# coolbeam/UPFlow_pytorch

Measured on AMD Instinct MI355X. Metric: frame-pairs/sec at 384x1280 bf16, higher is better.
Workload: dtype bf16; 1 GPU; config2: UPFlow_net inference forward (flow fwd+bwd, occlusion masks, SGU on), 384x1280, batch 4 per GPU, random-init weights; global_batch=4, parallelism=replicas x1 (image pairs sharded, no collective), ranks=1, hip_graph=True, capture_fallback=False, steps_in_flight=4, pyramid_convs=HIP (MFMA kernel), pyramid_dtype=fp16

## Files before the change

### include/upflow_hip.h

```cpp
#ifndef UPFLOW_HIP_H
#define UPFLOW_HIP_H

#ifdef __cplusplus
extern "C" {
#endif

enum { UPF_F32 = 0, UPF_F16 = 1, UPF_BF16 = 2 };
enum { UPF_OK = 0, UPF_EINVAL = -1, UPF_EDTYPE = -2, UPF_EALIGN = -3, UPF_EUNSUPPORTED = -4 };
enum { UPF_MASK_NONE = 0, UPF_MASK_LITERAL = 1, UPF_MASK_ROBUST = 2 };

const char* upf_version(void);
const char* upf_last_error(void);

int upf_corr81_forward(const void* f1, const void* f2, void* out,
                       int B, int C, int H, int W, int dtype,
                       long long out_batch_stride, float leaky_slope, void* stream);

int upf_corr81_forward_timed(const void* f1, const void* f2, void* out,
                             int B, int C, int H, int W, int dtype,
                             long long out_batch_stride, float leaky_slope, void* stream,
                             int nrep, float* avg_us, float* min_us);

int upf_corr81_norm_supported(int C, int dtype);
long long upf_corr81_norm_workspace_bytes(int B, int C, int H, int W);
int upf_corr81_norm_forward(const void* f1, const void* f2, void* out,
                            int B, int C, int H, int W, int dtype,
                            long long out_batch_stride, float leaky_slope, void* workspace, void* stream);
int upf_corr81_norm_forward_c8(const void* f1, const void* f2, void* out8, long long out8_batch_stride,
                               int B, int C, int H, int W, int dtype, float leaky_slope, void* workspace, void* stream);
int upf_corr81_norm_forward_pitched(const void* f1, const void* f2, int f_row_pitch, void* out,
                                    int B, int C, int H, int W, int dtype,
                                    long long out_batch_stride, float leaky_slope, void* workspace, void* stream);
int upf_corr81_norm_forward_c8_pitched(const void* f1, const void* f2, int f_row_pitch, void* out8, long long out8_batch_stride,
                                       int B, int C, int H, int W, int dtype, float leaky_slope, void* workspace, void* stream);
int upf_corr81_norm_forward_mixed(const void* f1, const void* f2, int f_row_pitch, void* out,
                                  int B, int C, int H, int W, int dtype, int out_dtype,
                                  long long out_batch_stride, float leaky_slope, void* workspace, void* stream);
int upf_corr81_norm_forward_c8_mixed(const void* f1, const void* f2, int f_row_pitch, void* out8, long long out8_batch_stride,
                                     int B, int C, int H, int W, int dtype, int out_dtype, float leaky_slope, void* workspace, void* stream);
int upf_corr81_norm_forward_timed(const void* f1, const void* f2, void* out,
                                  int B, int C, int H, int W, int dtype,
                                  long long out_batch_stride, float leaky_slope, void* workspace, void* stream,
                                  int nrep, float* avg_us, float* min_us);
int upf_corr81_norm_forward_c8_timed(const void* f1, const void* f2, void* out8, long long out8_batch_stride,
                                     int B, int C, int H, int W, int dtype, float leaky_slope, void* workspace, void* stream,
                                     int nrep, float* avg_us, float* min_us);

int upf_corr81_norm_forward_c8_timed_pitched(const void* f1, const void* f2, int f_row_pitch, void* out8, long long out8_batch_stride,
                                             int B, int C, int H, int W, int dtype, float leaky_slope, void* workspace, void* stream,
                                             int nrep, float* avg_us, float* min_us);

int upf_corr81_norm_forward_c8_timed_mixed(const void* f1, const void* f2, int f_row_pitch, void* out8, long long out8_batch_stride,
                                           int B, int C, int H, int W, int dtype, int out_dtype, float leaky_slope, void* workspace, void* stream,
                                           int nrep, float* avg_us, float* min_us);

int upf_corr_set_option(const char* name, int value);

int upf_corr81_backward(const void* f1, const void* f2, const void* grad_out, void* g1, void* g2,
                        int B, int C, int H, int W, int dtype, void* stream);

int upf_correlation_forward(const void* in1, const void* in2, void* out,
                            int B, int C, int H, int W, int dtype,
                            int pad_size, int kernel_size, int max_displacement,
                            int stride1, int stride2, int corr_type_multiply, void* stream);
int upf_correlation_backward(const void* in1, const void* in2, const void* grad_out, void* g1, void* g2,
                             int B, int C, int H, int W, int dtype,
                             int pad_size, int kernel_size, int max_displacement,
                             int stride1, int stride2, int corr_type_multiply, void* stream);
int upf_correlation_out_shape(int H, int W, int pad_size, int kernel_size, int max_displacement,
                              int stride1, int stride2, int* out_channels, int* out_h, int* out_w);

int upf_warp_forward(const void* x, const float* flow, void* y,
                     int B, int C, int H, int W, int dtype, int mask_mode, int batch_shift, void* stream);
int upf_warp_forward_strided(const void* x, long long x_batch_stride, const float* flow, void* y, long long y_batch_stride,
                             int B, int C, int H, int W, int dtype, int mask_mode, int batch_shift, void* stream);
int upf_warp_forward_pitched(const void* x, long long x_batch_stride, int x_row_pitch, const float* flow, void* y, long long y_batch_stride,
                             int y_row_pitch, int B, int C, int H, int W, int dtype, int mask_mode, int batch_shift, void* stream);
int upf_warp_forward_c8(const void* x8, long long x_batch_stride, const float* flow, void* y8, long long y_batch_stride,
                        int B, int n_oct, int H, int W, int dtype, int mask_mode, int batch_shift, void* stream);
long long upf_warp_backward_workspace_bytes(int B, int C, int H, int W);
int upf_warp_backward(const void* x, const float* flow, const void* grad_y,
                      void* gx, float* gflow, void* workspace,
                      int B, int C, int H, int W, int dtype, int mask_mode, int batch_shift, void* stream);

int upf_flow_upsample_forward(const float* x, float* y, int B, int C, int h, int w, int H, int W,
                              int if_rate, void* stream);
int upf_flow_upsample_backward(const float* grad_y, float* gx, int B, int C, int h, int w, int H, int W,
                               int if_rate, void* stream);

long long upf_sgu_blend_forward_workspace_bytes(int B, int h, int w, int Hf, int Wf);
int upf_sgu_blend_forward(const float* flow_init, const void* x_out, float* flow_up,
                          float* inter_flow, float* inter_mask, void* workspace,
                          int B, int h, int w, int Hf, int Wf, int dtype, void* stream);
int upf_sgu_blend_forward_flow16(const float* flow_init, const void* x_out, float* flow_up, void* flow16, long long flow16_batch_stride,
                                 int flow16_is_c8, int B, int H, int W, int dtype, void* stream);
long long upf_sgu_blend_backward_workspace_bytes(int B, int h, int w, int Hf, int Wf);
int upf_sgu_blend_backward(const float* flow_init, const void* x_out, const float* grad_flow_up,
                           float* g_flow_init32, float* g_x_out32, void* workspace,
                           int B, int h, int w, int Hf, int Wf, int dtype, void* stream);

long long upf_normalize_workspace_bytes(long long N, int HW);
int upf_normalize_forward(const void* x, void* y, float* mean, float* rstd, void* workspace,
                          long long N, int HW, int dtype, void* stream);
int upf_normalize_backward(const void* y, const void* grad_y, const float* rstd, void* gx,
                           long long N, int HW, int dtype, void* stream);

long long upf_conv_packed_bytes(int Cin, int Cout, int kernel_size);
int upf_conv_pack_weights(const void* w , void* w_packed, int Cin, int Cout, int kernel_size,
                          int dtype, void* stream);
int upf_conv_forward(const void* x, long long x_batch_stride, const void* w_packed, const float* bias,
                     void* y, long long y_batch_stride, int B, int Cin, int Cout, int H, int W,
                     int kernel_size, int dilation, int stride, float leaky_slope, int dtype, void* stream);
int upf_conv_forward_pitched(const void* x, long long x_batch_stride, int x_row_pitch, const void* w_packed, const float* bias,
                             void* y, long long y_batch_stride, int y_row_pitch, int B, int Cin, int Cout, int H, int W,
                             int kernel_size, int dilation, int stride, float leaky_slope, int dtype, void* stream);
int upf_conv1x1_forward_mixed(const void* x, long long x_batch_stride, int x_row_pitch, const void* w_packed, const float* bias,
                              void* y, long long y_batch_stride, int y_row_pitch, int y_is_c8, int B, int Cin, int Cout, int H, int W,
                              float leaky_slope, int dtype, int out_dtype, void* stream);
int upf_conv1x1_forward_c8_dual(const void* x, long long x_batch_stride, int x_row_pitch, const void* w_packed, const float* bias,
                                void* y8_a, long long ya_batch_stride, void* y8_b, long long yb_batch_stride,
                                int B, int Cin, int Cout, int H, int W, float leaky_slope, int dtype, int out_dtype, void* stream);
int upf_conv_set_option(const char* name, int value);

long long upf_conv_x3_packed_bytes(int Cin, int Cout, int kernel_size);
int upf_conv_x3_pack_weights(const float* w, void* w_packed, int Cin, int Cout, int kernel_size, void* stream);
int upf_conv_x3_forward(const float* x, long long x_batch_stride, const void* w_packed, const float* bias, float* y,
                        long long y_batch_stride, int B, int Cin, int Cout, int H, int W, int kernel_size, int dilation,
                        int stride, float leaky_slope, int nprod, void* stream);
int upf_conv_x3_set_option(const char* name, int value);
int upf_mfma_f16_denorm_probe(float* out_device, void* stream);

long long upf_conv_packed_bytes_k(int K, int Cout, int kernel_size);
int upf_conv_c8_k(int n8_oct, int C2);
int upf_conv_pack_weights_kmap(const void* w , void* w_packed, int Cin, int Cout, int kernel_size,
                               const int* kmap , int K, int dtype, void* stream);
int upf_conv_forward_c8(const void* x8, long long x8_batch_stride, int n8_oct, const void* x2, long long x2_batch_stride, int C2,
                        const void* w_packed, const float* bias, void* y, long long y_batch_stride, int y_is_c8,
                        int B, int Cout, int H, int W, int kernel_size, int dilation, int stride, float leaky_slope,
                        int dtype, void* stream);
int upf_conv_forward_c8_pitched(const void* x8, long long x8_batch_stride, int n8_oct, const void* x2, long long x2_batch_stride, int x2_row_pitch, int C2,
                                const void* w_packed, const float* bias, void* y, long long y_batch_stride, int y_row_pitch, int y_is_c8,
                                int B, int Cout, int H, int W, int kernel_size, int dilation, int stride, float leaky_slope,
                                int dtype, void* stream);
int upf_conv_c8_set_option(const char* name, int value);
long long upf_conv_packed_bytes_k16(int K, int Cout);
int upf_conv_pack_weights_kmap16(const void* w , void* w_packed, int Cin, int Cout,
                                 const int* kmap , int K, int dtype, void* stream);
int upf_conv_forward_c8_narrow(const void* x8, long long x8_batch_stride, int n8_oct, const void* w_packed16, const float* bias,
                               void* y, long long y_batch_stride, int y_is_c8, int B, int Cout, int H, int W, float leaky_slope,
                               int dtype, void* stream);
int upf_conv_forward_c8_split(const void* x8, long long x8_batch_stride, int n8_oct, const void* w_packed ,
                              const float* bias , void* y8, long long y_batch_stride, int C_main,
                              float* partial, long long partial_batch_stride , int partial_pitch ,
                              int B, int Cout, int H, int W, float leaky_slope, int dtype, void* stream);
int upf_conv_forward_c8_narrow_init(const void* x8, long long x8_batch_stride, int n8_oct, const void* w_packed16,
                                    const float* partial, long long partial_batch_stride, int partial_pitch, int partial_offset ,
                                    void* y, long long y_batch_stride, int y_is_c8, int B, int Cout, int H, int W, float leaky_slope,
                                    int dtype, void* stream);

int upf_conv_pair_forward(const void* x, long long x_batch_stride, int x_row_pitch, int Cin,
                          const void* wa_packed, const float* bias_a , float slope_a, int C1, int stride_a,
                          const void* wb_packed, const float* bias_b , float slope_b, int C2, int stride_b,
                          void* y, long long y_batch_stride, int y_row_pitch, int y_is_c8,
                          int B, int H, int W, int dtype, void* stream);

int upf_conv_pack_weights_f32(const float* w , void* w_packed, int Cin, int Cout, int kernel_size,
                              int dtype, int dgrad, void* stream);
int upf_conv_pack_weights_f32_multi(const float* const* w, void* const* w_packed, const int* Cin, const int* Cout, const int* kernel_size,
                                    const int* dgrad, int njobs, int dtype, void* stream);
int upf_conv_pack_stacked_dgrad(const float* const* w, const int* Cin, const int* Cout, const int* first_channel, int nlayers,
                                void* const* w_packed, const int* slice_channel, const int* slice_width, const int* nconsumers,
                                int nslices, int dtype, void* stream);
int upf_leaky_backward(const void* grad_y, const void* y, void* grad_pre, long long n, float slope, int dtype, void* stream);
int upf_conv_wgrad_supported(int Cin, int Cout, int H, int W, int kernel_size, int dilation, int stride, int dtype);
long long upf_conv_wgrad_workspace_bytes(int B, int Cin, int Cout, int H, int W, int kernel_size, int dilation);
int upf_conv_wgrad(const void* x, long long x_batch_stride, const void* grad_pre, long long g_batch_stride, float* grad_w,
                   void* workspace, int B, int Cin, int Cout, int H, int W, int kernel_size, int dilation, int dtype, void* stream);
typedef struct {
  const void* x;        long long x_batch_stride;
  const void* grad_pre; long long g_batch_stride;
  int B, H, W;
} upf_wgrad_level;
long long upf_conv_wgrad_multi_workspace_bytes(const upf_wgrad_level* levels, int nlevels, int Cin, int Cout, int kernel_size, int dilation);
int upf_conv_wgrad_multi(const upf_wgrad_level* levels , int nlevels, float* grad_w, void* workspace, int Cin, int Cout,
                         int kernel_size, int dilation, int dtype, void* stream);
int upf_conv_wgrad_multi_bias(const upf_wgrad_level* levels, int nlevels, float* grad_w, void* workspace, int Cin, int Cout,
                              int kernel_size, int dilation, const float* const* bias_partials , int npartials, float* grad_bias,
                              int dtype, void* stream);
int upf_space_to_depth2(const void* src, void* dst, int B, int C , int H, int W , int inverse, int dtype, void* stream);
int upf_conv_wgrad_s2d(const upf_wgrad_level* levels, int nlevels, float* grad_w, void* workspace, int Cin, int Cout, int dtype, void* stream);
int upf_act_grad(const void* src, long long src_batch_stride, const void* add, long long add_batch_stride, const void* y,
                 long long y_batch_stride, void* dst, long long dst_batch_stride, float* bias_partial, int B, int C, int HW,
                 float slope, int dtype, void* stream);
int upf_conv_forward_gated(const void* x, long long x_batch_stride, int x_row_pitch, const void* w_packed, const float* bias,
                           void* y, long long y_batch_stride, int y_row_pitch, const void* add, long long add_batch_stride,
                           const void* act, long long act_batch_stride, float mask_slope,
                           int B, int Cin, int Cout, int H, int W, int dtype, void* stream);
int upf_conv_bias_grad_finish(const float* const* partials , int npartials, float* grad_bias,
                              int Cout, void* stream);
long long upf_conv_bias_grad_workspace_bytes(int Cout);
int upf_conv_bias_grad(const void* grad_pre, long long g_batch_stride, float* grad_bias, void* workspace, int B, int Cout, int HW,
                       int dtype, void* stream);

int upf_act_grad_x3(const float* grad_y, long long gy_batch_stride, const float* y, long long y_batch_stride, float* grad_pre_scaled,
                    long long dst_batch_stride, float* bias_partial, float* scale_slot, int B, int C, int HW, float slope, void* stream);
int upf_conv_x3_pack_weights_dgrad(const float* w, void* w_packed, int Cin, int Cout, int kernel_size, void* stream);
int upf_conv_x3_dgrad(const float* grad_pre_scaled, long long g_batch_stride, const float* scale_slot, const float* w,
                      void* w_packed_dgrad, const float* zero_bias, float* grad_x, long long gx_batch_stride, int B, int Cin,
                      int Cout, int H, int W, int kernel_size, int dilation, int stride, void* stream);
int upf_conv_x3_wgrad_workspace_bytes(const upf_wgrad_level* levels, int nlevels, int Cin, int Cout, int kernel_size,
                                      int dilation, int stride, long long* bytes );
int upf_conv_x3_wgrad(const upf_wgrad_level* levels , const float* const* scale_slots , int nlevels,
                      float* grad_w, void* workspace, int Cin, int Cout, int kernel_size, int dilation, int stride,
                      const float* const* bias_partials , float* grad_bias, void* stream);

int upf_flow_update(const float* a, const void* b, const void* c, void* out, long long out_batch_stride,
                    int out_is_f32, int N, int per_item, int dtype, void* stream);
int upf_flow_update_c8(const float* a, const void* b, const void* c, void* out8, long long out8_batch_stride,
                       int N, int HW, int dtype, void* stream);

int upf_occ_check(const float* flow_f, const float* flow_b, float* occ_fw, float* occ_bw,
                  int B, int H, int W, float alpha1, float alpha2, void* stream);

int upf_div_selftest(int size, unsigned long long* mismatches, void* stream);

int upf_census_forward(const float* gray1, const float* gray2, float* dist, int B, int H, int W, int max_distance, void* stream);
int upf_census_backward(const float* gray1, const float* gray2, const float* grad_dist, float* g_gray1, float* g_gray2,
                        int B, int H, int W, int max_distance, void* stream);

int upf_boundary_warp_forward(const float* image, const float* flow, const float* start, float* out,
                              int B, int C, int Hi, int Wi, int h, int w, void* stream);
int upf_boundary_warp_backward(const float* image, const float* flow, const float* start, const float* grad_out,
                               float* grad_flow, int B, int C, int Hi, int Wi, int h, int w, void* stream);

int upf_loss_partials(long long n_pixels);

int upf_robust_loss_forward(const float* x, const float* y, const float* occ, float* partials,
                            int B, int C, int HW, float eps, float q, void* stream);
int upf_robust_loss_backward(const float* x, const float* y, const float* occ, const float* coef,
                             float* grad_x, float* grad_y, int B, int C, int HW, float eps, float q, void* stream);

int upf_grey_forward(const float* image, float* grey, int B, int HW, void* stream);

int upf_msd_upup_partials(int B, int H, int W);
int upf_msd_upup_forward(const float* const* x_low, const int* hs, const int* ws, int nlevels, const float* y, const float* occ,
                         float* partials, float* out2, int B, int H, int W, float weight, float eps, float q, void* stream);
int upf_msd_upup_backward(const float* const* x_low, float* const* grad_x_low, const int* hs, const int* ws, int nlevels, const float* y,
                          const float* occ, const float* grad_out, const float* fwd_out2, int B, int H, int W, float weight, float eps, float q,
                          void* stream);

int upf_smooth_edge1_forward(const float* img, const float* pred, float* partials,
                             int B, int Ci, int Cp, int H, int W, void* stream);
int upf_smooth_edge1_backward(const float* img, const float* pred, const float* grad_up, float* grad_pred,
                              int B, int Ci, int Cp, int H, int W, void* stream);


int upf_smooth_edge2_forward(const float* img, const float* pred, float* partials,
                             int B, int Ci, int Cp, int H, int W, void* stream);
int upf_smooth_edge2_backward(const float* img, const float* pred, const float* grad_up, float* grad_pred,
                              int B, int Ci, int Cp, int H, int W, void* stream);

int upf_smooth_delta_forward(const float* flow, float* partials, int BC, int H, int W, int second_order, void* stream);
int upf_smooth_delta_backward(const float* flow, const float* grad_up, float* grad_flow, int BC, int H, int W,
                              int second_order, void* stream);

enum { UPF_LOSS_CHARBONNIER = 0, UPF_LOSS_L1 = 1 };
int upf_pointwise_loss_forward(const float* x, const float* y, const float* occ, float* partials,
                               int B, int C, int HW, int kind, float q, void* stream);
int upf_pointwise_loss_backward(const float* x, const float* y, const float* occ, const float* coef,
                                float* grad_x, float* grad_y, int B, int C, int HW, int kind, float q, void* stream);

int upf_ssim_forward(const float* x, const float* y, const float* weight, float* map, float* w_avg, float* partials,
                     int B, int C, int H, int W, float c2, float weight_epsilon, void* stream);
int upf_ssim_backward(const float* x, const float* y, const float* weight, const float* grad_map,
                      const float* coef_w, const float* coef_u, float* grad_x, float* grad_y,
                      int B, int C, int H, int W, float c2, float weight_epsilon, void* stream);

#define UPF_MT_TENSORS 48
#define UPF_MT_BLOCKS 256
#define UPF_MT_CHUNK 16384
typedef struct {
  void* param[UPF_MT_TENSORS];
  void* grad[UPF_MT_TENSORS];
  void* exp_avg[UPF_MT_TENSORS];
  void* exp_avg_sq[UPF_MT_TENSORS];
  void* max_exp_avg_sq[UPF_MT_TENSORS];
  int numel[UPF_MT_TENSORS];
  int block_chunk[UPF_MT_BLOCKS];
  unsigned char block_tensor[UPF_MT_BLOCKS];
  int n_tensors, n_blocks;
} upf_mt_launch;
int upf_grads_nonfinite_check(const upf_mt_launch* launch, int* flag, void* stream);
int upf_adam_amsgrad_step(const upf_mt_launch* launch, const float* lr, const float* step, const float* loss_scale,
                          const int* flag, double beta1, double beta2, double eps, double weight_decay, void* stream);
int upf_loss_scale_update(float* loss_scale, int* growth_tracker, int* skipped_steps, int* flag, float* steps, int nsteps,
                          float growth_factor, float backoff_factor, int growth_interval, void* stream);

int upf_frames_u8_assemble(const unsigned char* src1, const unsigned char* src2, const int* aug, float* raw1, float* raw2,
                           float* crop1, float* crop2, float* start, int B, int H, int W, int ph, int pw,
                           double mean0, double mean1, double mean2, double stddev, void* stream);

int upf_frames_u8_stack16(const unsigned char* src1, const unsigned char* src2, const int* flip,
                          void* x, int x_dtype, long long x_pitch, long long x_batch_stride,
                          void* xd, int xd_dtype, long long xd_pitch, long long xd_batch_stride,
                          int B, int H, int W, double mean0, double mean1, double mean2, double stddev, void* stream);

#ifdef __cplusplus
}
#endif
#endif
```

### upflow_pytorch_amd/_build.py

```python
import os
import subprocess
import sys

PKG = os.path.dirname(os.path.abspath(__file__))
CSRC = os.path.join(PKG, 'csrc')
LIB = os.path.join(PKG, 'libupflow_hip.so')

SOURCES = [
    ('api.hip', []),
    ('corr81_fwd.hip', ['-ffp-contract=off']),
    ('corr81_bwd.hip', []),
    ('conv3x3.hip', []),
    ('conv_c8.hip', []),
    ('conv_pair.hip', []),
    ('conv_x3.hip', []),
    ('conv_x3_bwd.hip', []),
    ('conv_wgrad.hip', []),
    ('warp.hip', ['-ffp-contract=off']),
    ('sgu_blend.hip', ['-ffp-contract=off']),
    ('misc.hip', ['-ffp-contract=off']),
    ('loss.hip', ['-ffp-contract=off']),
    ('loss_variants.hip', ['-ffp-contract=off']),
    ('optim.hip', ['-ffp-contract=off']),
    ('ingest.hip', ['-ffp-contract=off']),
]
COMMON = ['--offload-arch=gfx950', '-O3', '-std=c++17', '-fPIC', '-fno-gpu-rdc', '-Wall', '-Wno-unused-function']
NO_PACKED_FP32 = ['-Xclang', '-target-feature', '-Xclang', '-packed-fp32-ops']


def hipcc():
    for c in (os.environ.get('HIPCC'), '/opt/rocm/bin/hipcc', 'hipcc'):
        if c and (os.path.isabs(c) and os.path.exists(c) or not os.path.isabs(c)):
            return c
    raise RuntimeError('hipcc not found')


def _stale(target, deps):
    if not os.path.exists(target):
        return True
    t = os.path.getmtime(target)
    return any(os.path.getmtime(d) > t for d in deps)


def _flags_tag(extra):
    import hashlib
    return hashlib.sha256(' '.join(COMMON + NO_PACKED_FP32 + list(extra)).encode()).hexdigest()[:16]


def _flags_stale(obj, extra):
    try:
        return open(obj + '.flags').read().strip() != _flags_tag(extra)
    except OSError:
        return True


def build(force=False, verbose=False):
    headers = [os.path.join(CSRC, h) for h in os.listdir(CSRC) if h.endswith('.hpp')]
    headers.append(os.path.join(os.path.dirname(PKG), 'include', 'upflow_hip.h'))
    objdir = os.path.join(PKG, 'build')
    os.makedirs(objdir, exist_ok=True)
    objs = []
    cc = hipcc()
    jobs = []
    for src, extra in SOURCES:
        s = os.path.join(CSRC, src)
        o = os.path.join(objdir, src.replace('.hip', '.o'))
        objs.append(o)
        if force or _stale(o, [s] + headers) or _flags_stale(o, extra):
            jobs.append(([cc] + COMMON + NO_PACKED_FP32 + extra + ['-c', s, '-o', o], o, extra))

    def run(job):
        cmd, obj, extra = job
        if os.path.exists(obj + '.flags'):
            os.remove(obj + '.flags')
        if verbose:
            print(' '.join(cmd), flush=True)
        r = subprocess.run(cmd, stderr=subprocess.PIPE, text=True)
        err = '\n'.join(l for l in r.stderr.splitlines() if 'is not a recognized feature for this target' not in l)
        if err.strip():
            sys.stderr.write(err + '\n')
        if r.returncode:
            raise subprocess.CalledProcessError(r.returncode, cmd)
        with open(obj + '.flags', 'w') as f:
            f.write(_flags_tag(extra) + '\n')
    if jobs:
        from concurrent.futures import ThreadPoolExecutor
        with ThreadPoolExecutor(max_workers=min(len(jobs), os.cpu_count() or 1)) as ex:
            list(ex.map(run, jobs))
    if force or _stale(LIB, objs):
        cmd = [cc, '--offload-arch=gfx950', '-shared', '-fPIC', '-o', LIB] + objs
        if verbose:
            print(' '.join(cmd), flush=True)
        subprocess.check_call(cmd)
    return LIB


if __name__ == '__main__':
    print(build(force='--force' in sys.argv, verbose=True))
```

### upflow_pytorch_amd/_lib.py

```python
import ctypes
import os

import torch

_PKG = os.path.dirname(os.path.abspath(__file__))
LIB_PATH = os.environ.get('UPF_HIP_LIB') or os.path.join(_PKG, 'libupflow_hip.so')

UPF_F32, UPF_F16, UPF_BF16 = 0, 1, 2
MASK_NONE, MASK_LITERAL, MASK_ROBUST = 0, 1, 2
_DTYPES = {torch.float32: UPF_F32, torch.float16: UPF_F16, torch.bfloat16: UPF_BF16}

_c = ctypes
_vp, _i, _f, _ll, _d = _c.c_void_p, _c.c_int, _c.c_float, _c.c_longlong, _c.c_double

SIGNATURES = {
    'upf_corr81_forward': [_vp, _vp, _vp, _i, _i, _i, _i, _i, _ll, _f, _vp],
    'upf_corr81_forward_timed': [_vp, _vp, _vp, _i, _i, _i, _i, _i, _ll, _f, _vp, _i, _c.POINTER(_f), _c.POINTER(_f)],
    'upf_corr81_norm_forward': [_vp, _vp, _vp, _i, _i, _i, _i, _i, _ll, _f, _vp, _vp],
    'upf_corr81_norm_forward_timed': [_vp, _vp, _vp, _i, _i, _i, _i, _i, _ll, _f, _vp, _vp, _i, _c.POINTER(_f), _c.POINTER(_f)],
    'upf_corr81_norm_forward_c8_timed': [_vp, _vp, _vp, _ll, _i, _i, _i, _i, _i, _f, _vp, _vp, _i, _c.POINTER(_f), _c.POINTER(_f)],
    'upf_corr81_norm_forward_pitched': [_vp, _vp, _i, _vp, _i, _i, _i, _i, _i, _ll, _f, _vp, _vp],
    'upf_corr81_norm_forward_c8_pitched': [_vp, _vp, _i, _vp, _ll, _i, _i, _i, _i, _i, _f, _vp, _vp],
    'upf_corr81_norm_forward_c8_timed_pitched': [_vp, _vp, _i, _vp, _ll, _i, _i, _i, _i, _i, _f, _vp, _vp, _i, _c.POINTER(_f), _c.POINTER(_f)],
    'upf_corr81_norm_forward_c8_timed_mixed': [_vp, _vp, _i, _vp, _ll, _i, _i, _i, _i, _i, _i, _f, _vp, _vp, _i, _c.POINTER(_f), _c.POINTER(_f)],
    'upf_warp_forward_pitched': [_vp, _ll, _i, _vp, _vp, _ll, _i, _i, _i, _i, _i, _i, _i, _i, _vp],
    'upf_conv_forward_gated': [_vp, _ll, _i, _vp, _vp, _vp, _ll, _i, _vp, _ll, _vp, _ll, _f, _i, _i, _i, _i, _i, _i, _vp],
    'upf_conv_forward_pitched': [_vp, _ll, _i, _vp, _vp, _vp, _ll, _i, _i, _i, _i, _i, _i, _i, _i, _i, _f, _i, _vp],
    'upf_conv_forward_c8_pitched': [_vp, _ll, _i, _vp, _ll, _i, _i, _vp, _vp, _vp, _ll, _i, _i, _i, _i, _i, _i, _i, _i, _i, _f, _i, _vp],
    'upf_corr81_norm_forward_mixed': [_vp, _vp, _i, _vp, _i, _i, _i, _i, _i, _i, _ll, _f, _vp, _vp],
    'upf_corr81_norm_forward_c8_mixed': [_vp, _vp, _i, _vp, _ll, _i, _i, _i, _i, _i, _i, _f, _vp, _vp],
    'upf_conv1x1_forward_mixed': [_vp, _ll, _i, _vp, _vp, _vp, _ll, _i, _i, _i, _i, _i, _i, _i, _f, _i, _i, _vp],
    'upf_conv1x1_forward_c8_dual': [_vp, _ll, _i, _vp, _vp, _vp, _ll, _vp, _ll, _i, _i, _i, _i, _i, _f, _i, _i, _vp],
    'upf_corr81_backward': [_vp, _vp, _vp, _vp, _vp, _i, _i, _i, _i, _i, _vp],
    'upf_correlation_forward': [_vp, _vp, _vp, _i, _i, _i, _i, _i, _i, _i, _i, _i, _i, _i, _vp],
    'upf_correlation_backward': [_vp, _vp, _vp, _vp, _vp, _i, _i, _i, _i, _i, _i, _i, _i, _i, _i, _i, _vp],
    'upf_correlation_out_shape': [_i, _i, _i, _i, _i, _i, _i, _c.POINTER(_i), _c.POINTER(_i), _c.POINTER(_i)],
    'upf_warp_forward': [_vp, _vp, _vp, _i, _i, _i, _i, _i, _i, _i, _vp],
    'upf_warp_forward_strided': [_vp, _ll, _vp, _vp, _ll, _i, _i, _i, _i, _i, _i, _i, _vp],
    'upf_warp_forward_c8': [_vp, _ll, _vp, _vp, _ll, _i, _i, _i, _i, _i, _i, _i, _vp],
    'upf_flow_update': [_vp, _vp, _vp, _vp, _ll, _i, _i, _i, _i, _vp],
    'upf_flow_update_c8': [_vp, _vp, _vp, _vp, _ll, _i, _i, _i, _vp],
    'upf_corr81_norm_forward_c8': [_vp, _vp, _vp, _ll, _i, _i, _i, _i, _i, _f, _vp, _vp],
    'upf_warp_backward': [_vp, _vp, _vp, _vp, _vp, _vp, _i, _i, _i, _i, _i, _i, _i, _vp],
    'upf_flow_upsample_forward': [_vp, _vp, _i, _i, _i, _i, _i, _i, _i, _vp],
    'upf_flow_upsample_backward': [_vp, _vp, _i, _i, _i, _i, _i, _i, _i, _vp],
    'upf_sgu_blend_forward': [_vp, _vp, _vp, _vp, _vp, _vp, _i, _i, _i, _i, _i, _i, _vp],
    'upf_sgu_blend_forward_flow16': [_vp, _vp, _vp, _vp, _ll, _i, _i, _i, _i, _i, _vp],
    'upf_sgu_blend_backward': [_vp, _vp, _vp, _vp, _vp, _vp, _i, _i, _i, _i, _i, _i, _vp],
    'upf_normalize_forward': [_vp, _vp, _vp, _vp, _vp, _ll, _i, _i, _vp],
    'upf_normalize_backward': [_vp, _vp, _vp, _vp, _ll, _i, _i, _vp],
    'upf_conv_pack_weights': [_vp, _vp, _i, _i, _i, _i, _vp],
    'upf_conv_forward': [_vp, _ll, _vp, _vp, _vp, _ll, _i, _i, _i, _i, _i, _i, _i, _i, _f, _i, _vp],
    'upf_conv_x3_pack_weights': [_vp, _vp, _i, _i, _i, _vp],
    'upf_conv_x3_forward': [_vp, _ll, _vp, _vp, _vp, _ll, _i, _i, _i, _i, _i, _i, _i, _i, _f, _i, _vp],
    'upf_mfma_f16_denorm_probe': [_vp, _vp],
    'upf_act_grad_x3': [_vp, _ll, _vp, _ll, _vp, _ll, _vp, _vp, _i, _i, _i, _f, _vp],
    'upf_conv_x3_pack_weights_dgrad': [_vp, _vp, _i, _i, _i, _vp],
    'upf_conv_x3_dgrad': [_vp, _ll, _vp, _vp, _vp, _vp, _vp, _ll, _i, _i, _i, _i, _i, _i, _i, _i, _vp],
    'upf_conv_x3_wgrad_workspace_bytes': [_vp, _i, _i, _i, _i, _i, _i, _c.POINTER(_ll)],
    'upf_conv_x3_wgrad': [_vp, _vp, _i, _vp, _vp, _i, _i, _i, _i, _i, _vp, _vp, _vp],
    'upf_conv_pack_weights_f32': [_vp, _vp, _i, _i, _i, _i, _i, _vp],
    'upf_conv_pack_stacked_dgrad': [_c.POINTER(_vp), _c.POINTER(_i), _c.POINTER(_i), _c.POINTER(_i), _i, _c.POINTER(_vp), _c.POINTER(_i), _c.POINTER(_i), _c.POINTER(_i), _i, _i, _vp],
    'upf_conv_pack_weights_f32_multi': [_c.POINTER(_vp), _c.POINTER(_vp), _c.POINTER(_i), _c.POINTER(_i), _c.POINTER(_i), _c.POINTER(_i), _i, _i, _vp],
    'upf_conv_pack_weights_kmap': [_vp, _vp, _i, _i, _i, _vp, _i, _i, _vp],
    'upf_conv_forward_c8': [_vp, _ll, _i, _vp, _ll, _i, _vp, _vp, _vp, _ll, _i, _i, _i, _i, _i, _i, _i, _i, _f, _i, _vp],
    'upf_conv_pack_weights_kmap16': [_vp, _vp, _i, _i, _vp, _i, _i, _vp],
    'upf_conv_forward_c8_narrow': [_vp, _ll, _i, _vp, _vp, _vp, _ll, _i, _i, _i, _i, _i, _f, _i, _vp],
    'upf_conv_forward_c8_split': [_vp, _ll, _i, _vp, _vp, _vp, _ll, _i, _vp, _ll, _i, _i, _i, _i, _i, _f, _i, _vp],
    'upf_conv_forward_c8_narrow_init': [_vp, _ll, _i, _vp, _vp, _ll, _i, _i, _vp, _ll, _i, _i, _i, _i, _i, _f, _i, _vp],
    'upf_conv_pair_forward': [_vp, _ll, _i, _i, _vp, _vp, _f, _i, _i, _vp, _vp, _f, _i, _i, _vp, _ll, _i, _i, _i, _i, _i, _i, _vp],
    'upf_leaky_backward': [_vp, _vp, _vp, _ll, _f, _i, _vp],
    'upf_conv_wgrad': [_vp, _ll, _vp, _ll, _vp, _vp, _i, _i, _i, _i, _i, _i, _i, _i, _vp],
    'upf_conv_bias_grad': [_vp, _ll, _vp, _vp, _i, _i, _i, _i, _vp],
    'upf_conv_wgrad_multi': [_vp, _i, _vp, _vp, _i, _i, _i, _i, _i, _vp],
    'upf_conv_wgrad_multi_bias': [_vp, _i, _vp, _vp, _i, _i, _i, _i, _vp, _i, _vp, _i, _vp],
    'upf_space_to_depth2': [_vp, _vp, _i, _i, _i, _i, _i, _i, _vp],
    'upf_conv_wgrad_s2d': [_vp, _i, _vp, _vp, _i, _i, _i, _vp],
    'upf_act_grad': [_vp, _ll, _vp, _ll, _vp, _ll, _vp, _ll, _vp, _i, _i, _i, _f, _i, _vp],
    'upf_conv_bias_grad_finish': [_vp, _i, _vp, _i, _vp],
    'upf_census_forward': [_vp, _vp, _vp, _i, _i, _i, _i, _vp],
    'upf_census_backward': [_vp, _vp, _vp, _vp, _vp, _i, _i, _i, _i, _vp],
    'upf_boundary_warp_forward': [_vp, _vp, _vp, _vp, _i, _i, _i, _i, _i, _i, _vp],
    'upf_boundary_warp_backward': [_vp, _vp, _vp, _vp, _vp, _i, _i, _i, _i, _i, _i, _vp],
    'upf_robust_loss_forward': [_vp, _vp, _vp, _vp, _i, _i, _i, _f, _f, _vp],
    'upf_robust_loss_backward': [_vp, _vp, _vp, _vp, _vp, _vp, _i, _i, _i, _f, _f, _vp],
    'upf_grey_forward': [_vp, _vp, _i, _i, _vp],
    'upf_msd_upup_forward': [_vp, _vp, _vp, _i, _vp, _vp, _vp, _vp, _i, _i, _i, _f, _f, _f, _vp],
    'upf_msd_upup_backward': [_vp, _vp, _vp, _vp, _i, _vp, _vp, _vp, _vp, _i, _i, _i, _f, _f, _f, _vp],
    'upf_smooth_edge1_forward': [_vp, _vp, _vp, _i, _i, _i, _i, _i, _vp],
    'upf_smooth_edge1_backward': [_vp, _vp, _vp, _vp, _i, _i, _i, _i, _i, _vp],
    'upf_smooth_edge2_forward': [_vp, _vp, _vp, _i, _i, _i, _i, _i, _vp],
    'upf_smooth_edge2_backward': [_vp, _vp, _vp, _vp, _i, _i, _i, _i, _i, _vp],
    'upf_smooth_delta_forward': [_vp, _vp, _i, _i, _i, _i, _vp],
    'upf_smooth_delta_backward': [_vp, _vp, _vp, _i, _i, _i, _i, _vp],
    'upf_pointwise_loss_forward': [_vp, _vp, _vp, _vp, _i, _i, _i, _i, _f, _vp],
    'upf_pointwise_loss_backward': [_vp, _vp, _vp, _vp, _vp, _vp, _i, _i, _i, _i, _f, _vp],
    'upf_ssim_forward': [_vp, _vp, _vp, _vp, _vp, _vp, _i, _i, _i, _i, _f, _f, _vp],
    'upf_ssim_backward': [_vp, _vp, _vp, _vp, _vp, _vp, _vp, _vp, _i, _i, _i, _i, _f, _f, _vp],
    'upf_div_selftest': [_i, _vp, _vp],
    'upf_occ_check': [_vp, _vp, _vp, _vp, _i, _i, _i, _f, _f, _vp],
    'upf_grads_nonfinite_check': [_vp, _vp, _vp],
    'upf_adam_amsgrad_step': [_vp, _vp, _vp, _vp, _vp, _d, _d, _d, _d, _vp],
    'upf_loss_scale_update': [_vp, _vp, _vp, _vp, _vp, _i, _f, _f, _i, _vp],
    'upf_frames_u8_assemble': [_vp, _vp, _vp, _vp, _vp, _vp, _vp, _vp, _i, _i, _i, _i, _i, _d, _d, _d, _d, _vp],
    'upf_frames_u8_stack16': [_vp, _vp, _vp, _vp, _i, _ll, _ll, _vp, _i, _ll, _ll, _i, _i, _i, _d, _d, _d, _d, _vp],
}



class WgradLevel(_c.Structure):
    _fields_ = [('x', _vp), ('x_batch_stride', _ll), ('grad_pre', _vp), ('g_batch_stride', _ll), ('B', _i), ('H', _i), ('W', _i)]


MT_TENSORS, MT_BLOCKS, MT_CHUNK = 48, 256, 16384


class MtLaunch(_c.Structure):
    _fields_ = [('param', _vp * MT_TENSORS), ('grad', _vp * MT_TENSORS), ('exp_avg', _vp * MT_TENSORS),
                ('exp_avg_sq', _vp * MT_TENSORS), ('max_exp_avg_sq', _vp * MT_TENSORS), ('numel', _i * MT_TENSORS),
                ('block_chunk', _i * MT_BLOCKS), ('block_tensor', _c.c_ubyte * MT_BLOCKS), ('n_tensors', _i), ('n_blocks', _i)]


_lib = None


class UpflowHipError(RuntimeError):
    """Raised for a rejected argument or a failed launch (the reference raises RuntimeError through
    AT_ERROR("CUDA call failed"), correlation_cuda.cc:81-83)."""


def lib():
    global _lib
    if _lib is None:
        if not os.path.exists(LIB_PATH):
            raise UpflowHipError(
                '%s is missing: build it with `python -c "import __graft_entry__ as g; g.build()"` '
                '(hipcc --offload-arch=gfx950). There is no CPU fallback.' % LIB_PATH)
        L = ctypes.CDLL(LIB_PATH)
        for name, argtypes in SIGNATURES.items():
            fn = getattr(L, name)
            fn.argtypes = argtypes
            fn.restype = _i
        L.upf_normalize_workspace_bytes.argtypes = [_ll, _i]
        L.upf_normalize_workspace_bytes.restype = _ll
        L.upf_corr81_norm_supported.argtypes = [_i, _i]
        L.upf_corr81_norm_supported.restype = _i
        L.upf_corr81_norm_workspace_bytes.argtypes = [_i, _i, _i, _i]
        L.upf_corr81_norm_workspace_bytes.restype = _ll
        L.upf_corr_set_option.argtypes = [_c.c_char_p, _i]
        L.upf_corr_set_option.restype = _i
        L.upf_warp_backward_workspace_bytes.argtypes = [_i, _i, _i, _i]
        L.upf_warp_backward_workspace_bytes.restype = _ll
        L.upf_sgu_blend_backward_workspace_bytes.argtypes = [_i, _i, _i, _i, _i]
        L.upf_sgu_blend_backward_workspace_bytes.restype = _ll
        L.upf_sgu_blend_forward_workspace_bytes.argtypes = [_i, _i, _i, _i, _i]
        L.upf_sgu_blend_forward_workspace_bytes.restype = _ll
        L.upf_conv_wgrad_supported.argtypes = [_i] * 8
        L.upf_conv_wgrad_supported.restype = _i
        L.upf_conv_wgrad_workspace_bytes.argtypes = [_i] * 7
        L.upf_conv_wgrad_workspace_bytes.restype = _ll
        L.upf_conv_wgrad_multi_workspace_bytes.argtypes = [_vp, _i, _i, _i, _i, _i]
        L.upf_conv_wgrad_multi_workspace_bytes.restype = _ll
        L.upf_conv_bias_grad_workspace_bytes.argtypes = [_i]
        L.upf_conv_bias_grad_workspace_bytes.restype = _ll
        L.upf_loss_partials.argtypes = [_ll]
        L.upf_loss_partials.restype = _i
        L.upf_msd_upup_partials.argtypes = [_i, _i, _i]
        L.upf_msd_upup_partials.restype = _i
        L.upf_conv_packed_bytes.argtypes = [_i, _i, _i]
        L.upf_conv_packed_bytes.restype = _ll
        L.upf_conv_x3_packed_bytes.argtypes = [_i, _i, _i]
        L.upf_conv_x3_packed_bytes.restype = _ll
        L.upf_conv_set_option.argtypes = [_c.c_char_p, _i]
        L.upf_conv_set_option.restype = _i
        L.upf_conv_c8_set_option.argtypes = [_c.c_char_p, _i]
        L.upf_conv_c8_set_option.restype = _i
        L.upf_conv_x3_set_option.argtypes = [_c.c_char_p, _i]
        L.upf_conv_x3_set_option.restype = _i
        L.upf_conv_packed_bytes_k.argtypes = [_i, _i, _i]
        L.upf_conv_packed_bytes_k.restype = _ll
        L.upf_conv_c8_k.argtypes = [_i, _i]
        L.upf_conv_c8_k.restype = _i
        L.upf_conv_packed_bytes_k16.argtypes = [_i, _i]
        L.upf_conv_packed_bytes_k16.restype = _ll
        L.upf_version.restype = _c.c_char_p
        L.upf_last_error.restype = _c.c_char_p
        _lib = L
        for item in filter(None, os.environ.get('UPF_CONV_OPTS', '').split(',')):
            k, v = item.split('=')
            if L.upf_conv_set_option(k.strip().encode(), int(v)) == -2 ** 31:
                raise UpflowHipError('UPF_CONV_OPTS: unknown option %r' % k)
    return _lib


def version():
    return lib().upf_version().decode()


def dtype_code(t):
    try:
        return _DTYPES[t.dtype]
    except KeyError:
        raise UpflowHipError('unsupported dtype %s (float32 / float16 / bfloat16 only)' % t.dtype)


def check_gpu(*tensors, contiguous=True):
    dev = None
    for t in tensors:
        if t is None:
            continue
        if not t.is_cuda:
            raise UpflowHipError('upflow_pytorch_amd operators run on the GPU only (got a %s tensor); '
                                 'there is no CPU fallback' % t.device)
        if contiguous and not t.is_contiguous():
            raise UpflowHipError('operand must be contiguous NCHW')
        if dev is None:
            dev = t.device
        elif t.device != dev:
            raise UpflowHipError('operands on different devices: %s vs %s' % (dev, t.device))
    return dev


def stream_ptr(device):
    return _vp(torch.cuda.current_stream(device).cuda_stream)


def ptr(t):
    return _vp(t.data_ptr()) if t is not None else _vp(0)


def call(name, *args):
    rc = getattr(lib(), name)(*args)
    if rc != 0:
        raise UpflowHipError('%s failed (%d): %s' % (name, rc, lib().upf_last_error().decode()))


def launch(device, name, *args):
    with torch.cuda.device(device):
        call(name, *args, stream_ptr(device))
```

### upflow_pytorch_amd/csrc/conv_c8.hip

```cpp
#include "conv_kernel.hpp"

namespace upf {
namespace conv {

template <typename T>
__global__ void pack_weights_kmap_kernel(const T* __restrict__ w, T* __restrict__ wp, int Cin, int Cout, int ntaps, const int* __restrict__ kmap, int K) {
  const int cop = pad32(Cout), nk = K / 16;
  const long long total = (long long)ntaps * cop * K;
  for (long long i = blockIdx.x * (long long)blockDim.x + threadIdx.x; i < total; i += (long long)gridDim.x * blockDim.x) {
    const int j = (int)(i & 7), px = (int)((i >> 3) & 31), kg = (int)((i >> 8) & 1);
    const long long b = i >> 9;
    const int tap = (int)(b % ntaps), kstep = (int)((b / ntaps) % nk), slab = (int)(b / ((long long)ntaps * nk));
    const int co = slab * 32 + px, kk = kstep * 16 + kg * 8 + j;
    const int ci = kmap[kk];
    T v; v.v = 0;
    if (ci >= 0 && ci < Cin && co < Cout) v = w[((size_t)co * Cin + ci) * ntaps + tap];
    wp[i] = v;
  }
}

template <typename T>
__global__ void pack_weights_kmap16_kernel(const T* __restrict__ w, T* __restrict__ wp, int Cin, int Cout, int ntaps, const int* __restrict__ kmap, int K) {
  const int nblk = (Cout + 15) / 16, nch = K / 32;
  const long long total = (long long)nblk * nch * ntaps * 512;
  for (long long i = blockIdx.x * (long long)blockDim.x + threadIdx.x; i < total; i += (long long)gridDim.x * blockDim.x) {
    const int j = (int)(i & 7), lane = (int)((i >> 3) & 63);
    const long long b = i >> 9;
    const int tap = (int)(b % ntaps), chunk = (int)((b / ntaps) % nch), blk = (int)(b / ((long long)ntaps * nch));
    const int co = blk * 16 + (lane & 15), kk = chunk * 32 + (lane >> 4) * 8 + j;
    const int ci = kmap[kk];
    T v; v.v = 0;
    if (ci >= 0 && ci < Cin && co < Cout) v = w[((size_t)co * Cin + ci) * ntaps + tap];
    wp[i] = v;
  }
}

struct ArgsC8 {
  const void* x8; long long x8bs; int n8oct;
  const void* x2; long long x2bs; int C2;
  const void* wp; const float* bias; void* y; long long ybs;
  int B, Cout, H, W, d, stride, ntaps; float slope; hipStream_t stream;
  int x2pitch, ypitch;
};

template <typename T, int MTW, int RPW, int S, int NOCTS, int D, int XL, bool YC8, bool N16 = false>
int launch_one_c8(const ArgsC8& a, int slabs) {
  constexpr int TH = (4 / MTW) * RPW;
  constexpr bool PH = (D >= 2 && S == 1);
  constexpr int DV = PH ? 1 : D;
  constexpr int rowsC = S * (TH - 1) + 2 * DV + 1;
  constexpr int XWP = xwp_eff(XL, S, D);
  constexpr int EB = NOCTS * rowsC * XWP, EBP = (EB + 63) & ~63;
  const int Ho = (a.H - 1) / S + 1, Wo = (a.W - 1) / S + 1;
  const int tiles_x = cdiv(Wo, TW), tiles_y = PH ? cdiv(Ho, D * TH) * D : cdiv(Ho, TH);
  size_t lds = (XL >= 1) ? (size_t)2 * EBP * 16 : (size_t)EB * 16;
  if (!YC8 && !N16 && lds < 4 * EPI_WAVE_BYTES) lds = 4 * EPI_WAVE_BYTES;
  UPF_REQUIRE(lds <= 160 * 1024, UPF_EUNSUPPORTED, "conv_forward_c8: tile does not fit LDS (dilation %d)", a.d);
  static LdsOptIn opt;
  auto kern = &conv_kernel<T, MTW, RPW, S, NOCTS, D, false, false, XL, YC8, N16>;
  opt.ensure(reinterpret_cast<const void*>(kern), lds);
  hipLaunchKernelGGL(kern, dim3((unsigned)(a.B * tiles_x * tiles_y), slabs), dim3(NTHREADS), lds, a.stream, (const T*)a.x2, a.x2bs,
                     (const T*)a.wp, a.bias, (T*)a.y, a.ybs, a.C2, a.Cout, a.H, a.W, Ho, Wo, g_ablate, tiles_x, tiles_y, a.slope,
                     (const T*)a.x8, a.x8bs, a.n8oct, a.x2pitch, a.ypitch);
  return check_launch("conv_forward_c8");
}

inline int g_c8_rpw4 = 1;
inline int g_c8_narrow_tall = 0;

template <typename T, int XL, bool YC8>
int launch_c8(const ArgsC8& a) {
  const int mt = cdiv(a.Cout, 32);
  const long long tiles = (long long)a.B * cdiv(a.W, TW) * cdiv(a.H, 8);
  int mtw = mt >= 3 ? 4 : mt;
  if (tiles <= g_small_grid && mt > 1) mtw = 2;
  if (g_force_mtw == 1 || g_force_mtw == 2 || g_force_mtw == 4) mtw = g_force_mtw < (mt >= 3 ? 4 : mt) ? g_force_mtw : (mt >= 3 ? 4 : mt);
  const int slabs = cdiv(mt, mtw);
  if (a.ntaps == 1) {
    if constexpr (XL == 0 && YC8) {
      if (mtw == 1) return launch_one_c8<T, 1, 2, 1, 4, 0, 0, true>(a, slabs);
    }
    set_error("conv_forward_c8: 1x1 kernels take an NCHW input, a C8 output and Cout <= 32");
    return UPF_EUNSUPPORTED;
  }
  if (a.stride == 2) {
    if constexpr (XL == 0 && YC8) {
      if (a.d == 1 && a.Cout <= 32 && a.C2 > 16) return launch_one_c8<T, 1, 2, 2, 4, 1, 0, true>(a, 1);
    }
    set_error("conv_forward_c8: stride 2 takes an NCHW input of more than 16 channels, a C8 output of at most 32 channels, dilation 1");
    return UPF_EUNSUPPORTED;
  }
  if (a.d == 1) {
    if constexpr (XL == 0 && YC8) {
      if (mtw == 4) return launch_one_c8<T, 4, 8, 1, 2, 1, 0, true>(a, slabs);
      if (mtw == 2) return launch_one_c8<T, 2, 4, 1, 4, 1, 0, true>(a, slabs);
      return launch_one_c8<T, 1, 2, 1, 4, 1, 0, true>(a, slabs);
    }
    if constexpr (XL >= 1) {
      if (mtw == 4) return launch_one_c8<T, 4, 8, 1, 2, 1, XL, YC8>(a, slabs);
      if (mtw == 2) return launch_one_c8<T, 2, 4, 1, 4, 1, XL, YC8>(a, slabs);
      if (g_c8_rpw4 && (long long)a.B * cdiv(a.W, TW) * cdiv(a.H, 16) >= g_rpw4_min) return launch_one_c8<T, 1, 4, 1, 2, 1, XL, YC8>(a, slabs);
      return launch_one_c8<T, 1, 2, 1, 4, 1, XL, YC8>(a, slabs);
    }
  }
  if constexpr (XL == 1 && YC8) {
    if (a.d == 2 || a.d == 4 || a.d == 8 || a.d == 16) {
      const int th = g_ph_fit ? ph_tile_rows(a.H, a.d, mtw) : 8;
#define UPF_C8_PH(MT, RP)                                                              \
      switch (a.d) {                                                                   \
        case 2: return launch_one_c8<T, MT, RP, 1, wide_nocts<MT, 2>(), 2, 1, true>(a, slabs);   \
        case 4: return launch_one_c8<T, MT, RP, 1, wide_nocts<MT, 4>(), 4, 1, true>(a, slabs);   \
        case 8: return launch_one_c8<T, MT, RP, 1, wide_nocts<MT, 8>(), 8, 1, true>(a, slabs);   \
        default: return launch_one_c8<T, MT, RP, 1, wide_nocts<MT, 16>(), 16, 1, true>(a, slabs); \
      }
      if (mtw == 4) { if (th == 6) { UPF_C8_PH(4, 6) } if (th == 4) { UPF_C8_PH(4, 4) } UPF_C8_PH(4, 8) }
      if (mtw == 2) { if (th == 6) { UPF_C8_PH(2, 3) } if (th == 4) { UPF_C8_PH(2, 2) } UPF_C8_PH(2, 4) }
      if (th == 4) { UPF_C8_PH(1, 1) }
      UPF_C8_PH(1, 2)
#undef UPF_C8_PH
    }
  }
  set_error("conv_forward_c8: no kernel for this combination (kernel %d taps, dilation %d, input layout %d, output C8 %d)", a.ntaps, a.d, XL, (int)YC8);
  return UPF_EUNSUPPORTED;
}

template <typename T>
int dispatch_c8(const ArgsC8& a, bool y_c8) {
  const int xl = a.x8 ? (a.x2 ? 2 : 1) : 0;
  if (xl == 2) return y_c8 ? launch_c8<T, 2, true>(a) : launch_c8<T, 2, false>(a);
  if (xl == 1) return y_c8 ? launch_c8<T, 1, true>(a) : launch_c8<T, 1, false>(a);
  if (y_c8) return launch_c8<T, 0, true>(a);
  set_error("conv_forward_c8: NCHW in, NCHW out is upf_conv_forward");
  return UPF_EINVAL;
}

}
}

extern "C" long long upf_conv_packed_bytes_k(int K, int Cout, int kernel_size) {
  return (long long)kernel_size * kernel_size * upf::conv::pad32(Cout) * (long long)K * 2;
}

extern "C" int upf_conv_c8_k(int n8_oct, int C2) {
  return (n8_oct > 0 ? upf::conv::pad32(n8_oct * 8) : 0) + (C2 > 0 ? upf::conv::pad32(C2) : 0);
}

extern "C" int upf_conv_pack_weights_kmap(const void* w, void* w_packed, int Cin, int Cout, int kernel_size, const int* kmap, int K,
                                          int dtype, void* stream) {
  using namespace upf;
  UPF_REQUIRE(w && w_packed && kmap && Cin > 0 && Cout > 0, UPF_EINVAL, "conv_pack_weights_kmap: bad arguments");
  UPF_REQUIRE(kernel_size == 3 || kernel_size == 1, UPF_EUNSUPPORTED, "conv_pack_weights_kmap: kernel_size %d (1 or 3)", kernel_size);
  UPF_REQUIRE(K > 0 && K % 32 == 0, UPF_EINVAL, "conv_pack_weights_kmap: K = %d must be a positive multiple of 32", K);
  UPF_REQUIRE(dtype == UPF_BF16 || dtype == UPF_F16, UPF_EDTYPE, "conv: bf16 / fp16 only");
  const int ntaps = kernel_size * kernel_size;
  const long long total = (long long)ntaps * conv::pad32(Cout) * K;
  const int blocks = (int)((total + 255) / 256 > 4096 ? 4096 : (total + 255) / 256);
  if (dtype == UPF_BF16)
    hipLaunchKernelGGL((conv::pack_weights_kmap_kernel<bf16_t>), dim3(blocks), dim3(256), 0, (hipStream_t)stream, (const bf16_t*)w, (bf16_t*)w_packed, Cin, Cout, ntaps, kmap, K);
  else
    hipLaunchKernelGGL((conv::pack_weights_kmap_kernel<f16_t>), dim3(blocks), dim3(256), 0, (hipStream_t)stream, (const f16_t*)w, (f16_t*)w_packed, Cin, Cout, ntaps, kmap, K);
  return check_launch("conv_pack_weights_kmap");
}

extern "C" int upf_conv_c8_set_option(const char* name, int value) {
  using namespace upf::conv;
  int* slot = nullptr;
  if (name && !strcmp(name, "rpw4")) slot = &g_c8_rpw4;
  else if (name && !strcmp(name, "narrow_tall")) slot = &g_c8_narrow_tall;
  if (!slot) return INT32_MIN;
  const int prev = *slot;
  *slot = value;
  return prev;
}

extern "C" int upf_conv_forward_c8_pitched(const void* x8, long long x8_batch_stride, int n8_oct, const void* x2, long long x2_batch_stride, int x2_row_pitch, int C2,
                                           const void* w_packed, const float* bias, void* y, long long y_batch_stride, int y_row_pitch, int y_is_c8,
                                           int B, int Cout, int H, int W, int kernel_size, int dilation, int stride, float leaky_slope,
                                           int dtype, void* stream) {
  using namespace upf;
  UPF_REQUIRE((x8 || x2) && w_packed && bias && y, UPF_EINVAL, "conv_forward_c8: null pointer");
  UPF_REQUIRE((x8 != nullptr) == (n8_oct > 0) && (x2 != nullptr) == (C2 > 0), UPF_EINVAL, "conv_forward_c8: a pointer and its channel count disagree");
  UPF_REQUIRE(B > 0 && Cout > 0 && H > 0 && W > 0, UPF_EINVAL, "conv_forward_c8: bad shape B=%d Cout=%d H=%d W=%d", B, Cout, H, W);
  UPF_REQUIRE(dtype == UPF_BF16 || dtype == UPF_F16, UPF_EDTYPE, "conv_forward_c8: bf16 / fp16 only");
  UPF_REQUIRE(kernel_size == 3 || kernel_size == 1, UPF_EUNSUPPORTED, "conv_forward_c8: kernel_size %d (1 or 3)", kernel_size);
  UPF_REQUIRE(stride == 1 || (stride == 2 && kernel_size == 3 && dilation == 1 && !x8), UPF_EUNSUPPORTED, "conv_forward_c8: stride %d (1, or 2 for a 3x3 with an NCHW input)", stride);
  UPF_REQUIRE(dilation >= 1 && dilation <= conv::MAXD, UPF_EUNSUPPORTED, "conv_forward_c8: dilation %d not in [1,%d]", dilation, conv::MAXD);
  const int Ho = (H - 1) / stride + 1, Wo = (W - 1) / stride + 1;
  if (x2_row_pitch == 0) x2_row_pitch = W;
  if (y_row_pitch == 0) y_row_pitch = Wo;
  UPF_REQUIRE(!x2 || (x2_row_pitch >= W && x2_row_pitch % 8 == 0), UPF_EUNSUPPORTED,
              "conv_forward_c8: the NCHW input's row pitch %d must be a multiple of 8 and >= W = %d (pitched rows, or upf_conv_forward)", x2_row_pitch, W);
  UPF_REQUIRE(y_is_c8 || y_row_pitch >= Wo, UPF_EINVAL, "conv_forward_c8: output row pitch %d < %d", y_row_pitch, Wo);
  UPF_REQUIRE(!x8 || (aligned_to(x8, 16) && x8_batch_stride % 8 == 0), UPF_EINVAL, "conv_forward_c8: the C8 input must be 16-byte aligned");
  UPF_REQUIRE(!x2 || (aligned_to(x2, 16) && x2_batch_stride % 8 == 0), UPF_EINVAL, "conv_forward_c8: the NCHW input must be 16-byte aligned");
  UPF_REQUIRE(!y_is_c8 || (aligned_to(y, 16) && y_batch_stride % 8 == 0), UPF_EINVAL, "conv_forward_c8: the C8 output must be 16-byte aligned");
  UPF_REQUIRE((long long)n8_oct * H * W * 16 < (1ll << 31) && (long long)C2 * H * x2_row_pitch * 2 < (1ll << 31), UPF_EINVAL, "conv_forward_c8: image too large for one buffer descriptor");
  UPF_REQUIRE((long long)((Cout + 7) / 8) * (H / stride + 1) * (W / stride + 1) * 16 < (1ll << 31) && (y_is_c8 || (long long)Cout * Ho * y_row_pitch * 2 < (1ll << 31)), UPF_EINVAL,
              "conv_forward_c8: output too large for one buffer descriptor");
  UPF_REQUIRE(leaky_slope >= 0.f && leaky_slope <= 1.f, UPF_EINVAL, "conv_forward_c8: leaky_slope %g not in [0,1]", (double)leaky_slope);
  conv::ArgsC8 a{x8, x8_batch_stride, n8_oct, x2, x2_batch_stride, C2, w_packed, bias, y, y_batch_stride,
                 B, Cout, H, W, kernel_size == 1 ? 0 : dilation, stride, kernel_size * kernel_size, leaky_slope == 0.f ? 1.f : leaky_slope, (hipStream_t)stream,
                 x2_row_pitch, y_row_pitch};
  return dtype == UPF_BF16 ? conv::dispatch_c8<bf16_t>(a, y_is_c8 != 0) : conv::dispatch_c8<f16_t>(a, y_is_c8 != 0);
}

extern "C" int upf_conv_forward_c8(const void* x8, long long x8_batch_stride, int n8_oct, const void* x2, long long x2_batch_stride, int C2,
                                   const void* w_packed, const float* bias, void* y, long long y_batch_stride, int y_is_c8,
                                   int B, int Cout, int H, int W, int kernel_size, int dilation, int stride, float leaky_slope,
                                   int dtype, void* stream) {
  return upf_conv_forward_c8_pitched(x8, x8_batch_stride, n8_oct, x2, x2_batch_stride, 0, C2, w_packed, bias, y, y_batch_stride, 0, y_is_c8,
                                     B, Cout, H, W, kernel_size, dilation, stride, leaky_slope, dtype, stream);
}

extern "C" long long upf_conv_packed_bytes_k16(int K, int Cout) {
  return (long long)((Cout + 15) / 16) * (upf::conv::pad32(K) / 32) * 9 * 1024;
}

extern "C" int upf_conv_pack_weights_kmap16(const void* w, void* w_packed, int Cin, int Cout, const int* kmap, int K, int dtype, void* stream) {
  using namespace upf;
  UPF_REQUIRE(w && w_packed && kmap && Cin > 0 && Cout > 0 && K > 0 && K % 32 == 0, UPF_EINVAL, "conv_pack_weights_kmap16: bad arguments (K %% 32 == 0)");
  UPF_REQUIRE(dtype == UPF_BF16 || dtype == UPF_F16, UPF_EDTYPE, "conv_pack_weights_kmap16: bf16 / fp16 only");
  const long long total = (long long)((Cout + 15) / 16) * (K / 32) * 9 * 512;
  const int blocks = (int)((total + 255) / 256 > 4096 ? 4096 : (total + 255) / 256);
  if (dtype == UPF_BF16)
    hipLaunchKernelGGL((conv::pack_weights_kmap16_kernel<bf16_t>), dim3(blocks), dim3(256), 0, (hipStream_t)stream, (const bf16_t*)w, (bf16_t*)w_packed, Cin, Cout, 9, kmap, K);
  else
    hipLaunchKernelGGL((conv::pack_weights_kmap16_kernel<f16_t>), dim3(blocks), dim3(256), 0, (hipStream_t)stream, (const f16_t*)w, (f16_t*)w_packed, Cin, Cout, 9, kmap, K);
  return check_launch("conv_pack_weights_kmap16");
}

extern "C" int upf_conv_forward_c8_narrow(const void* x8, long long x8_batch_stride, int n8_oct, const void* w_packed16, const float* bias,
                                          void* y, long long y_batch_stride, int y_is_c8, int B, int Cout, int H, int W, float leaky_slope,
                                          int dtype, void* stream) {
  using namespace upf;
  UPF_REQUIRE(x8 && n8_oct > 0 && w_packed16 && bias && y, UPF_EINVAL, "conv_forward_c8_narrow: null pointer");
  UPF_REQUIRE(B > 0 && Cout > 0 && H > 0 && W > 0, UPF_EINVAL, "conv_forward_c8_narrow: bad shape B=%d Cout=%d H=%d W=%d", B, Cout, H, W);
  UPF_REQUIRE(dtype == UPF_BF16 || dtype == UPF_F16, UPF_EDTYPE, "conv_forward_c8_narrow: bf16 / fp16 only");
  UPF_REQUIRE(aligned_to(x8, 16) && x8_batch_stride % 8 == 0, UPF_EINVAL, "conv_forward_c8_narrow: the C8 input must be 16-byte aligned");
  UPF_REQUIRE(!y_is_c8 || (aligned_to(y, 16) && y_batch_stride % 8 == 0), UPF_EINVAL, "conv_forward_c8_narrow: the C8 output must be 16-byte aligned");
  UPF_REQUIRE((long long)n8_oct * H * W * 16 < (1ll << 31), UPF_EINVAL, "conv_forward_c8_narrow: input too large for one buffer descriptor");
  UPF_REQUIRE((long long)(y_is_c8 ? (Cout + 7) / 8 * 8 : Cout) * H * W * 2 < (1ll << 31), UPF_EINVAL, "conv_forward_c8_narrow: output too large for one buffer descriptor");
  UPF_REQUIRE(leaky_slope >= 0.f && leaky_slope <= 1.f, UPF_EINVAL, "conv_forward_c8_narrow: leaky_slope %g not in [0,1]", (double)leaky_slope);
  conv::ArgsC8 a{x8, x8_batch_stride, n8_oct, nullptr, 0, 0, w_packed16, bias, y, y_batch_stride, B, Cout, H, W, 1, 1, 9,
                 leaky_slope == 0.f ? 1.f : leaky_slope, (hipStream_t)stream, W, W};
  const int blocks16 = (Cout + 15) / 16;
  const bool tall = conv::g_c8_narrow_tall && (long long)B * cdiv(W, conv::TW) * cdiv(H, 16) >= conv::g_rpw4_min;
#define UPF_N16(T)                                                                                                   \
  if (y_is_c8) return tall ? conv::launch_one_c8<T, 1, 4, 1, 4, 1, 1, true, true>(a, blocks16) : conv::launch_one_c8<T, 1, 2, 1, 4, 1, 1, true, true>(a, blocks16);   \
  return tall ? conv::launch_one_c8<T, 1, 4, 1, 4, 1, 1, false, true>(a, blocks16) : conv::launch_one_c8<T, 1, 2, 1, 4, 1, 1, false, true>(a, blocks16);
  if (dtype == UPF_BF16) { UPF_N16(bf16_t) }
  UPF_N16(f16_t)
#undef UPF_N16
}

namespace upf {
namespace conv {

template <typename T, int MTW, int RPW, int NOCTS>
int launch_split(const ArgsC8& a, const SplitOut& so) {
  constexpr int TH = (4 / MTW) * RPW;
  constexpr int rowsC = (TH - 1) + 2 + 1;
  constexpr int XWP = xwp_eff(1, 1, 1);
  constexpr int EB = NOCTS * rowsC * XWP, EBP = (EB + 63) & ~63;
  const int tiles_x = cdiv(a.W, TW), tiles_y = cdiv(a.H, TH);
  const size_t lds = (size_t)2 * EBP * 16;
  static LdsOptIn opt;
  auto kern = &conv_split_kernel<T, MTW, RPW, NOCTS>;
  opt.ensure(reinterpret_cast<const void*>(kern), lds);
  hipLaunchKernelGGL(kern, dim3((unsigned)(a.B * tiles_x * tiles_y), (unsigned)cdiv(cdiv(a.Cout, 32), MTW)), dim3(NTHREADS), lds, a.stream, (const T*)a.wp, a.bias, (T*)a.y, a.ybs,
                     a.Cout, a.H, a.W, tiles_x, tiles_y, a.slope, (const T*)a.x8, a.x8bs, a.n8oct, so);
  return check_launch("conv_forward_c8_split");
}

template <typename T>
int dispatch_split(const ArgsC8& a, const SplitOut& so) {
  const int mt = cdiv(a.Cout, 32);
  const long long tiles = (long long)a.B * cdiv(a.W, TW) * cdiv(a.H, 8);
  int mtw = mt >= 3 ? 4 : mt;
  if (tiles <= g_small_grid && mt > 1) mtw = 2;
  if (mtw == 4) return launch_split<T, 4, 8, 2>(a, so);
  if (mtw == 2) return launch_split<T, 2, 4, 4>(a, so);
  if (g_c8_rpw4 && (long long)a.B * cdiv(a.W, TW) * cdiv(a.H, 16) >= g_rpw4_min) return launch_split<T, 1, 4, 2>(a, so);
  return launch_split<T, 1, 2, 4>(a, so);
}

template <typename T, int RPW, bool YC8>
int launch_accinit(const ArgsC8& a, const AccInit& ai) {
  constexpr int TH = 4 * RPW;
  constexpr int rowsC = (TH - 1) + 2 + 1;
  constexpr int XWP = xwp_eff(1, 1, 1);
  constexpr int EB = 4 * rowsC * XWP, EBP = (EB + 63) & ~63;
  const int tiles_x = cdiv(a.W, TW), tiles_y = cdiv(a.H, TH);
  const size_t lds = (size_t)2 * EBP * 16;
  static LdsOptIn opt;
  auto kern = &conv_accinit_kernel<T, RPW, YC8>;
  opt.ensure(reinterpret_cast<const void*>(kern), lds);
  hipLaunchKernelGGL(kern, dim3((unsigned)(a.B * tiles_x * tiles_y), (unsigned)cdiv(a.Cout, 16)), dim3(NTHREADS), lds, a.stream, (const T*)a.wp, (T*)a.y, a.ybs,
                     a.Cout, a.H, a.W, tiles_x, tiles_y, a.slope, (const T*)a.x8, a.x8bs, a.n8oct, ai);
  return check_launch("conv_forward_c8_narrow_init");
}

}
}

extern "C" int upf_conv_forward_c8_split(const void* x8, long long x8_batch_stride, int n8_oct, const void* w_packed, const float* bias,
                                         void* y8, long long y_batch_stride, int C_main, float* partial, long long partial_batch_stride, int partial_pitch,
                                         int B, int Cout, int H, int W, float leaky_slope, int dtype, void* stream) {
  using namespace upf;
  UPF_REQUIRE(x8 && n8_oct > 0 && w_packed && bias && y8 && partial, UPF_EINVAL, "conv_forward_c8_split: null pointer");
  UPF_REQUIRE(B > 0 && H > 0 && W > 0, UPF_EINVAL, "conv_forward_c8_split: bad shape B=%d H=%d W=%d", B, H, W);
  UPF_REQUIRE(C_main > 0 && C_main % 8 == 0 && Cout > C_main && Cout <= 128, UPF_EINVAL,
              "conv_forward_c8_split: C_main = %d must be a positive multiple of 8 below Cout = %d <= 128", C_main, Cout);
  UPF_REQUIRE(partial_pitch % 4 == 0 && partial_pitch >= (Cout - C_main + 3) / 4 * 4, UPF_EINVAL,
              "conv_forward_c8_split: partial pitch %d must be a multiple of 4 floats holding the %d partial channels", partial_pitch, Cout - C_main);
  UPF_REQUIRE(dtype == UPF_BF16 || dtype == UPF_F16, UPF_EDTYPE, "conv_forward_c8_split: bf16 / fp16 only");
  UPF_REQUIRE(aligned_to(x8, 16) && x8_batch_stride % 8 == 0 && aligned_to(y8, 16) && y_batch_stride % 8 == 0 && aligned_to(partial, 16) && partial_batch_stride % 4 == 0,
              UPF_EINVAL, "conv_forward_c8_split: operands must be 16-byte aligned");
  UPF_REQUIRE((long long)n8_oct * H * W * 16 < (1ll << 31) && (long long)H * W * partial_pitch * 4 < (1ll << 31), UPF_EINVAL,
              "conv_forward_c8_split: image too large for one buffer descriptor");
  UPF_REQUIRE(leaky_slope >= 0.f && leaky_slope <= 1.f, UPF_EINVAL, "conv_forward_c8_split: leaky_slope %g not in [0,1]", (double)leaky_slope);
  conv::ArgsC8 a{x8, x8_batch_stride, n8_oct, nullptr, 0, 0, w_packed, bias, y8, y_batch_stride, B, Cout, H, W, 1, 1, 9,
                 leaky_slope == 0.f ? 1.f : leaky_slope, (hipStream_t)stream, W, W};
  const conv::SplitOut so{partial, partial_batch_stride, partial_pitch, C_main};
  return dtype == UPF_BF16 ? conv::dispatch_split<bf16_t>(a, so) : conv::dispatch_split<f16_t>(a, so);
}

extern "C" int upf_conv_forward_c8_narrow_init(const void* x8, long long x8_batch_stride, int n8_oct, const void* w_packed16,
                                               const float* partial, long long partial_batch_stride, int partial_pitch, int partial_offset,
                                               void* y, long long y_batch_stride, int y_is_c8, int B, int Cout, int H, int W, float leaky_slope,
                                               int dtype, void* stream) {
  using namespace upf;
  UPF_REQUIRE(x8 && n8_oct > 0 && w_packed16 && partial && y, UPF_EINVAL, "conv_forward_c8_narrow_init: null pointer");
  UPF_REQUIRE(B > 0 && Cout > 0 && Cout <= 16 && H > 0 && W > 0, UPF_EINVAL, "conv_forward_c8_narrow_init: bad shape B=%d Cout=%d (<= 16) H=%d W=%d", B, Cout, H, W);
  UPF_REQUIRE(partial_pitch % 4 == 0 && partial_offset % 4 == 0 && partial_offset >= 0 && partial_offset + (Cout + 3) / 4 * 4 <= partial_pitch, UPF_EINVAL,
              "conv_forward_c8_narrow_init: partial pitch %d / offset %d must be multiples of 4 floats holding the layer's %d channels", partial_pitch, partial_offset, Cout);
  UPF_REQUIRE(dtype == UPF_BF16 || dtype == UPF_F16, UPF_EDTYPE, "conv_forward_c8_narrow_init: bf16 / fp16 only");
  UPF_REQUIRE(aligned_to(x8, 16) && x8_batch_stride % 8 == 0 && aligned_to(partial, 16) && partial_batch_stride % 4 == 0, UPF_EINVAL,
              "conv_forward_c8_narrow_init: the C8 input and the partial must be 16-byte aligned");
  UPF_REQUIRE(!y_is_c8 || (aligned_to(y, 16) && y_batch_stride % 8 == 0), UPF_EINVAL, "conv_forward_c8_narrow_init: the C8 output must be 16-byte aligned");
  UPF_REQUIRE((long long)n8_oct * H * W * 16 < (1ll << 31) && (long long)H * W * partial_pitch * 4 < (1ll << 31), UPF_EINVAL,
              "conv_forward_c8_narrow_init: image too large for one buffer descriptor");
  UPF_REQUIRE((long long)(y_is_c8 ? (Cout + 7) / 8 * 8 : Cout) * H * W * 2 < (1ll << 31), UPF_EINVAL, "conv_forward_c8_narrow_init: output too large for one buffer descriptor");
  UPF_REQUIRE(leaky_slope >= 0.f && leaky_slope <= 1.f, UPF_EINVAL, "conv_forward_c8_narrow_init: leaky_slope %g not in [0,1]", (double)leaky_slope);
  conv::ArgsC8 a{x8, x8_batch_stride, n8_oct, nullptr, 0, 0, w_packed16, nullptr, y, y_batch_stride, B, Cout, H, W, 1, 1, 9,
                 leaky_slope == 0.f ? 1.f : leaky_slope, (hipStream_t)stream, W, W};
  const conv::AccInit ai{partial, partial_batch_stride, partial_pitch, partial_offset};
#define UPF_N16I(T) return y_is_c8 ? conv::launch_accinit<T, 2, true>(a, ai) : conv::launch_accinit<T, 2, false>(a, ai);
  if (dtype == UPF_BF16) { UPF_N16I(bf16_t) }
  UPF_N16I(f16_t)
#undef UPF_N16I
}
```

### upflow_pytorch_amd/csrc/conv_kernel.hpp

```cpp
#pragma once
#include "common.hpp"
#include <cstring>
#include <cstdint>

namespace upf {
namespace conv {

constexpr int TW = 32, NTHREADS = 256;
constexpr int MAXD = 16;
__host__ __device__ constexpr int margin_of(int D) { return (D == 16 || D < 0) ? 16 : 8; }
__host__ __device__ constexpr int xw(int S, int marg) { return S * TW + 2 * marg; }
#ifndef UPF_C8_TIGHT
#define UPF_C8_TIGHT 1
#endif
__host__ __device__ constexpr bool tight_rows(int XL) { return XL == 1 && UPF_C8_TIGHT != 0; }
__host__ __device__ constexpr int marg_eff(int XL, int D) { return tight_rows(XL) ? (D > 0 ? D : 0) : margin_of(D); }
__host__ __device__ constexpr int xw_eff(int XL, int S, int D) { return xw(S, marg_eff(XL, D)); }
__host__ __device__ constexpr int xwp_eff(int XL, int S, int D) { return tight_rows(XL) ? (xw_eff(XL, S, D) | 1) : xw_eff(XL, S, D) + xw_eff(XL, S, D) / 16; }

typedef __attribute__((ext_vector_type(8))) __bf16 bf16x8;
typedef __attribute__((ext_vector_type(8))) _Float16 f16x8;
typedef __attribute__((ext_vector_type(16))) float f32x16;
typedef __attribute__((ext_vector_type(4))) float f32x4;
typedef __attribute__((ext_vector_type(4))) unsigned int u32x4;
// ... 321 lines not shown
  const int colx[3] = {pos_of(marg + px - (D > 0 ? D : 0)), pos_of(marg + px), pos_of(marg + px + (D > 0 ? D : 0))};

  auto matrix_phase = [&](const uint4* __restrict__ xb, int cc) {
    __builtin_amdgcn_s_setprio(2);

    if (abl & 1) {
    } else if constexpr (N16) {
      constexpr int NR = RPW + 2;
      const int c16[2][3] = {{pos_of(marg + p16 - 1), pos_of(marg + p16), pos_of(marg + p16 + 1)}, {pos_of(marg + p16 + 15), pos_of(marg + p16 + 16), pos_of(marg + p16 + 17)}};
      uint4 bq[2][6];
      auto bload = [&](int sr, uint4 (&b)[6]) {
#pragma unroll
        for (int h = 0; h < 2; ++h)
#pragma unroll
          for (int kx = 0; kx < 3; ++kx) b[h * 3 + kx] = xb[(ko * rows + RPW * rg + sr) * XWP + c16[h][kx]];
      };
      bload(0, bq[0]);
#pragma unroll
      for (int sr = 0; sr < NR; ++sr) {
        if (sr + 1 < NR) bload(sr + 1, bq[(sr + 1) & 1]);
        __builtin_amdgcn_sched_barrier(0);
#pragma unroll
        for (int kx = 0; kx < 3; ++kx)
#pragma unroll
          for (int h = 0; h < 2; ++h)
#pragma unroll
            for (int ky = 0; ky < 3; ++ky)
              if (sr - ky >= 0 && sr - ky < RPW)
                acc16[sr - ky][h] = Mma16<T>::mma(wa[ky * 3 + kx][0], bq[sr & 1][h * 3 + kx], acc16[sr - ky][h]);
#pragma unroll
        for (int ky = 0; ky < 3; ++ky)
          if (sr == ky + RPW - 1) {
#pragma unroll
            for (int kx = 0; kx < 3; ++kx) wa[ky * 3 + kx][0] = wload(cc + 1, ky * 3 + kx, 0);
          }
        __builtin_amdgcn_sched_barrier(0);
      }
    } else if constexpr (REUSE) {
      constexpr int NR = RPW + 2 * DV;
      uint4 bq[2][3 * KS];
      auto bload = [&](int sr, uint4 (&b)[3 * KS]) {
#pragma unroll
        for (int kx = 0; kx < 3; ++kx)
#pragma unroll
          for (int ks = 0; ks < KS; ++ks) b[kx * KS + ks] = xb[((2 * ks + kg) * rows + RPW * rg + sr) * XWP + colx[kx]];
      };
      constexpr bool PIPEB = !ONE;
      if constexpr (PIPEB) bload(0, bq[0]);
#pragma unroll
      for (int sr = 0; sr < NR; ++sr) {
        if constexpr (PIPEB) { if (sr + 1 < NR) bload(sr + 1, bq[(sr + 1) & 1]); }
        else bload(sr, bq[sr & 1]);
        __builtin_amdgcn_sched_barrier(0);
#pragma unroll
        for (int kx = 0; kx < 3; ++kx)
#pragma unroll
          for (int ks = 0; ks < KS; ++ks)
#pragma unroll
            for (int ky = 0; ky < 3; ++ky)
              if (sr - ky * DV >= 0 && sr - ky * DV < RPW)
                acc[sr - ky * DV] = Mma32<T>::mma(wa[ky * 3 + kx][ks], bq[sr & 1][kx * KS + ks], acc[sr - ky * DV]);
#pragma unroll
        for (int ky = 0; ky < 3; ++ky)
          if (sr == ky * DV + RPW - 1) {
#pragma unroll
            for (int kx = 0; kx < 3; ++kx)
#pragma unroll
              for (int ks = 0; ks < KS; ++ks) wa[ky * 3 + kx][ks] = wload(cc + 1, ky * 3 + kx, ks);
          }
        __builtin_amdgcn_sched_barrier(0);
      }
    } else {
#pragma unroll
      for (int tap = 0; tap < ntaps; ++tap) {
        const int ky = (ntaps == 1) ? 1 : tap / 3, kx = (ntaps == 1) ? 1 : tap - 3 * (tap / 3);
        const int col = pos_of(marg + S * px + (kx - 1) * d);
#pragma unroll
        for (int ks = 0; ks < KS; ++ks)
#pragma unroll
          for (int r = 0; r < RPW; ++r) {
            const uint4 b = xb[((2 * ks + kg) * rows + S * (RPW * rg + r) + ky * (PH ? 1 : d)) * XWP + col];
            acc[r] = Mma32<T>::mma(wa[tap][ks], b, acc[r]);
          }
#pragma unroll
        for (int ks = 0; ks < KS; ++ks) wa[tap][ks] = wload(cc + 1, tap, ks);
      }
    }
    __builtin_amdgcn_s_setprio(0);
  };

  if constexpr (XL >= 1) {
    constexpr int rowsC = S * (TH - 1) + 2 * DV + 1;
    constexpr int EB = NOCTS * rowsC * XWP, EBP = (EB + 63) & ~63;
    constexpr int NSL = (EBP / 64 + 3) / 4;
    constexpr int DH = (D > 0) ? D : 0;
    const int wave_u = __builtin_amdgcn_readfirstlane(wave);
    __amdgpu_buffer_rsrc_t x8r = __builtin_amdgcn_make_buffer_rsrc(const_cast<T*>(x8 + (size_t)n * x8bs), 0, (uint32_t)n8oct * (uint32_t)HW * 16u, 0x00020000);
    uint32_t voff8[NSL];
#pragma unroll
    for (int j = 0; j < NSL; ++j) {
      const int p = (j * 4 + wave_u) * 64 + lane;
      const int oct = p / (rowsC * XWP), rem = p - oct * (rowsC * XWP), r = rem / XWP, pos = rem - r * XWP;
      const int grp = pos & ~7, col = LIN ? pos : (grp | ((pos - (grp >> 4)) & 7));
      const int gy = PH ? y0 + (r - 1) * RS : S * y0 - DV + r, gx = S * x0 - marg + col;
      const bool in = p < EB && pos < XW && col >= marg - DH && col < marg + S * TW + DH && gy >= 0 && gy < H && gx >= 0 && gx < W && !(abl & 2);
      voff8[j] = in ? (uint32_t)((oct * HW + gy * W + gx) * 16) : 0x80000000u;
    }
    auto land = [&](int cc) {
      if constexpr (XL == 2) {
        if (cc >= n8c && cc < nchunks) {
          uint4* xb = xs + (cc & 1) * EBP;
          if (tid < ntasks) stage_store<false>(xb, dst0, sh0, pre);
          for (int t = tid + NTHREADS; t < ntasks; t += NTHREADS) {
            uint32_t off; int dsti, sh;
            task_geom(t, off, dsti, sh);
            u32x4 ch[8];
            task_load(off, cc - n8c, ch);
            stage_store<false>(xb, dsti, sh, ch);
          }
        }
      }
    };
    for (int cc = -1; cc < nchunks; ++cc) {
      const int nx = cc + 1;
      if (nx < n8c) {
        const uint32_t cadd = (uint32_t)nx * (uint32_t)(NOCTS * 16) * (uint32_t)HW;
#pragma unroll
        for (int j = 0; j < NSL; ++j) {
          const int piece = j * 4 + wave_u;
          if (piece * 64 < EBP)
            __builtin_amdgcn_raw_ptr_buffer_load_lds(x8r, (__attribute__((address_space(3))) void*)(xs + ((nx & 1) * EBP + piece * 64)), 16, (int)(voff8[j] + cadd), 0, 0, 0);
        }
      } else if constexpr (XL == 2) {
        if (nx < nchunks) task_load(off0, nx - n8c, pre);
      }
      if (cc >= 0) matrix_phase(xs + (cc & 1) * EBP, cc);
      land(nx);
      asm volatile("s_waitcnt vmcnt(0)" ::: "memory");
      __syncthreads();
    }
  } else {
  for (int cc = 0; cc < nchunks; ++cc) {
      __syncthreads();
      if constexpr (PRE) { if (tid < ntasks) task_store(dst0, sh0, pre); }
      for (int t = tid + (PRE ? NTHREADS : 0); t < ntasks; t += NTHREADS) {
        uint32_t off; int dsti, sh;
        task_geom(t, off, dsti, sh);
        u32x4 ch[8];
        task_load(off, cc, ch);
        task_store(dsti, sh, ch);
      }
      __syncthreads();
      if constexpr (PRE) { if (cc + 1 < nchunks) task_load(off0, cc + 1, pre); }
      matrix_phase(xs, cc);
    }
  }

  const int gy0 = __builtin_amdgcn_readfirstlane(y0 + RPW * rg * RS);
  if constexpr (N16) {
    const uint32_t plane16 = (uint32_t)(Ho * Wo) * 16u, plane2 = (uint32_t)(Ho * ypitch) * 2u;
    __amdgpu_buffer_rsrc_t yr = __builtin_amdgcn_make_buffer_rsrc(y + (size_t)n * ybs, 0, YC8 ? (uint32_t)((Cout + 7) / 8) * plane16 : (uint32_t)Cout * plane2, 0x00020000);
#pragma unroll
    for (int r = 0; r < RPW; ++r) {
      const int gy = gy0 + r;
      if (gy < Ho) {
#pragma unroll
        for (int h = 0; h < 2; ++h) {
          const int gx = x0 + p16 + 16 * h;
          float v[4];
#pragma unroll
          for (int i = 0; i < 4; ++i) { v[i] = acc16[r][h][i]; v[i] = fmaxf(v[i], v[i] * slope); }
          if constexpr (YC8) {
            const uint32_t off = (gx < Wo) ? (uint32_t)(slab * 2 + (ko >> 1)) * plane16 + (uint32_t)(gy * Wo + gx) * 16u + (uint32_t)(ko & 1) * 8u : 0x80000000u;
            u32x2 o;
            o.x = pack2<TO>(v[0], v[1]); o.y = pack2<TO>(v[2], v[3]);
            __builtin_amdgcn_raw_buffer_store_b64(o, yr, off, 0, 0);
          } else {
            const uint32_t off = (gx < Wo) ? (uint32_t)(slab * 16 + 4 * ko) * plane2 + (uint32_t)(gy * ypitch + gx) * 2u : 0x80000000u;
            const uint32_t p01 = pack2<TO>(v[0], v[1]), p23 = pack2<TO>(v[2], v[3]);
            __builtin_amdgcn_raw_buffer_store_b16((unsigned short)p01, yr, off, 0, 0);
            __builtin_amdgcn_raw_buffer_store_b16((unsigned short)(p01 >> 16), yr, off + plane2, 0, 0);
            __builtin_amdgcn_raw_buffer_store_b16((unsigned short)p23, yr, off + 2u * plane2, 0, 0);
            __builtin_amdgcn_raw_buffer_store_b16((unsigned short)(p23 >> 16), yr, off + 3u * plane2, 0, 0);
          }
        }
      }
    }
    return;
  }
  if constexpr (!N16) {
  if constexpr (YC8) {
    const uint32_t plane16 = (uint32_t)(Ho * Wo) * 16u;
    int cout_y = Cout;
    if constexpr (G::split) cout_y = gate.cmain;
    __amdgpu_buffer_rsrc_t yr = __builtin_amdgcn_make_buffer_rsrc(y + (size_t)n * ybs, 0, (uint32_t)((cout_y + 7) / 8) * plane16, 0x00020000);
    const int gx = x0 + px;
    const uint32_t lane_off = (gx < Wo) ? (uint32_t)(slab * 4) * plane16 + (uint32_t)gx * 16u + (uint32_t)kg * 8u : 0x80000000u;
    __amdgpu_buffer_rsrc_t pr;
    if constexpr (G::split)
      pr = __builtin_amdgcn_make_buffer_rsrc(gate.part + (size_t)n * gate.pbs, 0, (uint32_t)(Ho * Wo) * (uint32_t)gate.ppitch * 4u, 0x00020000);
#pragma unroll
    for (int r = 0; r < RPW; ++r) {
      const int gy = gy0 + r * RS;
      if (gy < Ho) {
#pragma unroll
        for (int g = 0; g < 4; ++g) {
          if constexpr (G::split) {
            if (slab * 32 + 8 * g >= gate.cmain) {
              const int c0 = slab * 32 + 8 * g + 4 * kg;
              const uint32_t off = (gx < Wo && c0 < Cout) ? (uint32_t)(((c0 - gate.cmain) >> 2) * (Ho * Wo) + gy * Wo + gx) * 16u : 0x80000000u;
              f32x4 pv;
#pragma unroll
              for (int q = 0; q < 4; ++q) pv[q] = acc[r][4 * g + q];
              __builtin_amdgcn_raw_buffer_store_b128(__builtin_bit_cast(u32x4, pv), pr, off, 0, 0);
              continue;
            }
          }
          float v[4];
#pragma unroll
          for (int q = 0; q < 4; ++q) { v[q] = acc[r][4 * g + q]; v[q] = fmaxf(v[q], v[q] * slope); }
          u32x2 o;
          o.x = pack2<TO>(v[0], v[1]); o.y = pack2<TO>(v[2], v[3]);
          __builtin_amdgcn_raw_buffer_store_b64(o, yr, lane_off + (uint32_t)g * plane16 + (uint32_t)(gy * Wo) * 16u, 0, 0);
          if constexpr (G::dual) {
            __amdgpu_buffer_rsrc_t yr2 = __builtin_amdgcn_make_buffer_rsrc(gate.y2 + (size_t)n * gate.y2bs, 0, (uint32_t)((cout_y + 7) / 8) * plane16, 0x00020000);
            __builtin_amdgcn_raw_buffer_store_b64(o, yr2, lane_off + (uint32_t)g * plane16 + (uint32_t)(gy * Wo) * 16u, 0, 0);
          }
        }
      }
    }
    return;
  }
  if constexpr (!GEN) {
    if (((ypitch & 7) | (int)(ybs & 7) | (int)(reinterpret_cast<uintptr_t>(y) & 15)) == 0) {
      __syncthreads();
      if constexpr (G::on) {
        const GateRsrc gr = gate_init<T>(gate, n, (uint32_t)Cout * (uint32_t)(Ho * ypitch) * 2u);
        epilogue_wide<TO, RPW, true>(acc, reinterpret_cast<unsigned char*>(xs) + wave * EPI_WAVE_BYTES, y + (size_t)n * ybs, Cout, Ho, Wo,
                                    slab, lane, x0, gy0, RS, slope, ypitch, &gr);
      } else {
        epilogue_wide<TO, RPW>(acc, reinterpret_cast<unsigned char*>(xs) + wave * EPI_WAVE_BYTES, y + (size_t)n * ybs, Cout, Ho, Wo,
                              slab, lane, x0, gy0, RS, slope, ypitch);
      }
      return;
    }
  }
  Epilogue ep;
  epilogue_init<TO, true>(ep, y + (size_t)n * ybs, Cout, Ho, Wo, slab, lane, x0, ypitch);
  GateRsrc gr;
  if constexpr (G::on) gr = gate_init<T>(gate, n, (uint32_t)Cout * ep.plane2);
#pragma unroll
  for (int r = 0; r < RPW; ++r) {
    if (gy0 + r * RS < Ho) {
#pragma unroll
      for (int j = 0; j < 8; ++j)
        epilogue_store<TO, true, G::on>(ep, acc[r][2 * j], acc[r][2 * j + 1], epilogue_choff(j) * ep.plane2 + (uint32_t)((gy0 + r * RS) * ypitch) * 2u, slope, &gr);
    }
  }
  }
}

template <typename T, int MTW, int RPW, int S, int NOCTS, int D, bool GEN, bool ONE = false, int XL = 0, bool YC8 = false, bool N16 = false, typename TO = T>
__global__ __launch_bounds__(NTHREADS, (ONE && (MTW == 1 || (MTW == 2 && S == 1))) ? 4 : 2)
void conv_kernel(const T* __restrict__ x, long long xbs, const T* __restrict__ wp, const float* __restrict__ bias,
                 TO* __restrict__ y, long long ybs, int Cin, int Cout, int H, int W, int Ho, int Wo, int d_rt,
                 int tiles_x, int tiles_y, float slope, const T* __restrict__ x8, long long x8bs, int n8oct, int xpitch, int ypitch) {
  conv_body<T, MTW, RPW, S, NOCTS, D, GEN, ONE, XL, YC8, N16, TO, NoGate>(x, xbs, wp, bias, y, ybs, Cin, Cout, H, W, Ho, Wo, d_rt, tiles_x, tiles_y, slope,
                                                                          x8, x8bs, n8oct, xpitch, ypitch, NoGate{});
}

template <typename T, int MTW, int RPW, int S, int NOCTS, int D, bool GEN, bool ONE = false>
__global__ __launch_bounds__(NTHREADS, (ONE && (MTW == 1 || (MTW == 2 && S == 1))) ? 4 : 2)
void conv_gated_kernel(const T* __restrict__ x, long long xbs, const T* __restrict__ wp, const float* __restrict__ bias,
                       T* __restrict__ y, long long ybs, int Cin, int Cout, int H, int W, int Ho, int Wo, int d_rt,
                       int tiles_x, int tiles_y, float slope, int xpitch, int ypitch, const ActGate<T> gate) {
  conv_body<T, MTW, RPW, S, NOCTS, D, GEN, ONE, 0, false, false, T, ActGate<T>>(x, xbs, wp, bias, y, ybs, Cin, Cout, H, W, Ho, Wo, d_rt, tiles_x, tiles_y, slope,
                                                                                nullptr, 0ll, 0, xpitch, ypitch, gate);
}

template <typename T, int MTW, int RPW, int NOCTS>
__global__ __launch_bounds__(NTHREADS, 2)
void conv_split_kernel(const T* __restrict__ wp, const float* __restrict__ bias, T* __restrict__ y, long long ybs, int Cout, int H, int W,
                       int tiles_x, int tiles_y, float slope, const T* __restrict__ x8, long long x8bs, int n8oct, const SplitOut so) {
  conv_body<T, MTW, RPW, 1, NOCTS, 1, false, false, 1, true, false, T, SplitOut>(nullptr, 0ll, wp, bias, y, ybs, 0, Cout, H, W, H, W, 0, tiles_x, tiles_y, slope,
                                                                                  x8, x8bs, n8oct, W, W, so);
}
template <typename T, int RPW, bool YC8>
__global__ __launch_bounds__(NTHREADS, 2)
void conv_accinit_kernel(const T* __restrict__ wp, T* __restrict__ y, long long ybs, int Cout, int H, int W,
                         int tiles_x, int tiles_y, float slope, const T* __restrict__ x8, long long x8bs, int n8oct, const AccInit ai) {
  conv_body<T, 1, RPW, 1, 4, 1, false, false, 1, YC8, true, T, AccInit>(nullptr, 0ll, wp, nullptr, y, ybs, 0, Cout, H, W, H, W, 0, tiles_x, tiles_y, slope,
                                                                        x8, x8bs, n8oct, W, W, ai);
}

template <typename T, typename TO>
__global__ __launch_bounds__(NTHREADS, 2)
void conv1x1_dual_kernel(const T* __restrict__ x, long long xbs, const T* __restrict__ wp, const float* __restrict__ bias, TO* __restrict__ y, long long ybs,
                         int Cin, int Cout, int H, int W, int tiles_x, int tiles_y, float slope, int xpitch, const DualOut<TO> d) {
  conv_body<T, 1, 2, 1, 4, 0, false, false, 0, true, false, TO, DualOut<TO>>(x, xbs, wp, bias, y, ybs, Cin, Cout, H, W, H, W, 0, tiles_x, tiles_y, slope,
                                                                            nullptr, 0ll, 0, xpitch, W, d);
}

inline int g_pair_th = 0;
inline int g_sk_grid = 48, g_sk_grid_narrow = 96, g_sk_grid_d4 = 16, g_small_grid = 256, g_rpw4_min = 256, g_ph_fit = 1, g_force_mtw = 0, g_force_sk = -1, g_ablate = 0;

struct Args {
  const void* x; long long xbs; const void* wp; const float* bias; void* y; long long ybs;
  int B, Cin, Cout, H, W, d, stride, ntaps; float slope; hipStream_t stream;
  int xpitch, ypitch;
  const void* gate_add = nullptr; long long gate_abs = 0; const void* gate_y = nullptr; long long gate_ybs = 0; float gate_slope = 0.f;
};

template <typename T, int MTW, int RPW, int S, int NOCTS, int D, bool GEN, bool ONE = false>
int launch_one(const Args& a, int slabs) {
  constexpr int TH = (4 / MTW) * RPW;
  constexpr bool PH = (D >= 2 && S == 1);
  const int Ho = (a.H - 1) / S + 1, Wo = (a.W - 1) / S + 1;
  const int tiles_x = cdiv(Wo, TW), tiles_y = PH ? cdiv(Ho, D * TH) * D : cdiv(Ho, TH);
  const int rows = PH ? TH + 2 : S * (TH - 1) + 2 * a.d + 1;
  size_t lds = (size_t)NOCTS * rows * (xw(S, margin_of(D)) + xw(S, margin_of(D)) / 16) * 16;
  if (lds < 4 * EPI_WAVE_BYTES) lds = 4 * EPI_WAVE_BYTES;
  UPF_REQUIRE(lds <= 160 * 1024, UPF_EUNSUPPORTED, "conv_forward: tile does not fit LDS (dilation %d, stride %d)", a.d, S);
  if (a.gate_y || a.gate_add) {
    if constexpr (S == 1 && D == 1) {
      static LdsOptIn gopt;
      auto gkern = &conv_gated_kernel<T, MTW, RPW, S, NOCTS, D, GEN, ONE>;
      gopt.ensure(reinterpret_cast<const void*>(gkern), lds);
      const ActGate<T> gate{(const T*)a.gate_add, a.gate_abs, (const T*)a.gate_y, a.gate_ybs, a.gate_slope};
      hipLaunchKernelGGL(gkern, dim3((unsigned)(a.B * tiles_x * tiles_y), slabs), dim3(NTHREADS), lds, a.stream, (const T*)a.x, a.xbs,
                         (const T*)a.wp, a.bias, (T*)a.y, a.ybs, a.Cin, a.Cout, a.H, a.W, Ho, Wo, g_ablate, tiles_x, tiles_y, a.slope,
                         a.xpitch, a.ypitch, gate);
      return check_launch("conv_forward_gated");
    } else {
      set_error("conv_forward_gated: 3x3, stride 1, dilation 1 only");
      return UPF_EUNSUPPORTED;
    }
  }
  static LdsOptIn opt;
  auto kern = &conv_kernel<T, MTW, RPW, S, NOCTS, D, GEN, ONE>;
  opt.ensure(reinterpret_cast<const void*>(kern), lds);
  hipLaunchKernelGGL(kern, dim3((unsigned)(a.B * tiles_x * tiles_y), slabs), dim3(NTHREADS), lds, a.stream, (const T*)a.x, a.xbs,
                     (const T*)a.wp, a.bias, (T*)a.y, a.ybs, a.Cin, a.Cout, a.H, a.W, Ho, Wo, D >= 0 ? g_ablate : a.d, tiles_x, tiles_y, a.slope,
                     (const T*)nullptr, 0ll, 0, a.xpitch, a.ypitch);
  return check_launch("conv_forward");
}

template <int MTW, int D> constexpr int wide_nocts() { return (MTW == 4 || D < 0 || (MTW == 2 && D == 16)) ? 2 : 4; }

inline int ph_tile_rows(int Ho, int d, int mtw) {
  const int rpp = cdiv(Ho, d);
  int best = 8; float best_cost = 1e30f;
  for (int th : {8, 6, 4}) {
    if (mtw == 1 && th == 6) continue;
    const float cost = (float)cdiv(rpp, th) * ((float)th + 2.5f);
    if (cost < best_cost - 1e-3f) { best_cost = cost; best = th; }
  }
  return best;
}

}
}
```

### upflow_pytorch_amd/model/pwc_modules.py

```python
import logging

import torch
import torch.nn as nn
import torch.nn.functional as tf

from .. import ops
from ..utils.tools import tools


def conv(in_planes, out_planes, kernel_size=3, stride=1, dilation=1, isReLU=True, if_IN=False, IN_affine=False, if_BN=False):
    layers = [nn.Conv2d(in_planes, out_planes, kernel_size=kernel_size, stride=stride, dilation=dilation,
                        padding=((kernel_size - 1) * dilation) // 2, bias=True)]
    if isReLU:
        layers.append(nn.LeakyReLU(0.1, inplace=True))
    if if_IN:
        layers.append(nn.InstanceNorm2d(out_planes, affine=IN_affine))
    elif if_BN:
        layers.append(nn.BatchNorm2d(out_planes, affine=IN_affine))
    return nn.Sequential(*layers)


def initialize_msra(modules):
    logging.info("Initializing MSRA")
    for layer in modules:
# ... 11 lines not shown
def _resize_flow(inputs, h, w, mode, if_rate):
    if mode != "bilinear":
        res = tf.interpolate(inputs, [h, w], mode=mode)
        if if_rate:
            _, _, h_, w_ = inputs.size()
            scale = torch.tensor([w / w_, h / h_], dtype=res.dtype, device=res.device).view(1, 2, 1, 1)
            res = res * scale
        return res
    return ops.flow_upsample(inputs, h, w, if_rate)


def upsample2d_flow_as(inputs, target_as, mode="bilinear", if_rate=False):
    _, _, h, w = target_as.size()
    return _resize_flow(inputs, h, w, mode, if_rate)


def upsample_flow(inputs, target_size=None, target_flow=None, mode="bilinear"):
    if target_size is not None:
        h, w = target_size
    elif target_flow is not None:
        _, _, h, w = target_flow.size()
    else:
        raise ValueError('wrong input')
    return _resize_flow(inputs, h, w, mode, True)


def rescale_flow(flow, div_flow, width_im, height_im, to_local=True):
    if to_local:
        u_scale = float(flow.size(3) / width_im / div_flow)
        v_scale = float(flow.size(2) / height_im / div_flow)
    else:
        u_scale = float(width_im * div_flow / flow.size(3))
        v_scale = float(height_im * div_flow / flow.size(2))
    scale = torch.tensor([u_scale, v_scale], dtype=flow.dtype, device=flow.device).view(1, 2, 1, 1)
    return flow * scale


class FeatureExtractor(nn.Module):

    def __init__(self, num_chs, if_end_relu=True, if_end_norm=False):
        super(FeatureExtractor, self).__init__()
        self.num_chs = num_chs
        self.convs = nn.ModuleList(
            nn.Sequential(conv(ci, co, stride=2), conv(co, co, isReLU=if_end_relu, if_IN=if_end_norm))
            for ci, co in zip(num_chs[:-1], num_chs[1:]))

    def forward(self, x, outs=None, pitched=False):
        pyramid = []
        cache = self.__dict__.setdefault('_fast_cache', {})
        hip = getattr(self, 'hip_convs', True)
        for i, stage in enumerate(self.convs):
            if (hip and FUSE_PAIRS[0] and not getattr(self, '_no_fuse_pairs', False) and len(stage[0]) == 2 and len(stage[1]) == 2
                    and ops.conv_pair_supported(x, stage[0][0], stage[1][0])):
                pc = cache.get(('pair', i)) or cache.setdefault(('pair', i), _PackedConvPair(stage[0], stage[1]))
                ho, wo = ops.conv3x3_out_hw(x.shape[2], x.shape[3], 2)
                y = outs[i] if (outs is not None and outs[i] is not None) else ops.empty_nchw((x.shape[0], stage[1][0].out_channels, ho, wo), x.dtype, x.device, pitched=pitched)
                x = pc(x, y)
                pyramid.append(x)
                continue
            x = fast_conv_seq(stage[0], x, cache, allow_hip=hip, pitched=pitched)
            x = fast_conv_seq(stage[1], x, cache, out=None if outs is None else outs[i], allow_hip=hip, pitched=pitched)
            pyramid.append(x)
        return pyramid[::-1]

    def out_shapes(self, H, W):
        shapes = []
        for c in self.num_chs[1:]:
            H, W = (H - 1) // 2 + 1, (W - 1) // 2 + 1
            shapes.append((c, H, W))
        return shapes


class WarpingLayer_no_div(nn.Module):

    def __init__(self, mask_mode='literal'):
        super(WarpingLayer_no_div, self).__init__()
        self.mask_mode = mask_mode

    def forward(self, x, flow, batch_shift=0):
        return ops.warp(x, flow, self.mask_mode, batch_shift)


class WarpingLayer(nn.Module):

    def __init__(self, mask_mode='literal'):
        super(WarpingLayer, self).__init__()
        self.mask_mode = mask_mode

    def forward(self, x, flow, height_im, width_im, div_flow):
        H, W = x.shape[2:]
        sx = (W - 1) / max(width_im - 1, 1) / div_flow
        sy = (H - 1) / max(height_im - 1, 1) / div_flow
        scale = torch.tensor([sx, sy], dtype=torch.float32, device=flow.device).view(1, 2, 1, 1)
        return ops.warp(x, flow.float() * scale, self.mask_mode)


class _PackedConv3x3(object):

    def __init__(self, seq):
        self.conv = seq[0]
        self.slope = 0.1 if any(isinstance(m, nn.LeakyReLU) for m in seq) else 0.0
        self.key = None
        self.packed = None
        self.bias = None
        self.key32 = None
        self.packed32 = None

    def _key(self):
        w, b = self.conv.weight, self.conv.bias
        return (w._version, w.dtype, w.device, w.data_ptr(), b._version, b.data_ptr())

    def get(self):
        key = self._key()
        if key != self.key:
            self.packed = ops.conv3x3_pack(self.conv.weight)
            self.bias = self.conv.bias.detach().float().contiguous()
            self.key = key
        return self.packed, self.bias

    def get32(self):
        key = self._key()
        if key != self.key32:
            self.packed32 = ops.conv3x3_pack(self.conv.weight.detach().float())
            self.bias = self.conv.bias.detach().float().contiguous()
            self.key32 = key
        return self.packed32, self.bias

    def invalidate(self):
        self.key = None
        self.key32 = None

    def __call__(self, x_view, y_view):
        c = self.conv
        if x_view.dtype != torch.float32 and x_view.shape[3] < 8:
            packed, bias = self.get32()
            ho, wo = ops.conv3x3_out_hw(x_view.shape[2], x_view.shape[3], c.stride[0])
            yf = torch.empty((x_view.shape[0], c.out_channels, ho, wo), dtype=torch.float32, device=x_view.device)
            ops.conv3x3_forward_raw(x_view.float(), packed, bias, yf, c.dilation[0], self.slope, c.stride[0], c.kernel_size[0])
            y_view.copy_(yf)
            return y_view
        packed, bias = self.get()
        return ops.conv3x3_forward_raw(x_view, packed, bias, y_view, c.dilation[0], self.slope, c.stride[0], c.kernel_size[0])


def packed_convs(net):
    out = []
    for m in net.modules():
        d = m.__dict__
        out += list(d.get('_fast_cache', {}).values())
        out += list(d.get('_packed', None) or [])
        for v in d.get('_packed8', {}).values():
            out += list(v[0]) if isinstance(v, tuple) else list(v)
    return [pc for pc in out if hasattr(pc, 'invalidate')]


def packed_operands(net):
    ts = []
    for pc in packed_convs(net):
        ts += [t for t in (getattr(pc, 'packed', None), getattr(pc, 'packed32', None), getattr(pc, 'bias', None)) if torch.is_tensor(t)]
        ts += [t for t in getattr(pc, 'extra_operands', lambda: [])() if torch.is_tensor(t)]
    return ts


_NO_NARROW = [False]


class _PackedConvC8(object):

    def __init__(self, seq, c8_channels=(), tail_channels=()):
        self.conv = seq[0]
        self.slope = 0.1 if any(isinstance(m, nn.LeakyReLU) for m in seq) else 0.0
        self.maps = (tuple(c8_channels), tuple(tail_channels))
        self.narrow = (not _NO_NARROW[0]) and ops.conv_c8_narrow_ok(self.conv.out_channels, self.conv.kernel_size[0], self.conv.dilation[0],
                                                                    self.conv.stride[0], len(self.maps[1]) > 0) and len(self.maps[0]) > 0
        self.key = None
        self.packed = None
        self.bias = None

    def get(self):
        w, b = self.conv.weight, self.conv.bias
        key = (w._version, w.dtype, w.device, w.data_ptr(), b._version, b.data_ptr())
        if key != self.key:
            self.packed = ops.conv_c8_pack16(w, self.maps[0]) if self.narrow else ops.conv_c8_pack(w, self.maps[0], self.maps[1])
            self.bias = self.conv.bias.detach().float().contiguous()
            self.key = key
        return self.packed, self.bias

    def invalidate(self):
        self.key = None

    def dual(self, x2, y_a, y_b):
        packed, bias = self.get()
        c = self.conv
        p = ops.nchw_pitch(x2)
        if (DUAL_1X1[0] and c.kernel_size == (1, 1) and not self.narrow and c.out_channels <= 32 and p is not None and p % 8 == 0
                and x2.data_ptr() % 16 == 0 and x2.stride(0) % 8 == 0):
            return ops.conv1x1_c8_dual_raw(x2, packed, bias, y_a, y_b, self.slope)
        self(None, x2, y_a)
        return self(None, x2, y_b)

    def __call__(self, x8, x2, y):
        packed, bias = self.get()
        if self.narrow:
            return ops.conv_c8_forward_narrow_raw(x8, packed, bias, y, self.slope)
        return ops.conv_c8_forward_raw(x8, x2, packed, bias, y, self.conv.dilation[0], self.slope, self.conv.kernel_size[0], self.conv.stride[0])


class _PackedTailC8(object):

    def __init__(self, seqs, m, J, kmap):
        self.m, self.J = int(m), sorted(int(j) for j in J)
        self.kmap = list(kmap)
        self.main = seqs[m][0]
        self.convs = [seqs[m][0]] + [seqs[j][0] for j in self.J]
        self.widths = [q[0].out_channels for q in seqs]
        self.slopes = {j: (0.1 if any(isinstance(m_, nn.LeakyReLU) for m_ in seqs[j]) else 0.0) for j in [m] + self.J}
        self.cmain = self.main.out_channels
        self.cin = self.main.in_channels
        self.offsets, off = {}, 0
        for j in self.J:
            self.offsets[j] = off
            off += (self.widths[j] + 3) // 4 * 4
        self.pp = off
        self.cout = self.cmain + off
        self.key = None
        self.packed = self.bias = None
        self.finish = {}

    @staticmethod
    def plan(widths):
        n = len(widths)
        cin = [None] * n
        acc = 0
        for k in range(n):
            cin[k] = acc
            acc += widths[k]
        best, best_score = None, 0
        for m in range(n - 2, -1, -1):
            if widths[m] % 8:
                continue
            mt = (widths[m] + 31) // 32
            free = 32 * (4 if mt >= 3 else mt) - widths[m]
            if mt > 4:
                continue
            J, used = [], 0
            for j in range(n - 1, m, -1):
                need = (widths[j] + 3) // 4 * 4
                if widths[j] > 16 or used + need > free or (j < n - 1 and widths[j] % 8):
                    break
                J.append(j); used += need
            if not J or any(widths[k] % 8 for k in range(m, n - 1)):
                continue
            score = len(J) * (cin[m] + 1000)
            if score > best_score:
                best, best_score = (m, sorted(J)), score
        return best

    def _key(self):
        k = []
        for c in self.convs:
            k += [c.weight._version, c.weight.dtype, c.weight.device, c.weight.data_ptr(), c.bias._version, c.bias.data_ptr()]
        return tuple(k)

    def get(self):
        key = self._key()
        if key != self.key:
            c0 = self.main
            rows, bias = [c0.weight.detach()], [c0.bias.detach().float()]
            self.finish = {}
            for j, c in zip(self.J, self.convs[1:]):
                front = sum(self.widths[self.m:j])
                w = c.weight.detach()
                assert w.shape[1] == front + self.cin
                pad = (c.out_channels + 3) // 4 * 4 - c.out_channels
                rows.append(w[:, front:])
                bias.append(c.bias.detach().float())
                if pad:
                    rows.append(w.new_zeros((pad, self.cin) + tuple(w.shape[2:])))
                    bias.append(bias[0].new_zeros(pad))
                self.finish[j] = ops.conv_c8_pack16(w[:, :front].contiguous(), list(range(front)))
            self.packed = ops.conv_c8_pack(torch.cat(rows, 0).contiguous(), self.kmap)
            self.bias = torch.cat(bias).contiguous()
            self.key = key
        return self.packed, self.bias

    def extra_operands(self):
        return list(self.finish.values())

    def invalidate(self):
        self.key = None

    def main_pass(self, x8, y8):
        packed, bias = self.get()
        B, _, H, W, _ = x8.shape
        part = torch.empty((B, self.pp // 4, H, W, 4), dtype=torch.float32, device=x8.device)
        ops.conv_c8_forward_split_raw(x8, packed, bias, y8, part, self.slopes[self.m])
        return part

    def finish_pass(self, j, x8_front, part, y):
        self.get()
        return ops.conv_c8_forward_narrow_init_raw(x8_front, self.finish[j], part, self.offsets[j], self.widths[j], y, self.slopes[j])


class _PackedConvPair(object):

    def __init__(self, seq_a, seq_b):
        self.convs = (seq_a[0], seq_b[0])
        self.strides = (seq_a[0].stride[0], seq_b[0].stride[0])
        self.slopes = tuple(0.1 if any(isinstance(m_, nn.LeakyReLU) for m_ in q) else 0.0 for q in (seq_a, seq_b))
        self.key = None
        self.packed = self.packed_b = self.bias = self.bias_b = None

    def _key(self):
        k = []
        for c in self.convs:
            k += [c.weight._version, c.weight.dtype, c.weight.device, c.weight.data_ptr(), c.bias._version, c.bias.data_ptr()]
        return tuple(k)

    def get(self):
        key = self._key()
        if key != self.key:
            a, b = self.convs
            self.packed, self.packed_b = ops.conv_pair_pack(a.weight, b.weight)
            self.bias, self.bias_b = a.bias.detach().float().contiguous(), b.bias.detach().float().contiguous()
            self.key = key
        return self.packed, self.bias, self.packed_b, self.bias_b

    def extra_operands(self):
        return [self.packed_b, self.bias_b]

    def invalidate(self):
        self.key = None

    def __call__(self, x, y):
        pa, ba, pb, bb = self.get()
        return ops.conv_pair_forward_raw(x, pa, ba, self.slopes[0], pb, bb, self.slopes[1], y, self.strides)


DUAL_1X1 = [True]
FUSE_PAIRS = [True]
MERGE_TAIL = [True]


def c8_level_ok(nb, H, W, dtype):
    return dtype in (torch.bfloat16, torch.float16) and nb * ((W + 31) // 32) * ((H + 7) // 8) >= 200


def fast_conv_seq(seq, x, cache, out=None, allow_hip=True, pitched=False):
    c = seq[0]
    k = c.kernel_size[0]
    if (allow_hip and _fast_conv_ok(x) and c.kernel_size in ((3, 3), (1, 1)) and c.stride[0] == c.stride[1] and c.groups == 1 and len(seq) <= 2
            and c.padding == (((k - 1) * c.dilation[0]) // 2,) * 2
            and (ops.conv3x3_supported(x, c.out_channels, c.dilation[0], c.stride[0], k)
                 or (x.shape[3] < 8 and 1 <= c.dilation[0] <= 16 and (c.stride[0] == 1 or (c.stride[0] == 2 and c.dilation[0] == 1 and k == 3))))):
        pc = cache.get(id(seq))
        if pc is None:
            pc = cache[id(seq)] = _PackedConv3x3(seq)
        ho, wo = ops.conv3x3_out_hw(x.shape[2], x.shape[3], c.stride[0])
        y = out if out is not None else ops.empty_nchw((x.shape[0], c.out_channels, ho, wo), x.dtype, x.device, pitched=pitched)
        return pc(x, y)
    if torch.is_grad_enabled() and x.is_cuda and x.dtype in (torch.bfloat16, torch.float16) and c.weight.dtype == torch.float32:
        y = train_conv_seq(seq, x)
    elif (FP32_TRAIN_CONV[0] == 'hip_x3' and torch.is_grad_enabled() and x.is_cuda and x.dtype == torch.float32
          and c.weight.dtype == torch.float32):
        y = train_conv_seq_x3(seq, x)
    else:
        y = seq(x if x.is_contiguous() else x.contiguous())
    if out is not None:
        out.copy_(y)
        return out
    return y


def train_conv_seq(seq, x):
    c = seq[0]
    k = c.kernel_size[0]
    slope = 0.0
    for m in list(seq)[1:]:
        if isinstance(m, nn.LeakyReLU):
            slope = float(m.negative_slope)
        else:
            return seq(x.float()).to(x.dtype)
    if (c.kernel_size in ((3, 3), (1, 1)) and c.stride[0] == c.stride[1] and c.groups == 1 and c.padding == (((k - 1) * c.dilation[0]) // 2,) * 2
            and ops.conv_train_supported(x, c.weight, c.stride[0], c.dilation[0])):
        return ops.conv_train(x, c.weight, c.bias, c.dilation[0], slope, c.stride[0])
    return seq(x.float()).to(x.dtype)


def train_conv_seq_x3(seq, x):
    c = seq[0]
    k = c.kernel_size[0]
    slope = 0.0
    for m in list(seq)[1:]:
        if not isinstance(m, nn.LeakyReLU):
            raise ops.UpflowHipError("fp32_train_conv='hip_x3': conv(...) Sequentials of Conv2d [+ LeakyReLU] only, got %s" % type(m).__name__)
        slope = float(m.negative_slope)
    if not (c.kernel_size in ((3, 3), (1, 1)) and c.stride[0] == c.stride[1] and c.groups == 1 and c.padding == (((k - 1) * c.dilation[0]) // 2,) * 2
            and c.dilation[0] == c.dilation[1] and c.padding_mode == 'zeros'):
        raise ops.UpflowHipError("fp32_train_conv='hip_x3': unsupported convolution %r" % (c,))
    return ops.conv_x3_train(x, c.weight, c.bias, c.dilation[0], slope, c.stride[0])


FP32_TRAIN_CONV = ['miopen']
FP32_TRAIN_CONV_MODES = ('miopen', 'hip_x3')


class fp32_train_conv_mode(object):
    def __init__(self, mode):
        if mode not in FP32_TRAIN_CONV_MODES:
            raise ValueError("fp32_train_conv must be one of %s, got %r" % (list(FP32_TRAIN_CONV_MODES), mode))
        self.mode = mode

    def __enter__(self):
        self.saved = FP32_TRAIN_CONV[0]
        FP32_TRAIN_CONV[0] = self.mode

    def __exit__(self, *exc):
        FP32_TRAIN_CONV[0] = self.saved


FP32_CONV = ['hip_x3']
FP32_CONV_NPROD = {'hip_x3': 3, 'hip_x3s': 11}


class fp32_conv_mode(object):
    def __init__(self, mode):
        if mode != 'miopen' and mode not in FP32_CONV_NPROD:
            raise ValueError("fp32_conv must be one of %s or 'miopen', got %r" % (sorted(FP32_CONV_NPROD), mode))
        self.mode = mode

    def __enter__(self):
        self.saved = (FP32_CONV[0], ops.CONV_X3_NPROD[0])
        FP32_CONV[0] = self.mode
        ops.CONV_X3_NPROD[0] = FP32_CONV_NPROD.get(self.mode, ops.CONV_X3_NPROD[0])

    def __exit__(self, *exc):
        FP32_CONV[0], ops.CONV_X3_NPROD[0] = self.saved


def _fast_conv_ok(t):
    if torch.is_grad_enabled() or not t.is_cuda:
        return False
    if t.dtype == torch.float32:
        return FP32_CONV[0] != 'miopen'
    return t.dtype in (torch.bfloat16, torch.float16)


class _DenseStack(tools.abstract_model):
    _NAMES = ('conv1', 'conv2', 'conv3', 'conv4', 'conv5')

    def _build(self, ch_in, f_channels, out_channel):
        n = ch_in
        for i, f in enumerate(f_channels):
            setattr(self, 'conv%d' % (i + 1), conv(n, f))
            n += f
        self.conv_last = conv(n, out_channel, isReLU=False)
        self._ch_in, self._f, self._n_total = ch_in, tuple(f_channels), n
        self._packed = None
        return n

    def alloc_buffer(self, B, H, W, dtype, device, tail=0):
        buf = torch.empty((B, self._n_total + tail, H, W), dtype=dtype, device=device)
        x0 = self._n_total - self._ch_in
        return buf, buf[:, x0:self._n_total]

    def forward_in_buffer(self, buf, out=None):
        if self._packed is None:
            self._packed = [_PackedConv3x3(getattr(self, n)) for n in self._NAMES] + [_PackedConv3x3(self.conv_last)]
        nt = self._n_total
        hi = nt - self._ch_in
        for pc, f in zip(self._packed[:5], self._f):
            pc(buf[:, hi:nt], buf[:, hi - f:hi])
            hi -= f
        x5 = buf[:, :nt]
        if out is None:
            out = torch.empty((buf.shape[0], self.conv_last[0].out_channels) + tuple(buf.shape[2:]), dtype=buf.dtype, device=buf.device)
        self._packed[5](x5, out)
        return x5, out

    def c8_ok(self):
        return self._ch_in % 8 == 0 and all(f % 8 == 0 for f in self._f)

    def c8_outputs_ok(self):
        return all(f % 8 == 0 for f in self._f)

    def forward_in_buffer_c8(self, buf8, out=None, in_map=None):
        key = None if in_map is None else tuple(in_map)
        cache = self.__dict__.setdefault('_packed8', {})
        if key not in cache:
            imap = list(range(self._ch_in)) if in_map is None else list(in_map)
            assert len(imap) % 8 == 0 and sorted(m for m in imap if m >= 0) == list(range(self._ch_in)), 'in_map must place every input channel once'
            packed, nconv = [], 0
            for name, f in zip(self._NAMES, self._f):
                packed.append(_PackedConvC8(getattr(self, name), list(range(nconv)) + [m + nconv if m >= 0 else -1 for m in imap]))
                nconv += f
            packed.append(_PackedConvC8(self.conv_last, list(range(nconv)) + [m + nconv if m >= 0 else -1 for m in imap]))
            widths = list(self._f) + [self.conv_last[0].out_channels]
            seqs = [getattr(self, n_) for n_ in self._NAMES] + [self.conv_last]
            plain = all(all(isinstance(x_, (nn.Conv2d, nn.LeakyReLU)) for x_ in q_) for q_ in seqs)
            pl = _PackedTailC8.plan(widths) if plain else None
            if pl is not None:
                nbefore = sum(self._f[:pl[0]])
                packed.append(_PackedTailC8(seqs, pl[0], pl[1], list(range(nbefore)) + [q + nbefore if q >= 0 else -1 for q in imap]))
            cache[key] = (packed, len(imap) // 8)
        packed, n_in = cache[key]
        nl = len(self._f)
        no = sum(self._f) // 8 + n_in
        starts, hi = [], sum(self._f) // 8
        for f in self._f:
            starts.append(hi)
            hi -= f // 8
        starts.append(hi)
        if out is None:
            out = torch.empty((buf8.shape[0], self.conv_last[0].out_channels) + tuple(buf8.shape[2:4]), dtype=buf8.dtype, device=buf8.device)
        tail = packed[nl + 1] if (len(packed) > nl + 1 and MERGE_TAIL[0] and not getattr(self, '_no_merge_tail', False)) else None
        part = None
        for k in range(nl + 1):
            y = buf8[:, starts[k + 1]:starts[k]] if k < nl else out
            if tail is not None and k == tail.m:
                part = tail.main_pass(buf8[:, starts[k]:no], y)
            elif tail is not None and k in tail.J:
                tail.finish_pass(k, buf8[:, starts[k]:starts[tail.m]], part, y)
            else:
                packed[k](buf8[:, starts[k]:no], None, y)
        return out

    def _train_convs(self):
        seqs = [getattr(self, n) for n in self._NAMES] + [self.conv_last]
        slope = None
        for i, q in enumerate(seqs):
            act = list(q)[1:]
            if i < 5:
                if len(act) != 1 or not isinstance(act[0], nn.LeakyReLU):
                    return None, None
                slope = float(act[0].negative_slope)
            elif act:
                return None, None
        return [q[0] for q in seqs], slope

    def train_in_buffer_ok(self, inputs):
        convs, _ = self._train_convs()
        return convs is not None and not getattr(self, '_no_train_buffer', False) and ops.dense_stack_train_supported(inputs, convs)

    def forward_train(self, inputs, flow_tail=None):
        convs, slope = self._train_convs()
        return ops.dense_stack_train(inputs, convs, slope, flow_tail)

    def forward(self, x):
        if _fast_conv_ok(x):
            buf, slot = self.alloc_buffer(x.shape[0], x.shape[2], x.shape[3], x.dtype, x.device)
            slot.copy_(x)
            return self.forward_in_buffer(buf)
        if self.train_in_buffer_ok([x]):
            buf, out = self.forward_train([x])
            return buf, out
        cache = self.__dict__.setdefault('_fast_cache', {})
        for name in self._NAMES:
            x = torch.cat([fast_conv_seq(getattr(self, name), x, cache), x], dim=1)
        return x, fast_conv_seq(self.conv_last, x, cache)


class FlowEstimatorDense_v2(_DenseStack):
    def __init__(self, ch_in, f_channels=(128, 128, 96, 64, 32), out_channel=2):
        super(FlowEstimatorDense_v2, self).__init__()
        self.n_channels = self._build(ch_in, f_channels, out_channel)


class FlowEstimatorDense(FlowEstimatorDense_v2):

    def __init__(self, ch_in):
        super(FlowEstimatorDense, self).__init__(ch_in)


class OpticalFlowEstimator(nn.Module):

    def __init__(self, ch_in):
        super(OpticalFlowEstimator, self).__init__()
        self.convs = nn.Sequential(conv(ch_in, 128), conv(128, 128), conv(128, 96), conv(96, 64), conv(64, 32))
        self.conv_last = conv(32, 2, isReLU=False)

    def forward(self, x):
        x_intm = self.convs(x)
        return x_intm, self.conv_last(x_intm)


class ContextNetwork_v2_(nn.Module):

    def __init__(self, ch_in, f_channels=(128, 128, 128, 96, 64, 32, 2)):
        super(ContextNetwork_v2_, self).__init__()
        dil = (1, 2, 4, 8, 16, 1, 1)
        chans = (ch_in,) + tuple(f_channels)
        self.convs = nn.Sequential(*[conv(chans[i], chans[i + 1], 3, 1, dil[i], isReLU=(i < 6)) for i in range(7)])

    def forward(self, x):
        cache = self.__dict__.setdefault('_fast_cache', {})
        for seq in self.convs:
            x = fast_conv_seq(seq, x, cache)
        return x

    def forward_c8(self, x, in_map=None):
        key = None if in_map is None else tuple(in_map)
        cache = self.__dict__.setdefault('_packed8', {})
        if key not in cache:
            chans = [s_[0].in_channels for s_ in self.convs]
            first = _PackedConvC8(self.convs[0], (), range(chans[0])) if in_map is None else _PackedConvC8(self.convs[0], list(in_map))
            cache[key] = [first] + [_PackedConvC8(self.convs[i], range(chans[i])) for i in range(1, 7)]
        B, H, W = x.shape[0], x.shape[2], x.shape[3]
        t = None
        for i, pc in enumerate(cache[key]):
            co = self.convs[i][0].out_channels
            y = ops.c8_empty(B, co, H, W, x.dtype, x.device) if i < 6 else torch.empty((B, co, H, W), dtype=x.dtype, device=x.device)
            if i == 0:
                pc(x if in_map is not None else None, None if in_map is not None else x, y)
            else:
                pc(t, None, y)
            t = y
        return t


class ContextNetwork(ContextNetwork_v2_):

    def __init__(self, ch_in):
        super(ContextNetwork, self).__init__(ch_in)
```

### upflow_pytorch_amd/ops.py

```python
import os

import torch
from torch.autograd import Function

from . import _lib
from ._operand_cache import OperandCache
from ._lib import MASK_NONE, MASK_LITERAL, MASK_ROBUST, UpflowHipError

_MASKS = {None: MASK_NONE, 'none': MASK_NONE, 'literal': MASK_LITERAL, 'robust': MASK_ROBUST,
          MASK_NONE: MASK_NONE, MASK_LITERAL: MASK_LITERAL, MASK_ROBUST: MASK_ROBUST}


def _f32(t):
    return t if t.dtype == torch.float32 else t.float()


PITCH_MULTIPLE = 8


def empty_nchw(shape, dtype, device, pitched=True):
    W = shape[-1]
    if pitched and dtype in (torch.bfloat16, torch.float16) and W >= 8 and W % PITCH_MULTIPLE:
        Wp = (W + PITCH_MULTIPLE - 1) // PITCH_MULTIPLE * PITCH_MULTIPLE
        return torch.empty(tuple(shape[:-1]) + (Wp,), dtype=dtype, device=device)[..., :W]
# ... 449 lines not shown
            raise UpflowHipError('sgu_blend: flow_init [B,2,Hf,Wf], x_out [B,3,h,w] expected, got %s / %s'
                                 % (tuple(flow_init.shape), tuple(x_out.shape)))
        dev = _lib.check_gpu(flow_init, x_out)
        flow_up = torch.empty_like(flow_init)
        inter_flow = torch.empty_like(flow_init) if want_inter else None
        inter_mask = torch.empty((B, 1, Hf, Wf), dtype=torch.float32, device=x_out.device) if want_inter else None
        nws = _lib.lib().upf_sgu_blend_forward_workspace_bytes(B, h, w, Hf, Wf)
        ws = torch.empty((nws,), dtype=torch.uint8, device=x_out.device) if nws else None
        with torch.cuda.device(dev):
            _lib.call('upf_sgu_blend_forward', _lib.ptr(flow_init), _lib.ptr(x_out), _lib.ptr(flow_up),
                      _lib.ptr(inter_flow), _lib.ptr(inter_mask), _lib.ptr(ws), B, h, w, Hf, Wf, _lib.dtype_code(x_out),
                      _lib.stream_ptr(dev))
        ctx.save_for_backward(flow_init, x_out)
        ctx.set_materialize_grads(False)
        if want_inter:
            ctx.mark_non_differentiable(inter_flow, inter_mask)
            return flow_up, inter_flow, inter_mask
        return flow_up, None, None

    @staticmethod
    def backward(ctx, g_up, _gi, _gm):
        if g_up is None:
            return None, None, None
        flow_init, x_out = ctx.saved_tensors
        B, _, h, w = x_out.shape
        _, _, Hf, Wf = flow_init.shape
        g_up = _f32(g_up).contiguous()
        dev = _lib.check_gpu(flow_init, x_out, g_up)
        g_init = torch.empty_like(flow_init)
        g_xo = torch.empty((B, 3, h, w), dtype=torch.float32, device=x_out.device)
        ws = torch.empty((_lib.lib().upf_sgu_blend_backward_workspace_bytes(B, h, w, Hf, Wf),), dtype=torch.uint8, device=x_out.device)
        with torch.cuda.device(dev):
            _lib.call('upf_sgu_blend_backward', _lib.ptr(flow_init), _lib.ptr(x_out), _lib.ptr(g_up), _lib.ptr(g_init),
                      _lib.ptr(g_xo), _lib.ptr(ws), B, h, w, Hf, Wf, _lib.dtype_code(x_out), _lib.stream_ptr(dev))
        return g_init, g_xo.to(x_out.dtype), None


def sgu_blend_flow16(flow_init, x_out, flow16):
    flow_init = _f32(flow_init).contiguous()
    x_out = x_out.contiguous()
    B, _, H, W = x_out.shape
    if tuple(flow_init.shape) != (B, 2, H, W) or x_out.shape[1] != 3 or x_out.dtype not in (torch.bfloat16, torch.float16) or flow16.dtype != x_out.dtype:
        raise UpflowHipError('sgu_blend_flow16: flow_init [B,2,H,W] fp32, x_out [B,3,H,W] 16-bit and a 16-bit flow slot of its type expected')
    c8 = flow16.dim() == 5
    if c8:
        if tuple(flow16.shape) != (B, 1, H, W, 8) or not _c8_view_ok(flow16):
            raise UpflowHipError('sgu_blend_flow16: the octet slot must be [B,1,H,W,8]')
    elif tuple(flow16.shape) != (B, 2, H, W) or not _is_channel_slice(flow16):
        raise UpflowHipError('sgu_blend_flow16: the NCHW slot must be a [B,2,H,W] channel slice of a contiguous buffer')
    dev = _lib.check_gpu(flow_init, x_out)
    flow_up = torch.empty_like(flow_init)
    with torch.cuda.device(dev):
        _lib.call('upf_sgu_blend_forward_flow16', _lib.ptr(flow_init), _lib.ptr(x_out), _lib.ptr(flow_up), _lib.ptr(flow16), flow16.stride(0), int(c8),
                  B, H, W, _lib.dtype_code(x_out), _lib.stream_ptr(dev))
    return flow_up


def sgu_blend(flow_init, x_out, output_level_flow=None, want_inter=True):
    base = output_level_flow if output_level_flow is not None else flow_init
    flow_up, inter_flow, inter_mask = SguBlendFunction.apply(base, x_out, want_inter)
    return base, flow_up, inter_flow, inter_mask


class NormalizeFunction(Function):
    @staticmethod
    def forward(ctx, x):
        x = x.contiguous()
        B, C, H, W = x.shape
        dev = _lib.check_gpu(x)
        y = torch.empty_like(x)
        rstd = torch.empty((B * C,), dtype=torch.float32, device=x.device)
        ws = torch.empty((_lib.lib().upf_normalize_workspace_bytes(B * C, H * W),), dtype=torch.uint8, device=x.device)
        with torch.cuda.device(dev):
            _lib.call('upf_normalize_forward', _lib.ptr(x), _lib.ptr(y), _lib.ptr(None), _lib.ptr(rstd), _lib.ptr(ws), B * C, H * W,
                      _lib.dtype_code(x), _lib.stream_ptr(dev))
        ctx.save_for_backward(y, rstd)
        return y

    @staticmethod
    def backward(ctx, gy):
        y, rstd = ctx.saved_tensors
        B, C, H, W = y.shape
        gy = gy.to(y.dtype).contiguous()
        dev = _lib.check_gpu(y, gy)
        gx = torch.empty_like(y)
        with torch.cuda.device(dev):
            _lib.call('upf_normalize_backward', _lib.ptr(y), _lib.ptr(gy), _lib.ptr(rstd), _lib.ptr(gx), B * C, H * W,
                      _lib.dtype_code(y), _lib.stream_ptr(dev))
        return gx


def normalize(x):
    return NormalizeFunction.apply(x)


def normalize_pair(a, b):
    return normalize(a), normalize(b)


def occ_check(flow_f, flow_b, alpha1=0.1, alpha2=0.5):
    ff = _f32(flow_f.detach()).contiguous()
    fb = _f32(flow_b.detach()).contiguous()
    B, _, H, W = ff.shape
    dev = _lib.check_gpu(ff, fb)
    o1 = torch.empty((B, 1, H, W), dtype=torch.float32, device=ff.device)
    o2 = torch.empty_like(o1)
    with torch.cuda.device(dev):
        _lib.call('upf_occ_check', _lib.ptr(ff), _lib.ptr(fb), _lib.ptr(o1), _lib.ptr(o2), B, H, W,
                  float(alpha1), float(alpha2), _lib.stream_ptr(dev))
    return o1, o2


CONV_X3_NPROD = [3]


def conv3x3_pack(weight):
    w = weight.detach().contiguous()
    Cout, Cin, kh, kw = w.shape
    if kh != kw or kh not in (1, 3):
        raise UpflowHipError('conv pack: 3x3 or 1x1 kernels only')
    dev = _lib.check_gpu(w)
    if w.dtype == torch.float32:
        packed = torch.empty((_lib.lib().upf_conv_x3_packed_bytes(Cin, Cout, kh) // 2,), dtype=torch.float16, device=w.device)
        with torch.cuda.device(dev):
            _lib.call('upf_conv_x3_pack_weights', _lib.ptr(w), _lib.ptr(packed), Cin, Cout, kh, _lib.stream_ptr(dev))
        return packed
    nbytes = _lib.lib().upf_conv_packed_bytes(Cin, Cout, kh)
    packed = torch.empty((nbytes // 2,), dtype=w.dtype, device=w.device)
    with torch.cuda.device(dev):
        _lib.call('upf_conv_pack_weights', _lib.ptr(w), _lib.ptr(packed), Cin, Cout, kh, _lib.dtype_code(w), _lib.stream_ptr(dev))
    return packed


def conv3x3_supported(x_view, Cout, dilation, stride=1, kernel_size=3):
    return (x_view.is_cuda and x_view.dtype in (torch.bfloat16, torch.float16, torch.float32) and kernel_size in (1, 3)
            and 1 <= dilation <= 16 and (stride == 1 or (stride == 2 and dilation == 1 and kernel_size == 3))
            and (x_view.shape[3] >= 8 or x_view.dtype == torch.float32))


def mfma_f16_denorm_probe(device):
    out = torch.zeros(1, dtype=torch.float32, device=device)
    with torch.cuda.device(device):
        _lib.call('upf_mfma_f16_denorm_probe', _lib.ptr(out), _lib.stream_ptr(device))
    return float(out.item()) == 2.0 ** -6


def conv_set_option(name, value):
    prev = _lib.lib().upf_conv_set_option(name.encode(), int(value))
    if prev == -2 ** 31:
        raise UpflowHipError('unknown convolution option %r' % name)
    return prev


def conv3x3_out_hw(H, W, stride=1):
    return (H - 1) // stride + 1, (W - 1) // stride + 1


def conv3x3_forward_raw(x_view, packed, bias32, y_view, dilation=1, leaky_slope=0.0, stride=1, kernel_size=3):
    B, Cin, H, W = x_view.shape
    Cout = y_view.shape[1]
    Ho, Wo = conv3x3_out_hw(H, W, stride)
    if tuple(y_view.shape) != (B, Cout, Ho, Wo):
        raise UpflowHipError('conv: output must be [%d,%d,%d,%d], got %s' % (B, Cout, Ho, Wo, tuple(y_view.shape)))
    xp, yp = _pitch_or_raise(x_view, 'conv: x'), _out_pitch_or_raise(y_view, 'conv: y')
    dev = x_view.device
    if x_view.dtype == torch.float32:
        if xp != W or yp != Wo:
            raise UpflowHipError('conv (fp32, split precision): contiguous rows expected (no row pitch)')
        if y_view.dtype != torch.float32 or packed.dtype != torch.float16:
            raise UpflowHipError('conv (fp32, split precision): fp32 output and weights packed from fp32 expected')
        with torch.cuda.device(dev):
            _lib.call('upf_conv_x3_forward', _lib.ptr(x_view), x_view.stride(0), _lib.ptr(packed), _lib.ptr(bias32),
                      _lib.ptr(y_view), y_view.stride(0), B, Cin, Cout, H, W, int(kernel_size), int(dilation), int(stride),
                      float(leaky_slope), int(CONV_X3_NPROD[0]), _lib.stream_ptr(dev))
        return y_view
    if y_view.dtype != x_view.dtype:
        if kernel_size != 1 or stride != 1 or Cout > 32 or y_view.dtype not in (torch.bfloat16, torch.float16):
            raise UpflowHipError('conv: an output type other than the operands\' is offered for 1x1 convolutions with Cout <= 32 only')
        with torch.cuda.device(dev):
            _lib.call('upf_conv1x1_forward_mixed', _lib.ptr(x_view), x_view.stride(0), xp, _lib.ptr(packed), _lib.ptr(bias32), _lib.ptr(y_view),
                      y_view.stride(0), yp, 0, B, Cin, Cout, H, W, float(leaky_slope), _lib.dtype_code(x_view), _lib.dtype_code(y_view), _lib.stream_ptr(dev))
        return y_view
    with torch.cuda.device(dev):
        _lib.call('upf_conv_forward_pitched', _lib.ptr(x_view), x_view.stride(0), xp, _lib.ptr(packed), _lib.ptr(bias32),
                  _lib.ptr(y_view), y_view.stride(0), yp, B, Cin, Cout, H, W, int(kernel_size), int(dilation), int(stride),
                  float(leaky_slope), _lib.dtype_code(x_view), _lib.stream_ptr(dev))
    return y_view


def conv3x3_forward_gated_raw(x_view, packed, bias32, y_view, add, act, mask_slope):
    B, Cin, H, W = x_view.shape
    Cout = y_view.shape[1]
    if tuple(y_view.shape) != (B, Cout, H, W):
        raise UpflowHipError('conv (gated): output must be [%d,%d,%d,%d], got %s' % (B, Cout, H, W, tuple(y_view.shape)))
    xp, yp = _pitch_or_raise(x_view, 'conv (gated): x'), _out_pitch_or_raise(y_view, 'conv (gated): y')
    if add is None and act is None:
        raise UpflowHipError('conv (gated): neither add nor act given')
    for t, name in ((add, 'add'), (act, 'act')):
        if t is None:
            continue
        if tuple(t.shape) != (B, Cout, H, W) or t.dtype != y_view.dtype or _pitch_or_raise(t, 'conv (gated): ' + name) != yp:
            raise UpflowHipError('conv (gated): %s must be a [%d,%d,%d,%d] channel slice of the output\'s dtype and row pitch' % (name, B, Cout, H, W))
    if x_view.dtype not in (torch.bfloat16, torch.float16) or y_view.dtype != x_view.dtype or not x_view.is_cuda:
        raise UpflowHipError('conv (gated): 16-bit GPU operands of one type expected (there is no CPU fallback)')
    dev = x_view.device
    with torch.cuda.device(dev):
        _lib.call('upf_conv_forward_gated', _lib.ptr(x_view), x_view.stride(0), xp, _lib.ptr(packed), _lib.ptr(bias32), _lib.ptr(y_view),
                  y_view.stride(0), yp, _lib.ptr(add), (add.stride(0) if add is not None else 0), _lib.ptr(act), (act.stride(0) if act is not None else 0),
                  float(mask_slope), B, Cin, Cout, H, W, _lib.dtype_code(x_view), _lib.stream_ptr(dev))
    return y_view


def c8_empty(B, C, H, W, dtype, device):
    return torch.empty((B, (C + 7) // 8, H, W, 8), dtype=dtype, device=device)


def to_c8(x):
    B, C, H, W = x.shape
    n = (C + 7) // 8
    if n * 8 != C:
        x = torch.cat([x, x.new_zeros(B, n * 8 - C, H, W)], 1)
    return x.view(B, n, 8, H, W).permute(0, 1, 3, 4, 2).contiguous()


def from_c8(x8, C=None):
    B, n, H, W, _ = x8.shape
    x = x8.permute(0, 1, 4, 2, 3).reshape(B, n * 8, H, W)
    return x if C is None else x[:, :C]


def conv_c8_k(n8_oct, C2):
    return _lib.lib().upf_conv_c8_k(int(n8_oct), int(C2))


def conv_c8_pack(weight, c8_channels=(), tail_channels=()):
    w = weight.detach().contiguous()
    Cout, Cin, kh, kw = w.shape
    if kh != kw or kh not in (1, 3):
        raise UpflowHipError('conv pack: 3x3 or 1x1 kernels only')
    c8_channels, tail_channels = list(c8_channels), list(tail_channels)
    if len(c8_channels) % 8:
        raise UpflowHipError('conv_c8_pack: the C8 slice must be whole octets')
    K = conv_c8_k(len(c8_channels) // 8, len(tail_channels))
    p8 = (len(c8_channels) + 31) // 32 * 32 if c8_channels else 0
    kmap = [-1] * K
    kmap[:len(c8_channels)] = c8_channels
    kmap[p8:p8 + len(tail_channels)] = tail_channels
    dev = _lib.check_gpu(w)
    kmap_t = torch.tensor(kmap, dtype=torch.int32, device=w.device)
    nbytes = _lib.lib().upf_conv_packed_bytes_k(K, Cout, kh)
    packed = torch.empty((nbytes // 2,), dtype=w.dtype, device=w.device)
    with torch.cuda.device(dev):
        _lib.call('upf_conv_pack_weights_kmap', _lib.ptr(w), _lib.ptr(packed), Cin, Cout, kh, _lib.ptr(kmap_t), K,
                  _lib.dtype_code(w), _lib.stream_ptr(dev))
    return packed


def conv_c8_narrow_ok(Cout, kernel_size, dilation, stride, has_tail):
    return Cout <= 16 and kernel_size == 3 and dilation == 1 and stride == 1 and not has_tail


def conv_c8_pack16(weight, c8_channels):
    w = weight.detach().contiguous()
    Cout, Cin, kh, kw = w.shape
    c8_channels = list(c8_channels)
    if kh != 3 or kw != 3 or len(c8_channels) % 8 or not c8_channels:
        raise UpflowHipError('conv_c8_pack16: 3x3 kernels, a C8 slice of whole octets')
    K = (len(c8_channels) + 31) // 32 * 32
    kmap = c8_channels + [-1] * (K - len(c8_channels))
    dev = _lib.check_gpu(w)
    kmap_t = torch.tensor(kmap, dtype=torch.int32, device=w.device)
    packed = torch.empty((_lib.lib().upf_conv_packed_bytes_k16(K, Cout) // 2,), dtype=w.dtype, device=w.device)
    with torch.cuda.device(dev):
        _lib.call('upf_conv_pack_weights_kmap16', _lib.ptr(w), _lib.ptr(packed), Cin, Cout, _lib.ptr(kmap_t), K,
                  _lib.dtype_code(w), _lib.stream_ptr(dev))
    return packed


def conv_c8_forward_narrow_raw(x8, packed16, bias32, y, leaky_slope=0.0):
    B, n, H, W, _ = x8.shape
    Cout = bias32.shape[0]
    y_is_c8 = y.dim() == 5
    if not _c8_view_ok(x8):
        raise UpflowHipError('conv_c8_narrow: x8 must be an octet slice of a contiguous C8 buffer')
    if y_is_c8:
        if not _c8_view_ok(y) or tuple(y.shape) != (B, (Cout + 7) // 8, H, W, 8):
            raise UpflowHipError('conv_c8_narrow: C8 output must be [%d,%d,%d,%d,8], got %s' % (B, (Cout + 7) // 8, H, W, tuple(y.shape)))
    elif tuple(y.shape) != (B, Cout, H, W) or y.stride()[1:] != (H * W, W, 1):
        raise UpflowHipError('conv_c8_narrow: NCHW output must be a [%d,%d,%d,%d] channel slice' % (B, Cout, H, W))
    dev = x8.device
    if not (x8.is_cuda and y.is_cuda) or x8.dtype != y.dtype:
        raise UpflowHipError('conv_c8_narrow: GPU tensors of one dtype expected (there is no CPU fallback)')
    with torch.cuda.device(dev):
        _lib.call('upf_conv_forward_c8_narrow', _lib.ptr(x8), x8.stride(0), n, _lib.ptr(packed16), _lib.ptr(bias32), _lib.ptr(y), y.stride(0),
                  int(y_is_c8), B, Cout, H, W, float(leaky_slope), _lib.dtype_code(x8), _lib.stream_ptr(dev))
    return y


def _partial_ok(partial, B, H, W):
    return (partial.dtype == torch.float32 and partial.dim() == 5 and partial.shape[0] == B and tuple(partial.shape[2:]) == (H, W, 4)
            and partial.stride()[1:] == (H * W * 4, W * 4, 4, 1))


def conv_c8_forward_split_raw(x8, packed, bias32, y8, partial, leaky_slope=0.0):
    B, n, H, W, _ = x8.shape
    Cout = bias32.shape[0]
    if not _c8_view_ok(x8) or not _c8_view_ok(y8) or tuple(y8.shape[0:1] + y8.shape[2:]) != (B, H, W, 8):
        raise UpflowHipError('conv_c8_split: x8 / y8 must be octet slices of contiguous C8 buffers of one size')
    cmain = 8 * y8.shape[1]
    if not _partial_ok(partial, B, H, W) or 4 * partial.shape[1] < (Cout - cmain + 3) // 4 * 4:
        raise UpflowHipError('conv_c8_split: partial must be fp32 [B,Q,H,W,4] (planes of channel quads, 4 Q >= the partial channels), got %s' % (tuple(partial.shape),))
    dev = x8.device
    if not (x8.is_cuda and y8.is_cuda and partial.is_cuda) or x8.dtype != y8.dtype:
        raise UpflowHipError('conv_c8_split: GPU tensors of one 16-bit dtype expected (there is no CPU fallback)')
    with torch.cuda.device(dev):
        _lib.call('upf_conv_forward_c8_split', _lib.ptr(x8), x8.stride(0), n, _lib.ptr(packed), _lib.ptr(bias32), _lib.ptr(y8), y8.stride(0), cmain,
                  _lib.ptr(partial), partial.stride(0), 4 * partial.shape[1], B, Cout, H, W, float(leaky_slope), _lib.dtype_code(x8), _lib.stream_ptr(dev))
    return y8


def conv_c8_forward_narrow_init_raw(x8, packed16, partial, offset, Cout, y, leaky_slope=0.0):
    B, n, H, W, _ = x8.shape
    y_is_c8 = y.dim() == 5
    if not _c8_view_ok(x8):
        raise UpflowHipError('conv_c8_narrow_init: x8 must be an octet slice of a contiguous C8 buffer')
    if y_is_c8:
        if not _c8_view_ok(y) or tuple(y.shape) != (B, (Cout + 7) // 8, H, W, 8):
            raise UpflowHipError('conv_c8_narrow_init: C8 output must be [%d,%d,%d,%d,8], got %s' % (B, (Cout + 7) // 8, H, W, tuple(y.shape)))
    elif tuple(y.shape) != (B, Cout, H, W) or y.stride()[1:] != (H * W, W, 1):
        raise UpflowHipError('conv_c8_narrow_init: NCHW output must be a [%d,%d,%d,%d] channel slice' % (B, Cout, H, W))
    if not _partial_ok(partial, B, H, W):
        raise UpflowHipError('conv_c8_narrow_init: partial must be fp32 [B,Q,H,W,4] (planes of channel quads)')
    dev = x8.device
    if not (x8.is_cuda and y.is_cuda and partial.is_cuda) or x8.dtype != y.dtype:
        raise UpflowHipError('conv_c8_narrow_init: GPU tensors of one 16-bit dtype expected (there is no CPU fallback)')
    with torch.cuda.device(dev):
        _lib.call('upf_conv_forward_c8_narrow_init', _lib.ptr(x8), x8.stride(0), n, _lib.ptr(packed16), _lib.ptr(partial), partial.stride(0), 4 * partial.shape[1],
                  int(offset), _lib.ptr(y), y.stride(0), int(y_is_c8), B, int(Cout), H, W, float(leaky_slope), _lib.dtype_code(x8), _lib.stream_ptr(dev))
    return y


def conv_pair_pack(w_a, w_b):
    C1, Cin, C2 = w_a.shape[0], w_a.shape[1], w_b.shape[0]
    if tuple(w_a.shape[2:]) != (3, 3) or tuple(w_b.shape[2:]) != (3, 3) or w_b.shape[1] != C1 or Cin > 16 or C1 not in (16, 32) or C2 > 32:
        raise UpflowHipError('conv_pair_pack: 3x3 layers with Cin <= 16, C1 = 16 | 32, C2 <= 32 expected, got %s / %s' % (tuple(w_a.shape), tuple(w_b.shape)))
    dev, dt = w_a.device, w_a.dtype
    lane = torch.arange(64, device=dev)
    co, kg, j = (lane % 32).view(1, 64, 1), (lane // 32).view(1, 64, 1), torch.arange(8, device=dev).view(1, 1, 8)
    wa = torch.zeros((32, 16, 12), dtype=dt, device=dev)
    wa[:C1, :Cin, :9] = w_a.detach().reshape(C1, Cin, 9)
    if Cin <= 4:
        s = torch.arange(3, device=dev).view(3, 1, 1)
        pa = wa[co.expand(3, 64, 8), (j % 4).expand(3, 64, 8), (4 * s + 2 * kg + j // 4).expand(3, 64, 8)]
    elif Cin <= 8:
        s = torch.arange(5, device=dev).view(5, 1, 1)
        pa = wa[co.expand(5, 64, 8), j.expand(5, 64, 8), (2 * s + kg).expand(5, 64, 8)]
    else:
        s = torch.arange(9, device=dev).view(9, 1, 1)
        pa = wa[co.expand(9, 64, 8), (8 * kg + j).expand(9, 64, 8), s.expand(9, 64, 8)]
    ksb = C1 // 16
    wbz = torch.zeros((32, C1, 9), dtype=dt, device=dev)
    wbz[:C2] = w_b.detach().reshape(C2, C1, 9)
    tap = torch.arange(9, device=dev).view(9, 1, 1, 1)
    ks = torch.arange(ksb, device=dev).view(1, ksb, 1, 1)
    shp = (9, ksb, 64, 8)
    pb = wbz[co.view(1, 1, 64, 1).expand(shp), (16 * ks + 8 * kg.view(1, 1, 64, 1) + j.view(1, 1, 1, 8)).expand(shp), tap.expand(shp)]
    return pa.contiguous(), pb.contiguous()


def conv_pair_forward_raw(x, packed_a, bias_a, slope_a, packed_b, bias_b, slope_b, y, strides=(1, 2)):
    B, Cin, H, W = x.shape
    C1, C2 = bias_a.shape[0], bias_b.shape[0]
    Ho, Wo = conv3x3_out_hw(H, W, 2)
    xp = _pitch_or_raise(x, 'conv_pair: x')
    y_is_c8 = y.dim() == 5
    if y_is_c8:
        if not _c8_view_ok(y) or tuple(y.shape) != (B, (C2 + 7) // 8, Ho, Wo, 8):
            raise UpflowHipError('conv_pair: C8 output must be [%d,%d,%d,%d,8], got %s' % (B, (C2 + 7) // 8, Ho, Wo, tuple(y.shape)))
        yp = 0
    else:
        if tuple(y.shape) != (B, C2, Ho, Wo):
            raise UpflowHipError('conv_pair: NCHW output must be [%d,%d,%d,%d], got %s' % (B, C2, Ho, Wo, tuple(y.shape)))
        yp = _out_pitch_or_raise(y, 'conv_pair: y')
    dev = x.device
    if not (x.is_cuda and y.is_cuda) or x.dtype != y.dtype or x.dtype not in (torch.bfloat16, torch.float16) or packed_a.dtype != x.dtype:
        raise UpflowHipError('conv_pair: GPU tensors of one 16-bit dtype expected (there is no CPU fallback)')
    with torch.cuda.device(dev):
        _lib.call('upf_conv_pair_forward', _lib.ptr(x), x.stride(0), xp, Cin, _lib.ptr(packed_a), _lib.ptr(bias_a), float(slope_a), C1, int(strides[0]),
                  _lib.ptr(packed_b), _lib.ptr(bias_b), float(slope_b), C2, int(strides[1]), _lib.ptr(y), y.stride(0), yp, int(y_is_c8), B, H, W,
                  _lib.dtype_code(x), _lib.stream_ptr(dev))
    return y


def conv_pair_supported(x, conv_a, conv_b):
    if torch.is_grad_enabled() or not x.is_cuda or x.dtype not in (torch.bfloat16, torch.float16) or x.dim() != 4:
        return False
    if (conv_a.stride, conv_b.stride) not in (((1, 1), (2, 2)), ((2, 2), (1, 1))):
        return False
    for c in (conv_a, conv_b):
        if c.kernel_size != (3, 3) or c.dilation != (1, 1) or c.padding != (1, 1) or c.groups != 1 or c.bias is None or c.weight.dtype != x.dtype:
            return False
    p = nchw_pitch(x)
    return (conv_a.in_channels <= 16 and conv_a.out_channels in (16, 32) and conv_b.in_channels == conv_a.out_channels and conv_b.out_channels <= 32
            and p is not None and p % 2 == 0 and x.data_ptr() % 4 == 0 and x.stride(0) % 2 == 0 and x.shape[3] >= 8)


def _c8_view_ok(t):
    B, n, H, W, e = t.shape
    return e == 8 and t.stride()[1:] == (H * W * 8, W * 8, 8, 1)


def conv_c8_supported(H, W, dtype, Cout, dilation, kernel_size, has_c8_in, has_tail, y_is_c8):
    if dtype not in (torch.bfloat16, torch.float16) or (W % 8 and has_tail):
        return False
    if kernel_size == 1:
        return (not has_c8_in) and has_tail and y_is_c8 and Cout <= 32
    if dilation == 1:
        return has_c8_in or (has_tail and y_is_c8)
    return dilation in (2, 4, 8, 16) and has_c8_in and not has_tail and y_is_c8


def conv_c8_forward_raw(x8, x2, packed, bias32, y, dilation=1, leaky_slope=0.0, kernel_size=3, stride=1):
    ref = x8 if x8 is not None else x2
    B, H, W = ref.shape[0], ref.shape[2], ref.shape[3]
    Cout = bias32.shape[0]
    y_is_c8 = y.dim() == 5
    Ho, Wo = conv3x3_out_hw(H, W, stride)
    if x8 is not None and not _c8_view_ok(x8):
        raise UpflowHipError('conv_c8: x8 must be an octet slice of a contiguous C8 buffer')
    x2p = _pitch_or_raise(x2, 'conv_c8: x2') if x2 is not None else 0
    yp = 0
    if y_is_c8:
        if not _c8_view_ok(y) or tuple(y.shape) != (B, (Cout + 7) // 8, Ho, Wo, 8):
            raise UpflowHipError('conv_c8: C8 output must be [%d,%d,%d,%d,8], got %s' % (B, (Cout + 7) // 8, Ho, Wo, tuple(y.shape)))
    else:
        if tuple(y.shape) != (B, Cout, Ho, Wo):
            raise UpflowHipError('conv_c8: NCHW output must be a [%d,%d,%d,%d] channel slice' % (B, Cout, Ho, Wo))
        yp = _out_pitch_or_raise(y, 'conv_c8: y')
    dev = ref.device
    if y.dtype != ref.dtype:
        if not (x8 is None and x2 is not None and kernel_size == 1 and stride == 1 and y_is_c8 and Cout <= 32 and y.dtype in (torch.bfloat16, torch.float16)):
            raise UpflowHipError('conv_c8: an output type other than the operands\' is offered for the 1x1 NCHW -> C8 projection (Cout <= 32) only')
        with torch.cuda.device(dev):
            _lib.call('upf_conv1x1_forward_mixed', _lib.ptr(x2), x2.stride(0), x2p, _lib.ptr(packed), _lib.ptr(bias32), _lib.ptr(y), y.stride(0), 0, 1,
                      B, x2.shape[1], Cout, H, W, float(leaky_slope), _lib.dtype_code(x2), _lib.dtype_code(y), _lib.stream_ptr(dev))
        return y
    with torch.cuda.device(dev):
        _lib.call('upf_conv_forward_c8_pitched', _lib.ptr(x8), x8.stride(0) if x8 is not None else 0, x8.shape[1] if x8 is not None else 0,
                  _lib.ptr(x2), x2.stride(0) if x2 is not None else 0, x2p, x2.shape[1] if x2 is not None else 0,
                  _lib.ptr(packed), _lib.ptr(bias32), _lib.ptr(y), y.stride(0), yp, int(y_is_c8), B, Cout, H, W, int(kernel_size),
                  int(dilation), int(stride), float(leaky_slope), _lib.dtype_code(ref), _lib.stream_ptr(dev))
    return y


def conv1x1_c8_dual_raw(x2, packed, bias32, y_a, y_b, leaky_slope=0.0):
    B, Cin, H, W = x2.shape
    Cout = bias32.shape[0]
    for y in (y_a, y_b):
        if y.dim() != 5 or not _c8_view_ok(y) or tuple(y.shape) != (B, (Cout + 7) // 8, H, W, 8) or y.dtype != y_a.dtype:
            raise UpflowHipError('conv1x1_c8_dual: outputs must be octet slices [%d,%d,%d,%d,8] of one type' % (B, (Cout + 7) // 8, H, W))
    xp = _pitch_or_raise(x2, 'conv1x1_c8_dual: x')
    dev = x2.device
    if not (x2.is_cuda and y_a.is_cuda and y_b.is_cuda) or x2.dtype not in (torch.bfloat16, torch.float16) or y_a.dtype not in (torch.bfloat16, torch.float16):
        raise UpflowHipError('conv1x1_c8_dual: 16-bit GPU tensors expected (there is no CPU fallback)')
    with torch.cuda.device(dev):
        _lib.call('upf_conv1x1_forward_c8_dual', _lib.ptr(x2), x2.stride(0), xp, _lib.ptr(packed), _lib.ptr(bias32), _lib.ptr(y_a), y_a.stride(0),
                  _lib.ptr(y_b), y_b.stride(0), B, Cin, Cout, H, W, float(leaky_slope), _lib.dtype_code(x2), _lib.dtype_code(y_a), _lib.stream_ptr(dev))
    return y_a


def conv_c8_set_option(name, value):
    prev = _lib.lib().upf_conv_c8_set_option(name.encode(), int(value))
    if prev == -2 ** 31:
        raise UpflowHipError('unknown C8 convolution option %r' % name)
    return prev


def conv_x3_set_option(name, value):
    prev = _lib.lib().upf_conv_x3_set_option(name.encode(), int(value))
    if prev == -2 ** 31:
        raise UpflowHipError('unknown split-precision convolution option %r' % name)
    return prev


class CensusFunction(Function):
    @staticmethod
    def forward(ctx, gray1, gray2, max_distance):
        gray1 = _f32(gray1).contiguous()
        gray2 = _f32(gray2).contiguous()
        if gray1.dim() != 4 or gray1.shape[1] != 1 or gray1.shape != gray2.shape:
            raise UpflowHipError('census: two [B,1,H,W] grey images expected, got %s / %s' % (tuple(gray1.shape), tuple(gray2.shape)))
        B, _, H, W = gray1.shape
        dev = _lib.check_gpu(gray1, gray2)
        dist = torch.empty_like(gray1)
        _lib.launch(dev, 'upf_census_forward', _lib.ptr(gray1), _lib.ptr(gray2), _lib.ptr(dist), B, H, W, int(max_distance))
        ctx.save_for_backward(gray1, gray2)
        ctx.max_distance = int(max_distance)
        return dist

    @staticmethod
    def backward(ctx, g):
        gray1, gray2 = ctx.saved_tensors
        B, _, H, W = gray1.shape
        g = _f32(g).contiguous()
        dev = _lib.check_gpu(gray1, gray2, g)
        g1 = torch.empty_like(gray1) if ctx.needs_input_grad[0] else None
        g2 = torch.empty_like(gray2) if ctx.needs_input_grad[1] else None
        if g1 is None and g2 is None:
            return None, None, None
        _lib.launch(dev, 'upf_census_backward', _lib.ptr(gray1), _lib.ptr(gray2), _lib.ptr(g), _lib.ptr(g1), _lib.ptr(g2), B, H, W,
                    ctx.max_distance)
        return g1, g2, None


def census_distance(gray1, gray2, max_distance=3):
    return CensusFunction.apply(gray1, gray2, max_distance)


def _lv_check(name, *tensors):
    for t in tensors:
        if t is None:
            continue
        if t.dtype != torch.float32:
            raise UpflowHipError('%s: float32 operands expected, got %s' % (name, t.dtype))
    return _lib.check_gpu(*tensors)


def _partial_sums(dev, name, n, k, tensors, *scalars):
    partials = torch.empty((_lib.lib().upf_loss_partials(n), k), dtype=torch.float32, device=dev)
    _lib.launch(dev, name, *[_lib.ptr(t) for t in tensors], _lib.ptr(partials), *scalars)
    return partials.sum(0)


def _grad_scalar(g):
    return _f32(g).reshape(1).contiguous()


class BoundaryWarpFunction(Function):
    @staticmethod
    def forward(ctx, image, flow, start):
        image = _f32(image).contiguous()
        flow = _f32(flow).contiguous()
        B, C, Hi, Wi = image.shape
        if flow.dim() != 4 or flow.shape[0] != B or flow.shape[1] != 2:
            raise UpflowHipError('boundary_warp: image [B,C,Hi,Wi] and flow [B,2,h,w] expected, got %s / %s' % (tuple(image.shape), tuple(flow.shape)))
        start = _f32(start).to(flow.device).reshape(-1)
        if start.numel() == 2:
            start = start.repeat(B)
        if start.numel() != 2 * B:
            raise UpflowHipError('boundary_warp: start must hold (x, y) per batch item, got %d values for B=%d' % (start.numel(), B))
        start = start.contiguous()
        h, w = flow.shape[2:]
        dev = _lib.check_gpu(image, flow, start)
        out = torch.empty((B, C, h, w), dtype=torch.float32, device=flow.device)
        _lib.launch(dev, 'upf_boundary_warp_forward', _lib.ptr(image), _lib.ptr(flow), _lib.ptr(start), _lib.ptr(out), B, C, Hi, Wi, h, w)
        ctx.save_for_backward(image, flow, start)
        return out

    @staticmethod
    def backward(ctx, g):
        image, flow, start = ctx.saved_tensors
        if ctx.needs_input_grad[0]:
            raise UpflowHipError('boundary_warp: the gradient wrt the image is not implemented (frames are data)')
        B, C, Hi, Wi = image.shape
        h, w = flow.shape[2:]
        g = _f32(g).contiguous()
        dev = _lib.check_gpu(image, flow, g)
        gflow = torch.empty_like(flow)
        _lib.launch(dev, 'upf_boundary_warp_backward', _lib.ptr(image), _lib.ptr(flow), _lib.ptr(start), _lib.ptr(g), _lib.ptr(gflow),
                    B, C, Hi, Wi, h, w)
        return None, gflow, None


def boundary_warp(image, flow, start):
    return BoundaryWarpFunction.apply(image, flow, start)


POINTWISE_KINDS = {'charbonnier': 0, 'L1': 1}


class PointwiseLossFunction(Function):

    @staticmethod
    def forward(ctx, x, y, occ, kind, q, eps):
        name = 'robust_loss' if kind == 'abs_robust' else 'pointwise_loss'
        if x.shape != y.shape or x.dim() != 4:
            raise UpflowHipError('%s: two [B,C,H,W] tensors expected, got %s / %s' % (name, tuple(x.shape), tuple(y.shape)))
        B, C, H, W = x.shape
        if occ is not None and tuple(occ.shape) != (B, 1, H, W):
            raise UpflowHipError('%s: occlusion mask must be [B,1,H,W], got %s' % (name, tuple(occ.shape)))
        dev = _lv_check(name, x, y, occ)
        ctx.name = name
        ctx.scalars = (B, C, H * W, float(eps) if kind == 'abs_robust' else POINTWISE_KINDS[kind], float(q))
        sums = _partial_sums(dev, 'upf_%s_forward' % name, B * H * W, 2, (x, y, occ), *ctx.scalars)
        ctx.save_for_backward(x, y, occ)
        s_loss, s_occ = sums.unbind(0)
        ctx.mark_non_differentiable(s_occ)
        ctx.set_materialize_grads(False)
        return s_loss, s_occ

    @staticmethod
    def backward(ctx, g, _g_occ):
        if g is None:
            return (None,) * 6
        if ctx.needs_input_grad[2]:
            raise UpflowHipError('%s: the occlusion weights are treated as constants (hard masks); a mask that '
                                 'requires grad would silently get a zero gradient' % ctx.name)
        x, y, occ = ctx.saved_tensors
        gx = torch.empty_like(x) if ctx.needs_input_grad[0] else None
        gy = torch.empty_like(y) if ctx.needs_input_grad[1] else None
        if gx is None and gy is None:
            return (None,) * 6
        coef = _grad_scalar(g)
        dev = _lib.check_gpu(x, y, coef)
        _lib.launch(dev, 'upf_%s_backward' % ctx.name, _lib.ptr(x), _lib.ptr(y), _lib.ptr(occ), _lib.ptr(coef), _lib.ptr(gx), _lib.ptr(gy),
                    *ctx.scalars)
        return gx, gy, None, None, None, None


def robust_loss_sums(x, y, occ=None, q=0.4, eps=0.01):
    occ = None if occ is None else _f32(occ).contiguous()
    return PointwiseLossFunction.apply(_f32(x).contiguous(), _f32(y).contiguous(), occ, 'abs_robust', q, eps)


def grey(image):
    image = _f32(image).contiguous()
    B, C, H, W = image.shape
    if C != 3:
        raise UpflowHipError('grey: an RGB image [B,3,H,W] expected, got %s' % (tuple(image.shape),))
    dev = _lib.check_gpu(image)
    out = torch.empty((B, 1, H, W), dtype=torch.float32, device=image.device)
    _lib.launch(dev, 'upf_grey_forward', _lib.ptr(image), _lib.ptr(out), B, H * W)
    return out


class MsdUpupFunction(Function):

    @staticmethod
    def forward(ctx, y, occ, weight, q, eps, *levels):
        y = _f32(y).contiguous()
        B, C, H, W = y.shape
# ... 1174 lines not shown
```

Baseline: 1939 frame-pairs/s.

## Fuse last two tail 3x3 convs into one LDS-resident pair kernel

Adds a kernel that computes two consecutive 3x3 convolutions (layer A into LDS with a halo, then a narrow layer B) in one launch. It is used by default at the SGU tail and is available but off for the context network. The aim is to remove the global round-trip of layer A's output and one kernel launch. In exchange, each tile recomputes layer A on a halo, and the kernel is limited to specific channel shapes with a tile-count threshold.

```diff
diff --git a/include/upflow_hip.h b/include/upflow_hip.h
--- a/include/upflow_hip.h
+++ b/include/upflow_hip.h
@@ -163,6 +163,12 @@
                           const void* wb_packed, const float* bias_b , float slope_b, int C2, int stride_b,
                           void* y, long long y_batch_stride, int y_row_pitch, int y_is_c8,
                           int B, int H, int W, int dtype, void* stream);
+
+int upf_conv_tail_pair_forward_c8(const void* x8, long long x8_batch_stride, int n8_oct,
+                                  const void* wa_packed, const float* bias_a , int Cout_a, float slope_a, void* ya8, long long ya_batch_stride,
+                                  const void* wb_packed16, const float* bias_b , int Cout_b, int shared_oct, float slope_b,
+                                  const float* partial, long long partial_batch_stride, int partial_pitch, int partial_offset_a, int partial_offset_b,
+                                  void* y, long long y_batch_stride, int y_row_pitch, int B, int H, int W, int dtype, void* stream);
 
 int upf_conv_pack_weights_f32(const float* w , void* w_packed, int Cin, int Cout, int kernel_size,
                               int dtype, int dgrad, void* stream);
diff --git a/upflow_pytorch_amd/_build.py b/upflow_pytorch_amd/_build.py
--- a/upflow_pytorch_amd/_build.py
+++ b/upflow_pytorch_amd/_build.py
@@ -13,6 +13,7 @@
     ('conv3x3.hip', []),
     ('conv_c8.hip', []),
     ('conv_pair.hip', []),
+    ('conv_tail.hip', []),
     ('conv_x3.hip', []),
     ('conv_x3_bwd.hip', []),
     ('conv_wgrad.hip', []),
diff --git a/upflow_pytorch_amd/_lib.py b/upflow_pytorch_amd/_lib.py
--- a/upflow_pytorch_amd/_lib.py
+++ b/upflow_pytorch_amd/_lib.py
@@ -69,6 +69,7 @@
     'upf_conv_forward_c8_split': [_vp, _ll, _i, _vp, _vp, _vp, _ll, _i, _vp, _ll, _i, _i, _i, _i, _i, _f, _i, _vp],
     'upf_conv_forward_c8_narrow_init': [_vp, _ll, _i, _vp, _vp, _ll, _i, _i, _vp, _ll, _i, _i, _i, _i, _i, _f, _i, _vp],
     'upf_conv_pair_forward': [_vp, _ll, _i, _i, _vp, _vp, _f, _i, _i, _vp, _vp, _f, _i, _i, _vp, _ll, _i, _i, _i, _i, _i, _i, _vp],
+    'upf_conv_tail_pair_forward_c8': [_vp, _ll, _i, _vp, _vp, _i, _f, _vp, _ll, _vp, _vp, _i, _i, _f, _vp, _ll, _i, _i, _i, _vp, _ll, _i, _i, _i, _i, _i, _vp],
     'upf_leaky_backward': [_vp, _vp, _vp, _ll, _f, _i, _vp],
     'upf_conv_wgrad': [_vp, _ll, _vp, _ll, _vp, _vp, _i, _i, _i, _i, _i, _i, _i, _i, _vp],
     'upf_conv_bias_grad': [_vp, _ll, _vp, _vp, _i, _i, _i, _i, _vp],
diff --git a/upflow_pytorch_amd/csrc/conv_c8.hip b/upflow_pytorch_amd/csrc/conv_c8.hip
--- a/upflow_pytorch_amd/csrc/conv_c8.hip
+++ b/upflow_pytorch_amd/csrc/conv_c8.hip
@@ -65,7 +65,6 @@
   return check_launch("conv_forward_c8");
 }
 
-inline int g_c8_rpw4 = 1;
 inline int g_c8_narrow_tall = 0;
 
 template <typename T, int XL, bool YC8>
diff --git a/upflow_pytorch_amd/csrc/conv_kernel.hpp b/upflow_pytorch_amd/csrc/conv_kernel.hpp
--- a/upflow_pytorch_amd/csrc/conv_kernel.hpp
+++ b/upflow_pytorch_amd/csrc/conv_kernel.hpp
@@ -647,6 +647,7 @@
 }
 
 inline int g_pair_th = 0;
+inline int g_c8_rpw4 = 1;
 inline int g_sk_grid = 48, g_sk_grid_narrow = 96, g_sk_grid_d4 = 16, g_small_grid = 256, g_rpw4_min = 256, g_ph_fit = 1, g_force_mtw = 0, g_force_sk = -1, g_ablate = 0;
 
 struct Args {
diff --git a/upflow_pytorch_amd/csrc/conv_tail.hip b/upflow_pytorch_amd/csrc/conv_tail.hip
--- /dev/null
+++ b/upflow_pytorch_amd/csrc/conv_tail.hip
@@ -0,0 +1,343 @@
+#include "conv_kernel.hpp"
+
+namespace upf {
+namespace conv {
+
+template <int TH> struct TailGeom {
+  static constexpr int RIN = TH + 4, CIN = TW + 4;
+  static constexpr int RA = TH + 2, CA = TW + 2;
+  static constexpr int NPIX = RA * CA;
+  static constexpr int PIN = (RIN * CIN + 63) / 64 * 64;
+  static constexpr int PA = (NPIX + 15) / 16 * 16;
+};
+template <int TH, int NIN> constexpr int tail_ein() { return (NIN * TailGeom<TH>::PIN + 63) & ~63; }
+template <int TH, int NIN, int NAO> constexpr size_t tail_lds_bytes() { return (size_t)(tail_ein<TH, NIN>() + NAO * TailGeom<TH>::PA) * 16; }
+
+struct TailArgs {
+  const void* x8; long long x8bs;
+  const void* wa; const float* ba; int couta; float slope_a;
+  void* ya8; long long yabs;
+  const void* wb; const float* bb; int coutb; float slope_b;
+  const float* part; long long pbs; int ppitch, coffa, coffb;
+  void* y; long long ybs; int ypitch;
+  int H, W, tiles_x, tiles_y;
+};
+
+template <typename T, int TH, bool A32, int NIN, int NAO, int KB, bool INIT, int CHA>
+__global__ __launch_bounds__(NTHREADS, 2)
+void conv_tail_pair_kernel(const TailArgs a) {
+  using G = TailGeom<TH>;
+  static_assert(TH % 4 == 0 && NAO + KB <= 4 && KB <= NIN && (!A32 || (NIN % CHA == 0 && NAO == 4)), "tail pair: geometry");
+  constexpr int RPW = TH / 4;
+  constexpr int EIN = tail_ein<TH, NIN>();
+  extern __shared__ __attribute__((aligned(16))) uint4 xs[];
+  uint4* const xin = xs;
+  uint4* const xa = xs + EIN;
+
+  const int bid = xcd_remap(blockIdx.x, gridDim.x);
+  const int tx = bid % a.tiles_x, ty = (bid / a.tiles_x) % a.tiles_y, n = bid / (a.tiles_x * a.tiles_y);
+  const int x0 = tx * TW, y0 = ty * TH;
+  const int tid = threadIdx.x, lane = tid & 63;
+  const int wave = __builtin_amdgcn_readfirstlane(tid >> 6);
+  const int H = a.H, W = a.W, HW = H * W;
+
+  constexpr int NP = EIN / 64, NSL = (NP + 3) / 4;
+  auto stage = [&]() {
+    asm volatile("" ::: "memory");
+    __amdgpu_buffer_rsrc_t x8r = __builtin_amdgcn_make_buffer_rsrc(const_cast<T*>((const T*)a.x8 + (size_t)n * a.x8bs), 0, (uint32_t)NIN * (uint32_t)HW * 16u, 0x00020000);
+#pragma unroll
+    for (int j = 0; j < NSL; ++j) {
+      const int piece = j * 4 + wave;
+      if (piece < NP) {
+        const int p = piece * 64 + lane;
+        const int oct = p / G::PIN, rem = p - oct * G::PIN, r = rem / G::CIN, c = rem - r * G::CIN;
+        const int gy = y0 - 2 + r, gx = x0 - 2 + c;
+        const bool in = oct < NIN && r < G::RIN && gy >= 0 && gy < H && gx >= 0 && gx < W;
+        const uint32_t off = in ? (uint32_t)((oct * HW + gy * W + gx) * 16) : 0x80000000u;
+        __builtin_amdgcn_raw_ptr_buffer_load_lds(x8r, (__attribute__((address_space(3))) void*)(xin + piece * 64), 16, (int)off, 0, 0, 0);
+      }
+    }
+    asm volatile("" ::: "memory");
+  };
+
+  __amdgpu_buffer_rsrc_t pr;
+  if constexpr (INIT)
+    pr = __builtin_amdgcn_make_buffer_rsrc(const_cast<float*>(a.part + (size_t)n * a.pbs), 0, (uint32_t)HW * (uint32_t)a.ppitch * 4u, 0x00020000);
+  __amdgpu_buffer_rsrc_t yar = __builtin_amdgcn_make_buffer_rsrc((T*)a.ya8 + (size_t)n * a.yabs, 0, a.ya8 ? (uint32_t)NAO * (uint32_t)HW * 16u : 0u, 0x00020000);
+
+  if constexpr (A32) {
+    constexpr int NBLK = (G::NPIX + 31) / 32, NBW = (NBLK + 3) / 4, KS = CHA / 2, NCH = NIN / CHA;
+    const int px = lane & 31, kg = lane >> 5;
+    __amdgpu_buffer_rsrc_t wr = __builtin_amdgcn_make_buffer_rsrc(const_cast<T*>((const T*)a.wa), 0, 9u * 32u * (uint32_t)(NIN * 8) * 2u, 0x00020000);
+    __amdgpu_buffer_rsrc_t br = __builtin_amdgcn_make_buffer_rsrc(const_cast<float*>(a.ba), 0, (uint32_t)a.couta * 4u, 0x00020000);
+    constexpr int NKS = NIN / 2;
+    auto wload = [&](int cc, int tap, int ks) {
+      const uint32_t idx = (uint32_t)((cc * KS + ks) * 9 + tap);
+      return __builtin_bit_cast(uint4, __builtin_amdgcn_raw_buffer_load_b128(wr, (cc * KS + ks < NKS) ? idx * 1024u + (uint32_t)lane * 16u : 0x80000000u, 0, 0));
+    };
+    uint4 wa[9][KS];
+#pragma unroll
+    for (int tap = 0; tap < 9; ++tap)
+#pragma unroll
+      for (int ks = 0; ks < KS; ++ks) wa[tap][ks] = wload(0, tap, ks);
+    f32x16 acc[NBW];
+#pragma unroll
+    for (int e = 0; e < 16; ++e) {
+      const float bv = __builtin_bit_cast(float, __builtin_amdgcn_raw_buffer_load_b32(br, (uint32_t)((e & 3) + 8 * (e >> 2) + 4 * kg) * 4u, 0, 0));
+#pragma unroll
+      for (int i = 0; i < NBW; ++i) acc[i][e] = bv;
+    }
+    stage();
+    int base[NBW];
+#pragma unroll
+    for (int i = 0; i < NBW; ++i) {
+      const int q = (wave + 4 * i) * 32 + px, qc = q < G::NPIX ? q : G::NPIX - 1;
+      const int r = qc / G::CA;
+      base[i] = r * G::CIN + (qc - r * G::CA);
+    }
+    asm volatile("s_waitcnt vmcnt(0)" ::: "memory");
+    __syncthreads();
+    __builtin_amdgcn_s_setprio(2);
+#pragma unroll
+    for (int cc = 0; cc < NCH; ++cc)
+#pragma unroll
+      for (int tap = 0; tap < 9; ++tap) {
+        const int ky = tap / 3, kx = tap - 3 * ky;
+#pragma unroll
+        for (int ks = 0; ks < KS; ++ks) {
+#pragma unroll
+          for (int i = 0; i < NBW; ++i)
+            if (wave + 4 * i < NBLK)
+              acc[i] = Mma32<T>::mma(wa[tap][ks], xin[(cc * CHA + 2 * ks + kg) * G::PIN + base[i] + ky * G::CIN + kx], acc[i]);
+          if (cc + 1 < NCH) wa[tap][ks] = wload(cc + 1, tap, ks);
+        }
+      }
+    __builtin_amdgcn_s_setprio(0);
+#pragma unroll
+    for (int i = 0; i < NBW; ++i) {
+      const int q = (wave + 4 * i) * 32 + px;
+      if (wave + 4 * i < NBLK && q < G::NPIX) {
+        const int r = q / G::CA, c = q - r * G::CA, gy = y0 - 1 + r, gx = x0 - 1 + c;
+        const bool in = gy >= 0 && gy < H && gx >= 0 && gx < W;
+        const bool own = in && r >= 1 && r <= TH && c >= 1 && c <= TW;
+        const uint32_t goff = own ? (uint32_t)(gy * W + gx) * 16u + (uint32_t)kg * 8u : 0x80000000u;
+#pragma unroll
+        for (int g = 0; g < NAO; ++g) {
+          float v[4];
+#pragma unroll
+          for (int k = 0; k < 4; ++k) { v[k] = acc[i][4 * g + k]; v[k] = fmaxf(v[k], v[k] * a.slope_a); }
+          u32x2 o;
+          o.x = in ? pack2<T>(v[0], v[1]) : 0u; o.y = in ? pack2<T>(v[2], v[3]) : 0u;
+          *reinterpret_cast<u32x2*>(reinterpret_cast<unsigned char*>(xa + g * G::PA + q) + kg * 8) = o;
+          if (a.ya8) __builtin_amdgcn_raw_buffer_store_b64(o, yar, goff + (uint32_t)g * (uint32_t)HW * 16u, 0, 0);
+        }
+      }
+    }
+  } else {
+    constexpr int NBLK = (G::NPIX + 15) / 16, NBW = (NBLK + 3) / 4;
+    static_assert(NIN <= 4, "tail pair: layer A on the 16-channel instruction reads one 32-channel chunk");
+    const int p16 = lane & 15, ko = lane >> 4;
+    __amdgpu_buffer_rsrc_t wr = __builtin_amdgcn_make_buffer_rsrc(const_cast<T*>((const T*)a.wa), 0, 9u * 1024u, 0x00020000);
+    uint4 wa[9];
+#pragma unroll
+    for (int tap = 0; tap < 9; ++tap) wa[tap] = __builtin_bit_cast(uint4, __builtin_amdgcn_raw_buffer_load_b128(wr, (uint32_t)tap * 1024u + (uint32_t)lane * 16u, 0, 0));
+    f32x4 acc[NBW];
+    int base[NBW];
+#pragma unroll
+    for (int i = 0; i < NBW; ++i) {
+      const int q = (wave + 4 * i) * 16 + p16, qc = q < G::NPIX ? q : G::NPIX - 1;
+      const int r = qc / G::CA, c = qc - r * G::CA;
+      base[i] = r * G::CIN + c;
+      if constexpr (INIT) {
+        const int gy = y0 - 1 + r, gx = x0 - 1 + c;
+        const bool in = gy >= 0 && gy < H && gx >= 0 && gx < W && 4 * ko < a.couta;
+        const uint32_t off = in ? (uint32_t)(((a.coffa >> 2) + ko) * HW + gy * W + gx) * 16u : 0x80000000u;
+        acc[i] = __builtin_bit_cast(f32x4, __builtin_amdgcn_raw_buffer_load_b128(pr, off, 0, 0));
+      }
+    }
+    if constexpr (!INIT) {
+      __amdgpu_buffer_rsrc_t br = __builtin_amdgcn_make_buffer_rsrc(const_cast<float*>(a.ba), 0, (uint32_t)a.couta * 4u, 0x00020000);
+#pragma unroll
+      for (int k = 0; k < 4; ++k) {
+        const float bv = __builtin_bit_cast(float, __builtin_amdgcn_raw_buffer_load_b32(br, (uint32_t)(4 * ko + k) * 4u, 0, 0));
+#pragma unroll
+        for (int i = 0; i < NBW; ++i) acc[i][k] = bv;
+      }
+    }
+    stage();
+    const bool kin = ko < NIN;
+    const uint4* const src = xin + (kin ? ko : 0) * G::PIN;
+    asm volatile("s_waitcnt vmcnt(0)" ::: "memory");
+    __syncthreads();
+    __builtin_amdgcn_s_setprio(2);
+#pragma unroll
+    for (int tap = 0; tap < 9; ++tap) {
+      const int ky = tap / 3, kx = tap - 3 * ky;
+#pragma unroll
+      for (int i = 0; i < NBW; ++i)
+        if (wave + 4 * i < NBLK) {
+          uint4 b = src[base[i] + ky * G::CIN + kx];
+          if (!kin) b = make_uint4(0u, 0u, 0u, 0u);
+          acc[i] = Mma16<T>::mma(wa[tap], b, acc[i]);
+        }
+    }
+    __builtin_amdgcn_s_setprio(0);
+#pragma unroll
+    for (int i = 0; i < NBW; ++i) {
+      const int q = (wave + 4 * i) * 16 + p16;
+      if (wave + 4 * i < NBLK && q < G::NPIX && (ko >> 1) < NAO) {
+        const int r = q / G::CA, c = q - r * G::CA, gy = y0 - 1 + r, gx = x0 - 1 + c;
+        const bool in = gy >= 0 && gy < H && gx >= 0 && gx < W;
+        const bool own = in && r >= 1 && r <= TH && c >= 1 && c <= TW;
+        float v[4];
+#pragma unroll
+        for (int k = 0; k < 4; ++k) { v[k] = acc[i][k]; v[k] = fmaxf(v[k], v[k] * a.slope_a); }
+        u32x2 o;
+        o.x = in ? pack2<T>(v[0], v[1]) : 0u; o.y = in ? pack2<T>(v[2], v[3]) : 0u;
+        *reinterpret_cast<u32x2*>(reinterpret_cast<unsigned char*>(xa + (ko >> 1) * G::PA + q) + (ko & 1) * 8) = o;
+        const uint32_t goff = own ? (uint32_t)((ko >> 1) * HW + gy * W + gx) * 16u + (uint32_t)(ko & 1) * 8u : 0x80000000u;
+        __builtin_amdgcn_raw_buffer_store_b64(o, yar, goff, 0, 0);
+      }
+    }
+  }
+  __syncthreads();
+
+  {
+    const int p16 = lane & 15, ko = lane >> 4;
+    const bool from_a = ko < NAO, live = ko < NAO + KB;
+    const uint4* const src = from_a ? xa + ko * G::PA : xin + (live ? ko - NAO : 0) * G::PIN + G::CIN + 1;
+    const int pitch = from_a ? G::CA : G::CIN;
+    __amdgpu_buffer_rsrc_t wr = __builtin_amdgcn_make_buffer_rsrc(const_cast<T*>((const T*)a.wb), 0, 9u * 1024u, 0x00020000);
+    uint4 wb[9];
+#pragma unroll
+    for (int tap = 0; tap < 9; ++tap) wb[tap] = __builtin_bit_cast(uint4, __builtin_amdgcn_raw_buffer_load_b128(wr, (uint32_t)tap * 1024u + (uint32_t)lane * 16u, 0, 0));
+    f32x4 acc16[RPW][2];
+    if constexpr (INIT) {
+#pragma unroll
+      for (int r = 0; r < RPW; ++r)
+#pragma unroll
+        for (int h = 0; h < 2; ++h) {
+          const int gx = x0 + p16 + 16 * h, gy = y0 + RPW * wave + r;
+          const uint32_t off = (gx < W && gy < H && 4 * ko < a.coutb) ? (uint32_t)(((a.coffb >> 2) + ko) * HW + gy * W + gx) * 16u : 0x80000000u;
+          acc16[r][h] = __builtin_bit_cast(f32x4, __builtin_amdgcn_raw_buffer_load_b128(pr, off, 0, 0));
+        }
+    } else {
+      __amdgpu_buffer_rsrc_t br = __builtin_amdgcn_make_buffer_rsrc(const_cast<float*>(a.bb), 0, (uint32_t)a.coutb * 4u, 0x00020000);
+#pragma unroll
+      for (int k = 0; k < 4; ++k) {
+        const float bv = __builtin_bit_cast(float, __builtin_amdgcn_raw_buffer_load_b32(br, (uint32_t)(4 * ko + k) * 4u, 0, 0));
+#pragma unroll
+        for (int r = 0; r < RPW; ++r) { acc16[r][0][k] = bv; acc16[r][1][k] = bv; }
+      }
+    }
+    constexpr int NR = RPW + 2;
+    uint4 bq[2][6];
+    auto bload = [&](int sr, uint4 (&b)[6]) {
+#pragma unroll
+      for (int h = 0; h < 2; ++h)
+#pragma unroll
+        for (int kx = 0; kx < 3; ++kx) {
+          uint4 v = src[(RPW * wave + sr) * pitch + p16 + 16 * h + kx];
+          if (!live) v = make_uint4(0u, 0u, 0u, 0u);
+          b[h * 3 + kx] = v;
+        }
+    };
+    __builtin_amdgcn_s_setprio(2);
+    bload(0, bq[0]);
+#pragma unroll
+    for (int sr = 0; sr < NR; ++sr) {
+      if (sr + 1 < NR) bload(sr + 1, bq[(sr + 1) & 1]);
+#pragma unroll
+      for (int kx = 0; kx < 3; ++kx)
+#pragma unroll
+        for (int h = 0; h < 2; ++h)
+#pragma unroll
+          for (int ky = 0; ky < 3; ++ky)
+            if (sr - ky >= 0 && sr - ky < RPW)
+              acc16[sr - ky][h] = Mma16<T>::mma(wb[ky * 3 + kx], bq[sr & 1][h * 3 + kx], acc16[sr - ky][h]);
+    }
+    __builtin_amdgcn_s_setprio(0);
+    const uint32_t plane2 = (uint32_t)(H * a.ypitch) * 2u;
+    __amdgpu_buffer_rsrc_t yr = __builtin_amdgcn_make_buffer_rsrc((T*)a.y + (size_t)n * a.ybs, 0, (uint32_t)a.coutb * plane2, 0x00020000);
+#pragma unroll
+    for (int r = 0; r < RPW; ++r) {
+      const int gy = y0 + RPW * wave + r;
+      if (gy < H) {
+#pragma unroll
+        for (int h = 0; h < 2; ++h) {
+          const int gx = x0 + p16 + 16 * h;
+          float v[4];
+#pragma unroll
+          for (int k = 0; k < 4; ++k) { v[k] = acc16[r][h][k]; v[k] = fmaxf(v[k], v[k] * a.slope_b); }
+          const uint32_t off = (gx < W) ? (uint32_t)(4 * ko) * plane2 + (uint32_t)(gy * a.ypitch + gx) * 2u : 0x80000000u;
+          const uint32_t p01 = pack2<T>(v[0], v[1]), p23 = pack2<T>(v[2], v[3]);
+          __builtin_amdgcn_raw_buffer_store_b16((unsigned short)p01, yr, off, 0, 0);
+          __builtin_amdgcn_raw_buffer_store_b16((unsigned short)(p01 >> 16), yr, off + plane2, 0, 0);
+          __builtin_amdgcn_raw_buffer_store_b16((unsigned short)p23, yr, off + 2u * plane2, 0, 0);
+          __builtin_amdgcn_raw_buffer_store_b16((unsigned short)(p23 >> 16), yr, off + 3u * plane2, 0, 0);
+        }
+      }
+    }
+  }
+}
+
+template <typename T, int TH, bool A32, int NIN, int NAO, int KB, bool INIT, int CHA>
+int launch_tail_pair(TailArgs a, int B, hipStream_t stream) {
+  a.tiles_x = cdiv(a.W, TW);
+  a.tiles_y = cdiv(a.H, TH);
+  constexpr size_t lds = tail_lds_bytes<TH, NIN, NAO>();
+  static_assert(lds <= 80 * 1024, "tail pair: two workgroups per CU");
+  static LdsOptIn opt;
+  auto kern = &conv_tail_pair_kernel<T, TH, A32, NIN, NAO, KB, INIT, CHA>;
+  opt.ensure(reinterpret_cast<const void*>(kern), lds);
+  hipLaunchKernelGGL(kern, dim3((unsigned)(B * a.tiles_x * a.tiles_y)), dim3(NTHREADS), lds, stream, a);
+  return check_launch("conv_tail_pair_forward_c8");
+}
+
+template <typename T>
+int dispatch_tail_pair(const TailArgs& a, int B, int n8oct, int kb, hipStream_t stream) {
+  if (n8oct == 8 && a.couta == 32 && kb == 0 && !a.part) {
+    const bool c16 = g_c8_rpw4 && (long long)B * cdiv(a.W, TW) * cdiv(a.H, 16) >= g_rpw4_min;
+    return c16 ? launch_tail_pair<T, 8, true, 8, 4, 0, false, 2>(a, B, stream) : launch_tail_pair<T, 8, true, 8, 4, 0, false, 4>(a, B, stream);
+  }
+  if (n8oct == 2 && a.couta == 8 && kb == 2 && a.part) return launch_tail_pair<T, 8, false, 2, 1, 2, true, 2>(a, B, stream);
+  set_error("conv_tail_pair_forward_c8: no kernel for %d input octets, %d channels of layer A, %d shared octets, %s", n8oct, a.couta, kb,
+            a.part ? "partials" : "biases");
+  return UPF_EUNSUPPORTED;
+}
+
+}
+}
+
+extern "C" int upf_conv_tail_pair_forward_c8(const void* x8, long long x8_batch_stride, int n8_oct,
+                                             const void* wa_packed, const float* bias_a, int Cout_a, float slope_a, void* ya8, long long ya_batch_stride,
+                                             const void* wb_packed16, const float* bias_b, int Cout_b, int shared_oct, float slope_b,
+                                             const float* partial, long long partial_batch_stride, int partial_pitch, int partial_offset_a, int partial_offset_b,
+                                             void* y, long long y_batch_stride, int y_row_pitch, int B, int H, int W, int dtype, void* stream) {
+  using namespace upf;
+  UPF_REQUIRE(x8 && n8_oct > 0 && wa_packed && wb_packed16 && y, UPF_EINVAL, "conv_tail_pair_forward_c8: null pointer");
+  UPF_REQUIRE(partial || (bias_a && bias_b), UPF_EINVAL, "conv_tail_pair_forward_c8: biases or a partial record");
+  UPF_REQUIRE(B > 0 && H > 0 && W > 0 && Cout_a > 0 && Cout_a <= 32 && Cout_a % 8 == 0 && Cout_b > 0 && Cout_b <= 4 && shared_oct >= 0, UPF_EINVAL,
+              "conv_tail_pair_forward_c8: bad shape B=%d H=%d W=%d Cout_a=%d (<= 32, whole octets) Cout_b=%d (<= 4)", B, H, W, Cout_a, Cout_b);
+  UPF_REQUIRE(dtype == UPF_BF16 || dtype == UPF_F16, UPF_EDTYPE, "conv_tail_pair_forward_c8: bf16 / fp16 only");
+  UPF_REQUIRE(aligned_to(x8, 16) && x8_batch_stride % 8 == 0, UPF_EINVAL, "conv_tail_pair_forward_c8: the C8 input must be 16-byte aligned");
+  UPF_REQUIRE(!ya8 || (aligned_to(ya8, 16) && ya_batch_stride % 8 == 0), UPF_EINVAL, "conv_tail_pair_forward_c8: layer A's C8 output must be 16-byte aligned");
+  if (y_row_pitch == 0) y_row_pitch = W;
+  UPF_REQUIRE(y_row_pitch >= W, UPF_EINVAL, "conv_tail_pair_forward_c8: output row pitch %d < %d", y_row_pitch, W);
+  UPF_REQUIRE((long long)n8_oct * H * W * 16 < (1ll << 31) && (long long)Cout_b * H * y_row_pitch * 2 < (1ll << 31), UPF_EINVAL,
+              "conv_tail_pair_forward_c8: image too large for one buffer descriptor");
+  if (partial) {
+    UPF_REQUIRE(aligned_to(partial, 16) && partial_batch_stride % 4 == 0 && partial_pitch % 4 == 0 && partial_offset_a % 4 == 0 && partial_offset_b % 4 == 0 &&
+                partial_offset_a >= 0 && partial_offset_b >= 0 && partial_offset_a + (Cout_a + 3) / 4 * 4 <= partial_pitch &&
+                partial_offset_b + (Cout_b + 3) / 4 * 4 <= partial_pitch, UPF_EINVAL,
+                "conv_tail_pair_forward_c8: partial pitch %d / offsets %d, %d must be multiples of 4 floats holding the layers' channels", partial_pitch,
+                partial_offset_a, partial_offset_b);
+    UPF_REQUIRE((long long)H * W * partial_pitch * 4 < (1ll << 31), UPF_EINVAL, "conv_tail_pair_forward_c8: partial too large for one buffer descriptor");
+  }
+  UPF_REQUIRE(slope_a >= 0.f && slope_a <= 1.f && slope_b >= 0.f && slope_b <= 1.f, UPF_EINVAL, "conv_tail_pair_forward_c8: leaky slopes not in [0,1]");
+  conv::TailArgs a{x8, x8_batch_stride, wa_packed, bias_a, Cout_a, slope_a == 0.f ? 1.f : slope_a, ya8, ya_batch_stride,
+                   wb_packed16, bias_b, Cout_b, slope_b == 0.f ? 1.f : slope_b, partial, partial_batch_stride, partial_pitch, partial_offset_a, partial_offset_b,
+                   y, y_batch_stride, y_row_pitch, H, W, 0, 0};
+  return dtype == UPF_BF16 ? conv::dispatch_tail_pair<bf16_t>(a, B, n8_oct, shared_oct, (hipStream_t)stream)
+                           : conv::dispatch_tail_pair<f16_t>(a, B, n8_oct, shared_oct, (hipStream_t)stream);
+}
diff --git a/upflow_pytorch_amd/model/pwc_modules.py b/upflow_pytorch_amd/model/pwc_modules.py
--- a/upflow_pytorch_amd/model/pwc_modules.py
+++ b/upflow_pytorch_amd/model/pwc_modules.py
@@ -337,6 +337,20 @@
         return ops.conv_c8_forward_narrow_init_raw(x8_front, self.finish[j], part, self.offsets[j], self.widths[j], y, self.slopes[j])
 
 
+    def pair_ok(self, dtype):
+        if len(self.J) != 2 or self.J[1] != self.J[0] + 1 or self.J[0] != self.m + 1:
+            return False
+        ja, jb = self.J
+        return ops.conv_tail_pair_supported(dtype, self.widths[self.m], self.widths[ja], self.widths[jb], self.widths[self.m] // 8, True)
+
+    def finish_pair(self, x8_front, part, y5_octets, y_last):
+        self.get()
+        ja, jb = self.J
+        return ops.conv_tail_pair_forward_raw(x8_front, self.finish[ja], None, self.slopes[ja], self.widths[ja], y5_octets,
+                                              self.finish[jb], None, self.slopes[jb], self.widths[jb], y_last, part,
+                                              (self.offsets[ja], self.offsets[jb]))
+
+
 class _PackedConvPair(object):
 
     def __init__(self, seq_a, seq_b):
@@ -372,8 +386,53 @@
         return ops.conv_pair_forward_raw(x, pa, ba, self.slopes[0], pb, bb, self.slopes[1], y, self.strides)
 
 
+class _PackedTailPair(object):
+
+    def __init__(self, seq_a, seq_b):
+        self.convs = (seq_a[0], seq_b[0])
+        self.slopes = tuple(0.1 if any(isinstance(m_, nn.LeakyReLU) for m_ in q) else 0.0 for q in (seq_a, seq_b))
+        self.key = None
+        self.packed = self.packed_b = self.bias = self.bias_b = None
+
+    def _key(self):
+        k = []
+        for c in self.convs:
+            k += [c.weight._version, c.weight.dtype, c.weight.device, c.weight.data_ptr(), c.bias._version, c.bias.data_ptr()]
+        return tuple(k)
+
+    def get(self):
+        key = self._key()
+        if key != self.key:
+            a, b = self.convs
+            self.packed, self.packed_b = ops.conv_tail_pair_pack(a.weight, b.weight)
+            self.bias, self.bias_b = a.bias.detach().float().contiguous(), b.bias.detach().float().contiguous()
+            self.key = key
+        return self.packed, self.bias, self.packed_b, self.bias_b
+
+    def extra_operands(self):
+        return [self.packed_b, self.bias_b]
+
+    def invalidate(self):
+        self.key = None
+
+    def __call__(self, x8, y, ya8=None):
+        pa, ba, pb, bb = self.get()
+        a, b = self.convs
+        return ops.conv_tail_pair_forward_raw(x8, pa, ba, self.slopes[0], a.out_channels, ya8, pb, bb, self.slopes[1], b.out_channels, y)
+
+
 DUAL_1X1 = [True]
 FUSE_PAIRS = [True]
+FUSE_TAIL_PAIRS = [True]
+TAIL_PAIR_SITES = {'sgu': True, 'context': False}
+TAIL_PAIR_MIN_TILES = [512]
+
+
+def tail_pair_on(site, B, H, W, module=None):
+    return (FUSE_TAIL_PAIRS[0] and TAIL_PAIR_SITES[site] and not getattr(module, '_no_tail_pair', False)
+            and B * ((W + 31) // 32) * ((H + 7) // 8) >= TAIL_PAIR_MIN_TILES[0])
+
+
 MERGE_TAIL = [True]
 
 
@@ -550,10 +609,16 @@
             out = torch.empty((buf8.shape[0], self.conv_last[0].out_channels) + tuple(buf8.shape[2:4]), dtype=buf8.dtype, device=buf8.device)
         tail = packed[nl + 1] if (len(packed) > nl + 1 and MERGE_TAIL[0] and not getattr(self, '_no_merge_tail', False)) else None
         part = None
+        pair = (tail is not None and tail_pair_on('sgu', buf8.shape[0], buf8.shape[2], buf8.shape[3], self) and tail.pair_ok(buf8.dtype)
+                and tail.J[1] == nl)
         for k in range(nl + 1):
             y = buf8[:, starts[k + 1]:starts[k]] if k < nl else out
             if tail is not None and k == tail.m:
                 part = tail.main_pass(buf8[:, starts[k]:no], y)
+            elif pair and k == tail.J[0]:
+                tail.finish_pair(buf8[:, starts[k]:starts[tail.m]], part, y, out)
+            elif pair and k == tail.J[1]:
+                pass
             elif tail is not None and k in tail.J:
                 tail.finish_pass(k, buf8[:, starts[k]:starts[tail.m]], part, y)
             else:
@@ -639,10 +704,20 @@
         if key not in cache:
             chans = [s_[0].in_channels for s_ in self.convs]
             first = _PackedConvC8(self.convs[0], (), range(chans[0])) if in_map is None else _PackedConvC8(self.convs[0], list(in_map))
-            cache[key] = [first] + [_PackedConvC8(self.convs[i], range(chans[i])) for i in range(1, 7)]
+            cache[key] = [first] + [_PackedConvC8(self.convs[i], range(chans[i])) for i in range(1, 7)] + [_PackedTailPair(self.convs[5], self.convs[6])]
         B, H, W = x.shape[0], x.shape[2], x.shape[3]
         t = None
-        for i, pc in enumerate(cache[key]):
+        packed = cache[key]
+        ca, cb = self.convs[5][0], self.convs[6][0]
+        pair = (tail_pair_on('context', B, H, W, self) and packed[6].narrow and not packed[5].narrow
+                and all(all(isinstance(m_, (nn.Conv2d, nn.LeakyReLU)) for m_ in q_) for q_ in (self.convs[5], self.convs[6]))
+                and ca.bias is not None and cb.bias is not None and ca.padding == (1, 1) and cb.padding == (1, 1) and ca.groups == cb.groups == 1
+                and ca.weight.dtype == x.dtype and cb.weight.dtype == x.dtype
+                and ops.conv_tail_pair_supported(x.dtype, ca.in_channels, ca.out_channels, cb.out_channels, 0, False,
+                                                 (ca.dilation[0], cb.dilation[0]), (ca.kernel_size[0], cb.kernel_size[0]), (ca.stride[0], cb.stride[0])))
+        for i, pc in enumerate(packed[:7]):
+            if pair and i == 5:
+                return packed[7](t, torch.empty((B, cb.out_channels, H, W), dtype=x.dtype, device=x.device))
             co = self.convs[i][0].out_channels
             y = ops.c8_empty(B, co, H, W, x.dtype, x.device) if i < 6 else torch.empty((B, co, H, W), dtype=x.dtype, device=x.device)
             if i == 0:
diff --git a/upflow_pytorch_amd/ops.py b/upflow_pytorch_amd/ops.py
--- a/upflow_pytorch_amd/ops.py
+++ b/upflow_pytorch_amd/ops.py
@@ -775,6 +775,11 @@
             and partial.stride()[1:] == (H * W * 4, W * 4, 4, 1))
 
 
+def _partial_slot_ok(partial, offset, Cout):
+    offset, Cout = int(offset), int(Cout)
+    return offset >= 0 and offset % 4 == 0 and offset + (Cout + 3) // 4 * 4 <= 4 * partial.shape[1]
+
+
 def conv_c8_forward_split_raw(x8, packed, bias32, y8, partial, leaky_slope=0.0):
     B, n, H, W, _ = x8.shape
     Cout = bias32.shape[0]
@@ -804,12 +809,65 @@
         raise UpflowHipError('conv_c8_narrow_init: NCHW output must be a [%d,%d,%d,%d] channel slice' % (B, Cout, H, W))
     if not _partial_ok(partial, B, H, W):
         raise UpflowHipError('conv_c8_narrow_init: partial must be fp32 [B,Q,H,W,4] (planes of channel quads)')
+    if not _partial_slot_ok(partial, offset, Cout):
+        raise UpflowHipError('conv_c8_narrow_init: partial channels [%d, +%d) must start at a multiple of 4 inside the %d channels of the record'
+                             % (int(offset), int(Cout), 4 * partial.shape[1]))
     dev = x8.device
     if not (x8.is_cuda and y.is_cuda and partial.is_cuda) or x8.dtype != y.dtype:
         raise UpflowHipError('conv_c8_narrow_init: GPU tensors of one 16-bit dtype expected (there is no CPU fallback)')
     with torch.cuda.device(dev):
         _lib.call('upf_conv_forward_c8_narrow_init', _lib.ptr(x8), x8.stride(0), n, _lib.ptr(packed16), _lib.ptr(partial), partial.stride(0), 4 * partial.shape[1],
                   int(offset), _lib.ptr(y), y.stride(0), int(y_is_c8), B, int(Cout), H, W, float(leaky_slope), _lib.dtype_code(x8), _lib.stream_ptr(dev))
+    return y
+
+
+def conv_tail_pair_supported(dtype, cin_a, cout_a, cout_b, shared_oct=0, partial=False, dilations=(1, 1), kernel_sizes=(3, 3), strides=(1, 1)):
+    if dtype not in (torch.bfloat16, torch.float16):
+        return False
+    if tuple(dilations) != (1, 1) or tuple(kernel_sizes) != (3, 3) or tuple(strides) != (1, 1):
+        return False
+    if not 0 < cout_b <= 4:
+        return False
+    if partial:
+        return (cin_a, cout_a, shared_oct) == (16, 8, 2)
+    return (cin_a, cout_a, shared_oct) == (64, 32, 0)
+
+
+def conv_tail_pair_pack(w_a, w_b):
+    ca, cin = w_a.shape[0], w_a.shape[1]
+    if cin % 8 or ca % 8 or w_b.shape[1] % 8 or w_b.shape[1] < ca:
+        raise UpflowHipError('conv_tail_pair_pack: whole octets expected, got %s / %s' % (tuple(w_a.shape), tuple(w_b.shape)))
+    pa = conv_c8_pack(w_a, list(range(cin))) if ca > 16 else conv_c8_pack16(w_a, list(range(cin)))
+    return pa, conv_c8_pack16(w_b, list(range(w_b.shape[1])))
+
+
+def conv_tail_pair_forward_raw(x8, packed_a, bias_a, slope_a, cout_a, ya8, packed_b, bias_b, slope_b, cout_b, y, partial=None, offsets=(0, 0)):
+    B, n, H, W, _ = x8.shape
+    cout_a, cout_b = int(cout_a), int(cout_b)
+    shared = n if partial is not None else 0
+    if not conv_tail_pair_supported(x8.dtype, 8 * n, cout_a, cout_b, shared, partial is not None):
+        raise UpflowHipError('conv_tail_pair: no kernel for %d -> %d -> %d channels (%s) in %s' % (8 * n, cout_a, cout_b,
+                             'partials' if partial is not None else 'biases', x8.dtype))
+    if not _c8_view_ok(x8):
+        raise UpflowHipError('conv_tail_pair: x8 must be an octet slice of a contiguous C8 buffer')
+    if ya8 is not None and (ya8.dim() != 5 or not _c8_view_ok(ya8) or tuple(ya8.shape) != (B, cout_a // 8, H, W, 8) or ya8.dtype != x8.dtype):
+        raise UpflowHipError('conv_tail_pair: layer A\'s output must be octets [%d,%d,%d,%d,8]' % (B, cout_a // 8, H, W))
+    if y.dim() != 4 or tuple(y.shape) != (B, cout_b, H, W) or y.dtype != x8.dtype:
+        raise UpflowHipError('conv_tail_pair: NCHW output must be a [%d,%d,%d,%d] channel slice' % (B, cout_b, H, W))
+    yp = _pitch_or_raise(y, 'conv_tail_pair: y')
+    if partial is not None:
+        if not _partial_ok(partial, B, H, W) or not _partial_slot_ok(partial, offsets[0], cout_a) or not _partial_slot_ok(partial, offsets[1], cout_b):
+            raise UpflowHipError('conv_tail_pair: partial must be fp32 [B,Q,H,W,4] (planes of channel quads) holding both layers\' channels')
+    elif bias_a is None or bias_b is None or bias_a.shape[0] != cout_a or bias_b.shape[0] != cout_b:
+        raise UpflowHipError('conv_tail_pair: fp32 biases of %d and %d channels expected' % (cout_a, cout_b))
+    dev = x8.device
+    if not (x8.is_cuda and y.is_cuda) or packed_a.dtype != x8.dtype or packed_b.dtype != x8.dtype:
+        raise UpflowHipError('conv_tail_pair: GPU tensors of one 16-bit dtype expected (there is no CPU fallback)')
+    with torch.cuda.device(dev):
+        _lib.call('upf_conv_tail_pair_forward_c8', _lib.ptr(x8), x8.stride(0), n, _lib.ptr(packed_a), _lib.ptr(bias_a), cout_a, float(slope_a),
+                  _lib.ptr(ya8), ya8.stride(0) if ya8 is not None else 0, _lib.ptr(packed_b), _lib.ptr(bias_b), cout_b, shared, float(slope_b),
+                  _lib.ptr(partial), partial.stride(0) if partial is not None else 0, 4 * partial.shape[1] if partial is not None else 0,
+                  int(offsets[0]), int(offsets[1]), _lib.ptr(y), y.stride(0), yp, B, H, W, _lib.dtype_code(x8), _lib.stream_ptr(dev))
     return y
 
 
```

New measurement: 1938 frame-pairs/s. Within noise of the previous version (-0.1%).
